# UMich-CURLY/unified_cvo

Hardware: AMD Instinct MI355X
Metric: frame-pair align()/sec, 10k x 10k geometric clouds (higher is better)
Workload: dtype f32

## Files before the change

include/cvo_hip_debug.h:

```cpp
#ifndef CVO_HIP_DEBUG_H
#define CVO_HIP_DEBUG_H

#include "cvo_hip.h"

#ifdef __cplusplus
extern "C" {
#endif

int cvo_debug_last_ell(cvo_ctx* ctx, int K, float* mat, int* ind, unsigned int* nonzeros);
int cvo_debug_last_geometry(cvo_ctx* ctx, int* n_groups, int* pairs_per_group);
int cvo_debug_time_scan(cvo_ctx* ctx, int reps, float* ms);
int cvo_debug_scan_stats(cvo_ctx* ctx, unsigned long long* tiles, int* rows_per_tile, int* targets_per_tile);
int cvo_debug_time_kernels(cvo_ctx* ctx, int reps, float* ms_assoc, float* ms_coeff);
int cvo_debug_kernel_clock(cvo_ctx* ctx, float* ms_assoc, float* ms_coeff, unsigned long long* launches);
int cvo_debug_list_builds(cvo_ctx* ctx, unsigned long long* builds, unsigned long long* iterations,
                          unsigned long long* candidate_evaluations);
int cvo_debug_row_classes(cvo_ctx* ctx, int pair, int* overflow_rows, int* scanned_rows, int* dense_regime);
int cvo_debug_speculation(cvo_ctx* ctx, int pair, int* adopted, int* iterations);
int cvo_debug_last_candidates(cvo_ctx* ctx, unsigned long long* out);
int cvo_debug_scalar_math(cvo_ctx* ctx, int op, int n, const double* in, double* out);
int cvo_debug_verified_rows(cvo_ctx* ctx, unsigned long long* rows);
int cvo_debug_cloud_order(const cvo_cloud* cloud, int* out);
int cvo_debug_last_score_batch(const cvo_ctx* ctx, int* overlap_evals, int* chain_evals, int* launches);
int cvo_debug_device_memory(cvo_ctx* ctx, size_t* free_bytes, size_t* total_bytes);
int cvo_debug_irls_normal(cvo_ctx* ctx, const cvo_cloud* frame1, const cvo_cloud* frame2, const double pose1[12],
                          const double pose2[12], double* out);
int cvo_debug_irls_eval(cvo_ctx* ctx, int n_frames, const cvo_cloud* const* clouds, const double* poses, int n_edges,
                        const int* edge_frames, const int* slot_off, const int* ent_r, const int* ent_c, const float* ent_w,
                        int normal, double* out);
int cvo_debug_irls_gather(cvo_ctx* ctx, int K, int* r, int* c, float* w);
int cvo_debug_voxel_stats(cvo_ctx* ctx, unsigned long long* capacity, unsigned long long* occupied,
                          unsigned long long* probes_total, unsigned long long* probe_longest, unsigned long long* entered);
int cvo_debug_rgbd_stats(cvo_ctx* ctx, int* n_tried, int* potentials , int* counts ,
                         unsigned long long* edge_selected, unsigned long long* edge_points,
                         unsigned long long* surface_points, unsigned long long* with_depth, int* on_device);
int cvo_debug_stereo_stats(cvo_ctx* ctx, int capacity, int* n_tried, int* thresholds, int* counts, int* threshold_used,
                           unsigned* histogram , unsigned long long* candidates, unsigned long long* kept, int* on_device);
int cvo_debug_lidar_stats(cvo_ctx* ctx, unsigned long long* counts , int* on_device);
int cvo_debug_lidar_atan2(int n, const double* y, const double* x, double* out);
int cvo_debug_nlm_stats(cvo_ctx* ctx, int* on_device, int* mult, int* shift, int* n_nonzero, int* tile_w, int* tile_h,
                        int* table_in_lds);

#ifdef __cplusplus
}
#endif
#endif
```

unified_cvo_amd/_capi.py:

```python
import ctypes as C
import os

HERE = os.path.dirname(os.path.abspath(__file__))
LIB_PATH = os.path.join(HERE, "lib", "libcvo_hip.so")

CVO_OK = 0
CVO_RET_FLOW_VANISHED = -1
CVO_E_INVALID = -2
CVO_E_HIP = -3
CVO_E_NOMEM = -4
CVO_E_UNSUPPORTED = -5
CVO_E_VERIFY = -6


class cvo_params_t(C.Structure):

    _fields_ = [
        ("ell_init_first_frame", C.c_float),
        ("ell_init", C.c_float),
        ("ell_min", C.c_float),
        ("min_ell_iter_limit", C.c_int),
        ("ell_max", C.c_float),
        ("dl", C.c_double),
        ("dl_step", C.c_double),
# ... 71 lines not shown
        ("ret", C.c_int),
        ("final_ell", C.c_float),
        ("final_num_neighbors", C.c_int),
        ("seconds", C.c_double),
    ]


class cvo_align_opts_t(C.Structure):
    _fields_ = [
        ("max_iterations", C.c_int),
        ("override_state", C.c_int),
        ("ell0", C.c_float),
        ("K0", C.c_int),
        ("trace", C.POINTER(cvo_trace_t)),
        ("trace_capacity", C.c_int),
        ("trace_dense", C.c_int),
        ("trace_every", C.c_int),
        ("n_trace", C.POINTER(C.c_int)),
        ("iters_per_launch", C.c_int),
        ("use_graph", C.c_int),
        ("kernel_clock", C.c_int),
    ]


class cvo_multiframe_info_t(C.Structure):
    _fields_ = [
        ("outer_iterations", C.c_int),
        ("solves", C.c_int),
        ("steps", C.c_int),
        ("accepted_steps", C.c_int),
        ("final_ell", C.c_float),
        ("last_total_nonzeros", C.c_uint),
        ("seconds", C.c_double),
    ]


class cvo_multiframe_trace_t(C.Structure):
    _fields_ = [
        ("iter", C.c_int),
        ("n_active_edges", C.c_int),
        ("solved", C.c_int),
        ("steps", C.c_int),
        ("accepted", C.c_int),
        ("termination", C.c_int),
        ("ell", C.c_float),
        ("total_nonzeros", C.c_uint),
        ("cost_initial", C.c_double),
        ("cost_final", C.c_double),
    ]


class cvo_batch_result_t(C.Structure):
    _fields_ = [
        ("ticket", C.c_longlong),
        ("transform", C.c_float * 16),
        ("info", cvo_align_info_t),
    ]


class cvo_rgbd_frame_t(C.Structure):
    _fields_ = [
        ("rows", C.c_int),
        ("cols", C.c_int),
        ("channels", C.c_int),
        ("image", C.c_void_p),
        ("gray", C.c_void_p),
        ("depth", C.c_void_p),
        ("depth_type", C.c_int),
        ("fx", C.c_float),
        ("fy", C.c_float),
        ("cx", C.c_float),
        ("cy", C.c_float),
        ("scaling_factor", C.c_float),
        ("num_classes", C.c_int),
        ("semantic", C.c_void_p),
    ]


class cvo_fast_schedule_t(C.Structure):
    _fields_ = [("thresh", C.c_int), ("num_want", C.c_int), ("num_min", C.c_int), ("break_thresh", C.c_int)]


class cvo_stereo_frame_t(C.Structure):
    _fields_ = [
        ("rows", C.c_int),
        ("cols", C.c_int),
        ("channels", C.c_int),
        ("image", C.c_void_p),
        ("gray", C.c_void_p),
        ("disparity", C.c_void_p),
        ("fx", C.c_float),
        ("fy", C.c_float),
        ("cx", C.c_float),
        ("cy", C.c_float),
        ("baseline", C.c_float),
        ("num_classes", C.c_int),
        ("semantic", C.c_void_p),
    ]


class cvo_lidar_scan_t(C.Structure):
    _fields_ = [("n", C.c_int), ("xyzi", C.c_void_p), ("semantic", C.c_void_p), ("num_classes", C.c_int)]


class cvo_lidar_config_t(C.Structure):
    _fields_ = [
        ("n_scan", C.c_int),
        ("horizon_scan", C.c_int),
        ("ang_res_x", C.c_float),
        ("ground_scan_ind", C.c_int),
        ("sensor_min_range", C.c_float),
        ("sensor_mount_angle", C.c_float),
        ("segment_theta", C.c_float),
        ("segment_alpha_x", C.c_float),
        ("segment_alpha_y", C.c_float),
        ("segment_valid_point_num", C.c_int),
        ("segment_valid_line_num", C.c_int),
        ("edge_threshold", C.c_float),
        ("surf_threshold", C.c_float),
        ("intensity_bound", C.c_double),
        ("depth_bound", C.c_double),
        ("distance_bound", C.c_double),
        ("beam_num", C.c_int),
        ("tan_theta", C.c_double),
        ("sin_alpha_x", C.c_double),
        ("cos_alpha_x", C.c_double),
        ("sin_alpha_y", C.c_double),
        ("cos_alpha_y", C.c_double),
        ("tan_ground_lo", C.c_double),
        ("tan_ground_hi", C.c_double),
        ("tan_self_lo", C.c_double),
        ("tan_self_hi", C.c_double),
    ]


class cvo_lidar_rand_t(C.Structure):
    _fields_ = [("r", C.c_uint * 31), ("front", C.c_int), ("rear", C.c_int)]


class cvo_nlm_config_t(C.Structure):
    _fields_ = [("h", C.c_float), ("template_window", C.c_int), ("search_window", C.c_int)]


CVO_DEPTH_U16, CVO_DEPTH_F32 = 0, 1
CVO_SELECT_CV_FAST, CVO_SELECT_DSO_EDGES, CVO_SELECT_FULL = 0, 2, 8
CVO_FAST_RGBD, CVO_FAST_STEREO, CVO_FAST_STEREO_SEMANTIC = (9, 15000, 12000, 13), (4, 24000, 15000, 50), (4, 28000, 15000, 50)

EXPORTED = [
    "cvo_params_default", "cvo_ctx_create", "cvo_ctx_destroy", "cvo_last_error", "cvo_ctx_stream",
    "cvo_ctx_synchronize", "cvo_cloud_upload", "cvo_cloud_upload_aos192", "cvo_cloud_size", "cvo_cloud_free",
    "cvo_align", "cvo_align_ex", "cvo_align_batch", "cvo_batch_poses_to_device", "cvo_inner_product",
    "cvo_function_angle", "cvo_association", "cvo_association_non_isotropic", "cvo_cloud_transformed", "cvo_edge_kernel_matrix", "cvo_debug_last_ell", "cvo_debug_time_scan", "cvo_debug_time_kernels",
    "cvo_debug_kernel_clock",
    "cvo_debug_last_candidates", "cvo_debug_list_builds", "cvo_debug_row_classes", "cvo_debug_speculation", "cvo_debug_scan_stats", "cvo_debug_last_geometry", "cvo_version",
    "cvo_align_association", "cvo_debug_scalar_math", "cvo_debug_verified_rows", "cvo_debug_device_memory", "cvo_cloud_upload_many",
    "cvo_ctx_set_option", "cvo_ctx_advice", "cvo_debug_cloud_order",
    "cvo_process_hint_hw_queues", "cvo_shutdown",
    "cvo_batch_open", "cvo_batch_submit", "cvo_batch_poll", "cvo_batch_pending", "cvo_batch_stats", "cvo_batch_close",
    "cvo_inner_product_batch", "cvo_function_angle_batch", "cvo_debug_last_score_batch",
    "cvo_multiframe_align", "cvo_debug_irls_normal", "cvo_debug_irls_eval", "cvo_debug_irls_gather",
    "cvo_voxel_select", "cvo_voxel_select_host", "cvo_cloud_upload_voxel", "cvo_debug_voxel_stats",
    "cvo_rgbd_points", "cvo_rgbd_points_host", "cvo_cloud_upload_rgbd", "cvo_debug_rgbd_stats",
    "cvo_fast_select", "cvo_fast_select_host", "cvo_stereo_points", "cvo_stereo_points_host", "cvo_cloud_upload_stereo",
    "cvo_cloud_upload_stereo_recipe", "cvo_debug_stereo_stats",
    "cvo_lidar_config_default", "cvo_lidar_config_derive", "cvo_lidar_rand_seed", "cvo_lidar_rand_next", "cvo_lidar_select", "cvo_lidar_select_host",
    "cvo_cloud_upload_lidar", "cvo_debug_lidar_stats", "cvo_debug_lidar_atan2",
    "cvo_nlm_config_default", "cvo_nlm_weights", "cvo_nlm_denoise_host", "cvo_nlm_denoise", "cvo_nlm_denoise_lab_host",
    "cvo_nlm_denoise_lab", "cvo_debug_nlm_stats",
]

_libs = {}


def lib(path=None):
    path = os.path.abspath(path) if path else LIB_PATH
    if path in _libs:
        return _libs[path]
    if not os.path.exists(path):
        raise RuntimeError(
            f"{path} is missing: build it with `python -m unified_cvo_amd.build` "
            "(there is no CPU fallback for the hot path)")
    L = C.CDLL(path)
    vp, ip, fp = C.c_void_p, C.c_int, C.POINTER(C.c_float)
    L.cvo_version.restype = C.c_char_p
    L.cvo_params_default.argtypes = [C.POINTER(cvo_params_t)]
    L.cvo_params_default.restype = None
    L.cvo_ctx_create.argtypes = [ip, C.POINTER(vp)]
    L.cvo_ctx_destroy.argtypes = [vp]
    L.cvo_ctx_destroy.restype = None
    L.cvo_ctx_set_option.argtypes = [vp, C.c_char_p, C.c_char_p]
    L.cvo_last_error.argtypes = [vp]
    L.cvo_last_error.restype = C.c_char_p
    L.cvo_ctx_advice.argtypes = [vp]
    L.cvo_ctx_advice.restype = C.c_char_p
    L.cvo_ctx_stream.argtypes = [vp]
    L.cvo_ctx_stream.restype = vp
    L.cvo_ctx_synchronize.argtypes = [vp]
    L.cvo_cloud_upload.argtypes = [vp, ip, fp, fp, fp, fp, C.POINTER(vp)]
    L.cvo_cloud_upload_aos192.argtypes = [vp, ip, vp, C.POINTER(vp)]
    L.cvo_cloud_upload_many.argtypes = [vp, ip, C.POINTER(C.c_int), C.POINTER(fp), C.POINTER(fp), C.POINTER(fp),
                                        C.POINTER(fp), ip, C.POINTER(vp)]
    L.cvo_cloud_size.argtypes = [vp]
    L.cvo_cloud_free.argtypes = [vp]
    L.cvo_cloud_free.restype = None
    L.cvo_align.argtypes = [vp, C.POINTER(cvo_params_t), vp, vp, fp, fp, C.POINTER(cvo_align_info_t)]
    L.cvo_align_ex.argtypes = [vp, C.POINTER(cvo_params_t), vp, vp, fp, fp, C.POINTER(cvo_align_info_t),
                               C.POINTER(cvo_align_opts_t)]
    L.cvo_align_batch.argtypes = [vp, C.POINTER(cvo_params_t), ip, C.POINTER(vp), C.POINTER(vp), fp, fp,
                                  C.POINTER(cvo_align_info_t), C.POINTER(cvo_align_opts_t)]
    L.cvo_batch_poses_to_device.argtypes = [vp, vp, ip]
    L.cvo_batch_open.argtypes = [vp, C.POINTER(cvo_params_t), ip, ip, ip, ip, C.POINTER(cvo_align_opts_t), C.POINTER(vp)]
    L.cvo_batch_submit.argtypes = [vp, vp, vp, fp, ip, C.POINTER(C.c_longlong)]
    L.cvo_batch_poll.argtypes = [vp, ip, ip, C.POINTER(cvo_batch_result_t), C.POINTER(C.c_int)]
    L.cvo_batch_pending.argtypes = [vp]
    L.cvo_batch_stats.argtypes = [vp, C.POINTER(C.c_ulonglong), C.POINTER(C.c_ulonglong), C.POINTER(C.c_ulonglong)]
    L.cvo_batch_close.argtypes = [vp]
    L.cvo_batch_close.restype = None
    L.cvo_inner_product.argtypes = [vp, C.POINTER(cvo_params_t), vp, vp, fp, C.c_float, fp]
    L.cvo_function_angle.argtypes = [vp, C.POINTER(cvo_params_t), vp, vp, fp, C.c_float, ip, fp]
    L.cvo_inner_product_batch.argtypes = [vp, C.POINTER(cvo_params_t), ip, C.POINTER(vp), C.POINTER(vp), fp, fp, fp]
    L.cvo_function_angle_batch.argtypes = [vp, C.POINTER(cvo_params_t), ip, C.POINTER(vp), C.POINTER(vp), fp, fp, ip, fp]
    L.cvo_debug_last_score_batch.argtypes = [vp, C.POINTER(C.c_int), C.POINTER(C.c_int), C.POINTER(C.c_int)]
    L.cvo_association.argtypes = [vp, C.POINTER(cvo_params_t), vp, vp, fp, C.c_float, C.POINTER(C.c_int),
                                  C.POINTER(C.c_int), fp, C.c_size_t, C.POINTER(C.c_size_t)]
    L.cvo_association_non_isotropic.argtypes = [vp, C.POINTER(cvo_params_t), vp, vp, fp, fp, C.POINTER(C.c_int),
                                                 C.POINTER(C.c_int), fp, C.c_size_t, C.POINTER(C.c_size_t)]
    L.cvo_cloud_transformed.argtypes = [vp, vp, fp, C.POINTER(vp)]
    L.cvo_edge_kernel_matrix.argtypes = [vp, C.POINTER(cvo_params_t), vp, vp, C.c_float, ip, fp, C.POINTER(C.c_int), C.POINTER(C.c_uint), C.POINTER(C.c_uint)]
    L.cvo_debug_last_ell.argtypes = [vp, ip, fp, C.POINTER(C.c_int), C.POINTER(C.c_uint)]
    L.cvo_debug_time_scan.argtypes = [vp, ip, fp]
    L.cvo_debug_time_kernels.argtypes = [vp, ip, fp, fp]
    L.cvo_debug_kernel_clock.argtypes = [vp, fp, fp, C.POINTER(C.c_ulonglong)]
    L.cvo_debug_last_candidates.argtypes = [vp, C.POINTER(C.c_ulonglong)]
    L.cvo_debug_list_builds.argtypes = [vp, C.POINTER(C.c_ulonglong), C.POINTER(C.c_ulonglong), C.POINTER(C.c_ulonglong)]
    L.cvo_debug_row_classes.argtypes = [vp, C.c_int, C.POINTER(C.c_int), C.POINTER(C.c_int), C.POINTER(C.c_int)]
    L.cvo_debug_speculation.argtypes = [vp, C.c_int, C.POINTER(C.c_int), C.POINTER(C.c_int)]
    L.cvo_debug_last_geometry.argtypes = [vp, C.POINTER(C.c_int), C.POINTER(C.c_int)]
    L.cvo_debug_scan_stats.argtypes = [vp, C.POINTER(C.c_ulonglong), C.POINTER(C.c_int), C.POINTER(C.c_int)]
    L.cvo_align_association.argtypes = [vp, ip, C.POINTER(C.c_int), C.POINTER(C.c_int), fp, C.c_size_t,
                                        C.POINTER(C.c_size_t), C.POINTER(C.c_int), C.POINTER(C.c_int)]
    L.cvo_debug_scalar_math.argtypes = [vp, ip, ip, C.POINTER(C.c_double), C.POINTER(C.c_double)]
    L.cvo_debug_verified_rows.argtypes = [vp, C.POINTER(C.c_ulonglong)]
    L.cvo_debug_device_memory.argtypes = [vp, C.POINTER(C.c_size_t), C.POINTER(C.c_size_t)]
    L.cvo_debug_cloud_order.argtypes = [vp, C.POINTER(C.c_int)]
    dp = C.POINTER(C.c_double)
    L.cvo_multiframe_align.argtypes = [vp, C.POINTER(cvo_params_t), ip, C.POINTER(vp), dp, C.POINTER(C.c_int), ip,
                                       C.POINTER(C.c_int), C.POINTER(cvo_multiframe_info_t),
                                       C.POINTER(cvo_multiframe_trace_t), ip, C.POINTER(C.c_int)]
    L.cvo_debug_irls_normal.argtypes = [vp, vp, vp, dp, dp, dp]
    ipp = C.POINTER(C.c_int)
    L.cvo_debug_irls_eval.argtypes = [vp, ip, C.POINTER(vp), dp, ip, ipp, ipp, ipp, ipp, fp, ip, dp]
    L.cvo_debug_irls_gather.argtypes = [vp, ip, ipp, ipp, fp]
    L.cvo_voxel_select.argtypes = [vp, ip, fp, C.c_float, ipp, ipp]
    L.cvo_voxel_select_host.argtypes = [ip, fp, C.c_float, ipp, ipp]
    L.cvo_cloud_upload_voxel.argtypes = [vp, ip, fp, fp, fp, fp, C.c_float, C.POINTER(vp), ipp, ipp]
    L.cvo_debug_voxel_stats.argtypes = [vp] + [C.POINTER(C.c_ulonglong)] * 5
    fr = C.POINTER(cvo_rgbd_frame_t)
    L.cvo_rgbd_points.argtypes = [vp, fr, ip, ipp, ipp, fp, fp, fp, fp]
    L.cvo_rgbd_points_host.argtypes = [fr, ip, ipp, ipp, fp, fp, fp, fp]
    L.cvo_cloud_upload_rgbd.argtypes = [vp, fr, C.c_float, C.c_float, C.POINTER(vp), ipp, C.POINTER(C.c_ubyte), ipp]
    L.cvo_debug_rgbd_stats.argtypes = [vp, ipp, ipp, ipp] + [C.POINTER(C.c_ulonglong)] * 4 + [ipp]
    sched, sf, up = C.POINTER(cvo_fast_schedule_t), C.POINTER(cvo_stereo_frame_t), C.POINTER(C.c_ubyte)
    L.cvo_fast_select.argtypes = [vp, ip, ip, up, sched, ipp, ipp, ipp]
    L.cvo_fast_select_host.argtypes = [ip, ip, up, sched, ipp, ipp, ipp]
    L.cvo_stereo_points.argtypes = [vp, sf, ip, ipp, ipp, fp, fp, fp, fp]
    L.cvo_stereo_points_host.argtypes = [sf, ip, ipp, ipp, fp, fp, fp, fp]
    L.cvo_cloud_upload_stereo.argtypes = [vp, sf, ip, C.POINTER(vp), ipp, ipp]
    L.cvo_cloud_upload_stereo_recipe.argtypes = [vp, sf, C.c_float, C.c_float, C.POINTER(vp), ipp, up, ipp]
    L.cvo_debug_stereo_stats.argtypes = [vp, ip, ipp, ipp, ipp, ipp, C.POINTER(C.c_uint)] + [C.POINTER(C.c_ulonglong)] * 2 + [ipp]
    ls, lc, lr = C.POINTER(cvo_lidar_scan_t), C.POINTER(cvo_lidar_config_t), C.POINTER(cvo_lidar_rand_t)
    L.cvo_lidar_config_default.argtypes = [lc, ip]
    L.cvo_lidar_config_default.restype = None
    L.cvo_lidar_config_derive.argtypes = [lc]
    L.cvo_lidar_config_derive.restype = None
    L.cvo_lidar_rand_seed.argtypes = [lr, C.c_uint]
    L.cvo_lidar_rand_seed.restype = None
    L.cvo_lidar_rand_next.argtypes = [lr]
    L.cvo_lidar_rand_next.restype = C.c_uint
    L.cvo_debug_lidar_atan2.argtypes = [ip, dp, dp, dp]
    L.cvo_lidar_select_host.argtypes = [ls, lc, lr, ipp, up, ipp]
    L.cvo_lidar_select.argtypes = [vp, ls, lc, lr, ipp, up, ipp]
    L.cvo_cloud_upload_lidar.argtypes = [vp, ls, lc, lr, C.POINTER(vp), ipp, ipp]
    L.cvo_debug_lidar_stats.argtypes = [vp, C.POINTER(C.c_ulonglong), ipp]
    nc, bp = C.POINTER(cvo_nlm_config_t), C.POINTER(C.c_ubyte)
    L.cvo_nlm_config_default.argtypes = [nc]
    L.cvo_nlm_config_default.restype = None
    L.cvo_nlm_weights.argtypes = [nc, ip, ipp, ip, ipp, ipp, ipp, ipp]
    L.cvo_nlm_denoise_host.argtypes = [ip, ip, ip, bp, nc, bp]
    L.cvo_nlm_denoise.argtypes = [vp, ip, ip, ip, bp, nc, bp]
    L.cvo_nlm_denoise_lab_host.argtypes = [ip, ip, bp, nc, C.c_float, bp]
    L.cvo_nlm_denoise_lab.argtypes = [vp, ip, ip, bp, nc, C.c_float, bp]
    L.cvo_debug_nlm_stats.argtypes = [vp] + [ipp] * 7
    for name in EXPORTED:
        getattr(L, name)
    _libs[path] = L
    return L
```

unified_cvo_amd/api.py:

```python
import ctypes as C
import weakref
import os

import numpy as np

from . import _capi
from .params import CvoParams, read_cvo_params_yaml
from .synth import FEATURE_DIMENSIONS, NUM_CLASSES


class CvoError(RuntimeError):
    pass


def _fptr(a):
    return None if a is None else a.ctypes.data_as(C.POINTER(C.c_float))


class CvoPointCloud:

    def __init__(self, feature_dimensions=0, num_classes=0):
        self.num_points_ = 0
        self.feature_dimensions_ = feature_dimensions
        self.num_classes_ = num_classes
# ... 967 lines not shown
        f1, f2 = self._dev(frame1), self._dev(frame2)
        K = int(num_neighbors)
        mat = np.zeros((f1.n, K), np.float32)
        ind = np.zeros((f1.n, K), np.int32)
        nz = np.zeros(f1.n, np.uint32)
        total = C.c_uint()
        p = self.params.to_ctypes()
        self._check(self.L.cvo_edge_kernel_matrix(self.ctx, C.byref(p), f1.handle, f2.handle, float(ell), K, _fptr(mat),
                                                  ind.ctypes.data_as(C.POINTER(C.c_int)),
                                                  nz.ctypes.data_as(C.POINTER(C.c_uint)), C.byref(total)))
        return mat, ind, nz, total.value

    def align_multiframe(self, frames, hold_const, edges, trace=False):
        frames = list(frames)
        F = len(frames)
        pos = {id(f): i for i, f in enumerate(frames)}
        flat = []
        for a, b in edges:
            for f in (a, b):
                flat.append(int(f) if isinstance(f, (int, np.integer)) else pos[id(f)])
        E = len(flat) // 2
        handles = (C.c_void_p * max(F, 1))(*[f._init.handle for f in frames])
        poses = np.ascontiguousarray(np.concatenate([np.asarray(f.pose_vec, np.float64).reshape(12) for f in frames])
                                     if F else np.zeros(12), np.float64)
        hold = None if hold_const is None else np.ascontiguousarray([1 if h else 0 for h in hold_const], np.int32)
        if hold is not None and hold.shape[0] != F:
            raise ValueError("hold_const: one flag per frame")
        ed = np.ascontiguousarray(flat if E else [0, 0], np.int32)
        info = _capi.cvo_multiframe_info_t()
        cap = max(self.params.multiframe_max_iters + 2, 1) if trace else 0
        rows = (_capi.cvo_multiframe_trace_t * max(cap, 1))()
        n_trace = C.c_int()
        p = self.params.to_ctypes()
        ip = C.POINTER(C.c_int)
        self._check(self.L.cvo_multiframe_align(
            self.ctx, C.byref(p), F, handles, poses.ctypes.data_as(C.POINTER(C.c_double)),
            None if hold is None else hold.ctypes.data_as(ip), E, ed.ctypes.data_as(ip), C.byref(info), rows, cap,
            C.byref(n_trace)))
        for i, f in enumerate(frames):
            f.pose_vec[:] = poses[12 * i:12 * i + 12]
            f.transform_pointcloud()
        names = [n for n, _ in _capi.cvo_multiframe_trace_t._fields_]
        out = [{n: getattr(rows[i], n) for n in names} for i in range(n_trace.value)]
        return {n: getattr(info, n) for n, _ in _capi.cvo_multiframe_info_t._fields_}, out

    def multiframe_align_raw(self, clouds, poses, hold_const, edges, trace_capacity=0):
        F = len(clouds)
        handles = (C.c_void_p * max(F, 1))(*[None if c is None else c.handle for c in clouds])
        P = np.ascontiguousarray(np.asarray(poses, np.float64).reshape(-1) if F else np.zeros(12), np.float64).copy()
        hold = None if hold_const is None else np.ascontiguousarray(hold_const, np.int32)
        ed = np.ascontiguousarray(list(edges) if len(edges) else [0, 0], np.int32)
        info = _capi.cvo_multiframe_info_t()
        rows = (_capi.cvo_multiframe_trace_t * max(trace_capacity, 1))()
        n_trace = C.c_int(-7)
        p = self.params.to_ctypes()
        ip = C.POINTER(C.c_int)
        rc = self.L.cvo_multiframe_align(self.ctx, C.byref(p), F, handles, P.ctypes.data_as(C.POINTER(C.c_double)),
                                         None if hold is None else hold.ctypes.data_as(ip), len(edges) // 2,
                                         ed.ctypes.data_as(ip), C.byref(info), rows, trace_capacity, C.byref(n_trace))
        return rc, P, info, rows, n_trace.value

    def debug_irls_normal(self, frame1, frame2, pose1, pose2):
        f1, f2 = self._dev(frame1), self._dev(frame2)
        a = np.ascontiguousarray(np.asarray(pose1, np.float64).reshape(12))
        b = np.ascontiguousarray(np.asarray(pose2, np.float64).reshape(12))
        out = np.zeros(91, np.float64)
        dp = C.POINTER(C.c_double)
        self._check(self.L.cvo_debug_irls_normal(self.ctx, f1.handle, f2.handle, a.ctypes.data_as(dp),
                                                 b.ctypes.data_as(dp), out.ctypes.data_as(dp)))
        H = np.zeros((12, 12))
        H[np.triu_indices(12)] = out[13:]
        H = H + np.triu(H, 1).T
        return out[0], out[1:13].copy(), H

    def debug_irls_eval(self, clouds, poses, edge_frames, slot_off, ent_r, ent_c, ent_w, normal=True):
        devs = [self._dev(c) for c in clouds]
        F = len(devs)
        handles = (C.c_void_p * max(F, 1))(*[d.handle for d in devs])
        X = np.ascontiguousarray(np.asarray(poses, np.float64).reshape(-1) if F else np.zeros(12))
        ef = np.ascontiguousarray(np.asarray(edge_frames, np.int32).reshape(-1))
        E = ef.shape[0] // 2
        so = np.ascontiguousarray(slot_off, np.int32)
        r, c = np.ascontiguousarray(ent_r, np.int32), np.ascontiguousarray(ent_c, np.int32)
        w = np.ascontiguousarray(ent_w, np.float32)
        if X.shape[0] != 12 * max(F, 1) or so.shape[0] != E + 1 or not (r.shape == c.shape == w.shape) or \
                (E and r.shape[0] < so[-1]):
            raise ValueError("debug_irls_eval: array sizes do not match")
        out = np.zeros((E, 91) if normal else (E,), np.float64)
        ip, dp = C.POINTER(C.c_int), C.POINTER(C.c_double)
        pad = np.zeros(1, np.int32)
        self._check(self.L.cvo_debug_irls_eval(
            self.ctx, F, handles, X.ctypes.data_as(dp), E, (ef if E else pad).ctypes.data_as(ip), so.ctypes.data_as(ip),
            (r if r.size else pad).ctypes.data_as(ip), (c if c.size else pad).ctypes.data_as(ip),
            _fptr(w if w.size else np.zeros(1, np.float32)), 1 if normal else 0,
            (out if E else np.zeros(1)).ctypes.data_as(dp)))
        return out

    def debug_irls_gather(self, n_rows, K):
        r = np.zeros((n_rows, K), np.int32)
        c = np.zeros((n_rows, K), np.int32)
        w = np.zeros((n_rows, K), np.float32)
        ip = C.POINTER(C.c_int)
        self._check(self.L.cvo_debug_irls_gather(self.ctx, K, r.ctypes.data_as(ip), c.ctypes.data_as(ip), _fptr(w)))
        return r, c, w

    def debug_last_ell(self, n_rows, K):
        mat = np.zeros((n_rows, K), np.float32)
        ind = np.zeros((n_rows, K), np.int32)
        nz = np.zeros(n_rows, np.uint32)
        self._check(self.L.cvo_debug_last_ell(self.ctx, K, _fptr(mat), ind.ctypes.data_as(C.POINTER(C.c_int)),
                                              nz.ctypes.data_as(C.POINTER(C.c_uint))))
        return mat, ind, nz

    def debug_time_scan(self, reps=20):
        ms = C.c_float()
        self._check(self.L.cvo_debug_time_scan(self.ctx, reps, C.byref(ms)))
        return ms.value

    def debug_time_kernels(self, reps=20):
        a, c = C.c_float(), C.c_float()
        self._check(self.L.cvo_debug_time_kernels(self.ctx, reps, C.byref(a), C.byref(c)))
        return a.value, c.value

    def debug_kernel_clock(self):
        a, c, n = C.c_float(), C.c_float(), C.c_ulonglong()
        self._check(self.L.cvo_debug_kernel_clock(self.ctx, C.byref(a), C.byref(c), C.byref(n)))
        return a.value, c.value, n.value

    def debug_last_geometry(self):
        g, p = C.c_int(), C.c_int()
        self._check(self.L.cvo_debug_last_geometry(self.ctx, C.byref(g), C.byref(p)))
        return g.value, p.value

    def debug_scan_stats(self):
        t, r, c = C.c_ulonglong(), C.c_int(), C.c_int()
        self._check(self.L.cvo_debug_scan_stats(self.ctx, C.byref(t), C.byref(r), C.byref(c)))
        return t.value, r.value, c.value

    def debug_list_builds(self):
        b, it, ce = C.c_ulonglong(), C.c_ulonglong(), C.c_ulonglong()
        self._check(self.L.cvo_debug_list_builds(self.ctx, C.byref(b), C.byref(it), C.byref(ce)))
        return b.value, it.value, ce.value

    def debug_row_classes(self, pair=0):
        a, b, c = C.c_int(), C.c_int(), C.c_int()
        self._check(self.L.cvo_debug_row_classes(self.ctx, pair, C.byref(a), C.byref(b), C.byref(c)))
        return a.value, b.value, bool(c.value)

    def debug_speculation(self, pair=0):
        a, it = C.c_int(), C.c_int()
        self._check(self.L.cvo_debug_speculation(self.ctx, pair, C.byref(a), C.byref(it)))
        return a.value, it.value

    def advice(self):
        return self.L.cvo_ctx_advice(self.ctx).decode()

    def debug_scalar_math(self, op, items):
        dp = C.POINTER(C.c_double)
        if op == 7:
            a = np.ascontiguousarray(items, np.float64).reshape(-1)
            n = a.shape[0] - 2
            out = np.zeros(n, np.float64)
        else:
            it = np.atleast_2d(np.asarray(items, np.float64))
            n = it.shape[0]
            a = np.zeros((n, 16), np.float64)
            a[:, :it.shape[1]] = it
            out = np.zeros((n, 16), np.float64)
        self._check(self.L.cvo_debug_scalar_math(self.ctx, op, n, a.ctypes.data_as(dp), out.ctypes.data_as(dp)))
        return out

    def debug_device_memory(self):
        f, t = C.c_size_t(), C.c_size_t()
        self._check(self.L.cvo_debug_device_memory(self.ctx, C.byref(f), C.byref(t)))
        return f.value, t.value

    def debug_verified_rows(self):
        v = C.c_ulonglong()
        self._check(self.L.cvo_debug_verified_rows(self.ctx, C.byref(v)))
        return v.value

    def debug_last_candidates(self):
        v = C.c_ulonglong()
        self._check(self.L.cvo_debug_last_candidates(self.ctx, C.byref(v)))
        return v.value


class CvoFrameGPU:

    def __init__(self, gpu, pts, poses):
        self.gpu = gpu
        self.points = pts
        self.pose_vec = np.asarray(poses, np.float64).reshape(12).copy()
        self._init = gpu.upload(pts)
        self._transformed = None
        self.transform_pointcloud()

    def transform_pointcloud(self):
        if self._transformed is not None:
            self._transformed.free()
        self._transformed = self.gpu.transformed(self._init, self.pose_vec)

    def points_transformed_gpu(self):
        return self._transformed


class BinaryStateGPU:

    def __init__(self, frame1, frame2, num_neighbor, init_ell):
        self.frame1, self.frame2 = frame1, frame2
        self.init_num_neighbors = int(num_neighbor)
        self.num_neighbors = int(num_neighbor)
        self.ell = float(init_ell)
        self.iter = 0
        self.mat = self.ind = self.nonzeros = None
        self.nonzero_sum = 0

    def update_inner_product(self):
        last = int(self.nonzeros.max()) if self.nonzeros is not None and self.nonzeros.size else 0
        if last > 0:
            self.num_neighbors = min(self.init_num_neighbors, int(last * 1.1))
        gpu = self.frame1.gpu
        self.mat, self.ind, self.nonzeros, self.nonzero_sum = gpu.edge_kernel_matrix(
            self.frame1.points_transformed_gpu(), self.frame2.points_transformed_gpu(), self.ell, self.num_neighbors)
        self.iter += 1
        return self.nonzero_sum
```

unified_cvo_amd/csrc/cvo_debug.hip:

```cpp
extern "C" {

int cvo_debug_scalar_math(cvo_ctx* ctx, int op, int n, const double* in, double* out) {
  if (!ctx || !in || !out || n <= 0 || op < 0 || op > 13) return fail(ctx, CVO_E_INVALID, "cvo_debug_scalar_math: bad argument");
  HIP_TRY(ctx, hipSetDevice(ctx->device));
  const size_t n_in = op == 7 ? (size_t)n + 2 : 16 * (size_t)n, n_out = op == 7 ? (size_t)n : 16 * (size_t)n;
  double *d_in = nullptr, *d_out = nullptr;
  PairState* d_st = nullptr;
  int rc = CVO_OK;
  auto cleanup = [&]() {
    if (d_in) (void)hipFree(d_in);
    if (d_out) (void)hipFree(d_out);
    if (d_st) (void)hipFree(d_st);
  };
  if (hipMalloc(&d_in, sizeof(double) * n_in) != hipSuccess || hipMalloc(&d_out, sizeof(double) * n_out) != hipSuccess ||
      hipMalloc(&d_st, sizeof(PairState)) != hipSuccess) {
    cleanup();
    return fail(ctx, CVO_E_NOMEM, "cvo_debug_scalar_math: hipMalloc failed");
  }
  hipError_t e = hipMemcpyAsync(d_in, in, sizeof(double) * n_in, hipMemcpyHostToDevice, ctx->stream);
  if (e == hipSuccess) e = hipMemsetAsync(d_out, 0, sizeof(double) * n_out, ctx->stream);
  if (e == hipSuccess) e = hipMemsetAsync(d_st, 0, sizeof(PairState), ctx->stream);
  if (e == hipSuccess) {
    hipLaunchKernelGGL(k_scalar_math, dim3(op == 7 ? 1 : n), dim3(64), 0, ctx->stream, op, n, d_in, d_out, d_st);
    e = hipGetLastError();
// ... 23 lines not shown
  if (!ctx) return CVO_E_INVALID;
  if (overlap_evals) *overlap_evals = ctx->last_score_overlap;
  if (chain_evals) *chain_evals = ctx->last_score_chain;
  if (launches) *launches = ctx->last_score_launches;
  return CVO_OK;
}

int cvo_debug_verified_rows(cvo_ctx* ctx, unsigned long long* rows) {
  if (!ctx || !rows || ctx->last_pairs < 1) return fail(ctx, CVO_E_INVALID, "cvo_debug_verified_rows: bad argument");
  unsigned long long t = 0;
  for (int p = 0; p < ctx->last_pairs; p++) t += ctx->h_states[p].verify_rows;
  *rows = t;
  return CVO_OK;
}

int cvo_debug_last_candidates(cvo_ctx* ctx, unsigned long long* out) {
  if (!ctx || !out || ctx->last_pairs < 1) return fail(ctx, CVO_E_INVALID, "cvo_debug_last_candidates: bad argument");
  *out = ctx->h_states[0].ncand;
  return CVO_OK;
}

int cvo_debug_time_kernels(cvo_ctx* ctx, int reps, float* ms_assoc, float* ms_coeff) {
  if (!ctx || reps <= 0 || ctx->last_pairs < 1 || !ms_assoc || !ms_coeff)
    return fail(ctx, CVO_E_INVALID, "cvo_debug_time_kernels: bad argument");
  HIP_TRY(ctx, hipSetDevice(ctx->device));
  const int n_pairs = ctx->last_pairs, G = ctx->last.G;
  const DevParams& dp = ctx->last_params;
  const LaunchGeom& g0 = ctx->last.geom;
  const IterWords w = iteration_words({.idx32 = !g0.idx16, .rebuild_follows = true, .replay = true});
  float out[2] = {0.f, 0.f};
  for (int which = 0; which < 2; which++) {
    auto sweep = [&]() {
      for (int q = 0; q < G; q++) {
        const LaunchGeom g = group_geom(ctx, ctx->last, n_pairs, q);
        const PairDesc* descs = ctx->d_descs + g.p0;
        if (which == 0)
          launch_assoc(ctx->stream, g.idx16, g.feat, g.instr, g.nba, g.n_pairs, descs, ctx->d_params, ctx->d_states + g.p0, g.arena,
                       w.assoc);
        else
          launch_coeff(ctx->stream, g.instr, g.nba, g.csplit, g.n_pairs, descs, ctx->d_params, ctx->d_states + g.p0, g.arena, w.iter);
      }
    };
    sweep();
    HIP_TRY(ctx, hipEventRecord(ctx->ev_start, ctx->stream));
    for (int r = 0; r < reps; r++) sweep();
    HIP_TRY(ctx, hipEventRecord(ctx->ev_stop, ctx->stream));
    HIP_TRY(ctx, hipGetLastError());
    HIP_TRY(ctx, hipStreamSynchronize(ctx->stream));
    HIP_TRY(ctx, hipEventElapsedTime(&out[which], ctx->ev_start, ctx->ev_stop));
    out[which] /= (float)(reps * G);
  }
  if (dp.phase_ticks) {
    static unsigned long long h[2][8192][4];
    HIP_TRY(ctx, hipMemcpyFromSymbol(h, HIP_SYMBOL(g_phase_ticks), sizeof(h)));
    const int np = n_pairs - (int)((long)n_pairs * (G - 1) / G);
    for (int which = 0; which < 2; which++) {
      const int nb = std::min(4096, 8 * ((np + 7) / 8) * g0.nba * (which ? g0.csplit : 1));
      double sum[3] = {0, 0, 0}, mx[3] = {0, 0, 0};
      int cnt = 0;
      for (int b = 0; b < nb; b++) {
        if (!h[which][b][0] || !h[which][b][3]) continue;
        for (int q = 0; q < 3; q++) {
          const double d = (double)(long long)(h[which][b][q + 1] - h[which][b][q]);
          sum[q] += d;
          mx[q] = std::max(mx[q], d);
        }
        cnt++;
      }
      if (!cnt) continue;
      fprintf(stderr, "[cvo] %s: %d blocks; ticks (avg / max) %s %.0f / %.0f, row loop %.0f / %.0f, %s %.0f / %.0f\n",
              which ? "k_coeff" : "k_assoc", cnt, which ? "prologue + twist" : "prologue", sum[0] / cnt, mx[0], sum[1] / cnt,
              mx[1], which ? "reduction + counter" : "reduction + flow gate", sum[2] / cnt, mx[2]);
      if (which)
        for (int p = 0; p < std::min(np, 3); p++)
          fprintf(stderr, "[cvo]   pair %d, updating block: entry -> counter %.0f, update %.0f ticks\n", p,
                  (double)(long long)(h[1][4096 + p][1] - h[1][4096 + p][0]),
                  (double)(long long)(h[1][4096 + p][2] - h[1][4096 + p][1]));
      if (which) {
        unsigned long long u[8];
        HIP_TRY(ctx, hipMemcpyFromSymbol(u, HIP_SYMBOL(g_upd_ticks), sizeof(u)));
        fprintf(stderr, "[cvo]   inside the update (last pair to run it): reduce %lld, step %lld, pose + distance + indicator %lld, "
                        "update_tf + list bookkeeping %lld, rest %lld, write-back %lld ticks\n",
                (long long)(u[1] - u[0]), (long long)(u[2] - u[1]), (long long)(u[3] - u[2]), (long long)(u[4] - u[3]),
                (long long)(u[5] - u[4]), (long long)(u[6] - u[5]));
      }
    }
  }
  *ms_assoc = out[0];
  *ms_coeff = out[1];
  return CVO_OK;
}

int cvo_debug_kernel_clock(cvo_ctx* ctx, float* ms_assoc, float* ms_coeff, unsigned long long* launches) {
  if (!ctx || ctx->last_pairs < 1 || !ms_assoc || !ms_coeff)
    return fail(ctx, CVO_E_INVALID, "cvo_debug_kernel_clock: bad argument");
  if (!ctx->last_params.kernel_clock) return fail(ctx, CVO_E_INVALID, "cvo_debug_kernel_clock: the last call ran without CVO_KERNEL_CLOCK");
  HIP_TRY(ctx, hipSetDevice(ctx->device));
  if (ctx->clock_ms_per_tick <= 0.0) {
    HIP_TRY(ctx, hipStreamSynchronize(ctx->stream));
    float ms = 0.f;
    for (int rep = 0; rep < 2; rep++) {
      HIP_TRY(ctx, hipEventRecord(ctx->ev_start, ctx->stream));
      hipLaunchKernelGGL(k_hold, dim3(1), dim3(64), 0, ctx->stream, 1000000ull);
      HIP_TRY(ctx, hipEventRecord(ctx->ev_stop, ctx->stream));
      HIP_TRY(ctx, hipStreamSynchronize(ctx->stream));
      HIP_TRY(ctx, hipEventElapsedTime(&ms, ctx->ev_start, ctx->ev_stop));
    }
    ctx->clock_ms_per_tick = (double)ms / 1e6;
  }
  double sum[2] = {0, 0}, n[2] = {0, 0};
  for (int p = 0; p < ctx->last_pairs; p++)
    for (int w = 0; w < 2; w++) {
      sum[w] += (double)ctx->h_states[p].clk_sum[w];
      n[w] += (double)ctx->h_states[p].clk_n[w];
    }
  *ms_assoc = n[0] > 0 ? (float)(sum[0] / n[0] * ctx->clock_ms_per_tick) : 0.f;
  *ms_coeff = n[1] > 0 ? (float)(sum[1] / n[1] * ctx->clock_ms_per_tick) : 0.f;
  if (launches) *launches = (unsigned long long)n[1];
  return CVO_OK;
}

int cvo_debug_list_builds(cvo_ctx* ctx, unsigned long long* builds, unsigned long long* iterations,
                          unsigned long long* candidate_evaluations) {
  if (!ctx || !builds || ctx->last_pairs < 1) return fail(ctx, CVO_E_INVALID, "cvo_debug_list_builds: bad argument");
  unsigned long long b = 0, it = 0, ce = 0;
  for (int p = 0; p < ctx->last_pairs; p++) {
    b += (unsigned long long)ctx->h_states[p].n_builds;
    it += (unsigned long long)ctx->h_states[p].iterations;
    ce += ctx->h_states[p].ncand_total;
  }
  *builds = b;
  if (iterations) *iterations = it;
  if (candidate_evaluations) *candidate_evaluations = ce;
  return CVO_OK;
}

int cvo_debug_row_classes(cvo_ctx* ctx, int pair, int* overflow_rows, int* scanned_rows, int* dense_regime) {
  if (!ctx || pair < 0 || pair >= ctx->last_pairs) return fail(ctx, CVO_E_INVALID, "cvo_debug_row_classes: bad argument");
  const PairState& st = ctx->h_states[pair];
  if (overflow_rows) *overflow_rows = st.n_ovf;
  if (scanned_rows) *scanned_rows = st.n_scan;
  if (dense_regime) *dense_regime = st.all_dense;
  return CVO_OK;
}

int cvo_debug_speculation(cvo_ctx* ctx, int pair, int* adopted, int* iterations) {
  if (!ctx || pair < 0 || pair >= ctx->last_pairs) return fail(ctx, CVO_E_INVALID, "cvo_debug_speculation: bad argument");
  const PairState& st = ctx->h_states[pair];
  if (adopted) *adopted = st.n_adopted;
  if (iterations) *iterations = st.status ? st.iterations : st.k;
  return CVO_OK;
}

int cvo_debug_scan_stats(cvo_ctx* ctx, unsigned long long* tiles, int* rows_per_tile, int* targets_per_tile) {
  if (!ctx || !tiles || ctx->last_pairs < 1) return fail(ctx, CVO_E_INVALID, "cvo_debug_scan_stats: bad argument");
  HIP_TRY(ctx, hipSetDevice(ctx->device));
  unsigned long long total = 0;
  for (int p = 0; p < ctx->last_pairs; p++) {
    unsigned long long v = 0;
    HIP_TRY(ctx, hipMemcpy(&v, ctx->h_descs[p].tile_count, sizeof(v), hipMemcpyDeviceToHost));
    total += v;
  }
  *tiles = total;
  if (rows_per_tile) *rows_per_tile = ROWS_PER_GROUP;
  if (targets_per_tile) *targets_per_tile = 64 * ctx->last.geom.T;
  return CVO_OK;
}

int cvo_debug_last_geometry(cvo_ctx* ctx, int* n_groups, int* pairs_per_group) {
  if (!ctx || ctx->last_pairs < 1) return fail(ctx, CVO_E_INVALID, "cvo_debug_last_geometry: bad argument");
  if (n_groups) *n_groups = ctx->last.G;
  if (pairs_per_group) *pairs_per_group = (ctx->last_pairs + ctx->last.G - 1) / ctx->last.G;
  return CVO_OK;
}

int cvo_debug_time_scan(cvo_ctx* ctx, int reps, float* ms) {
  if (!ctx || !ms || reps <= 0 || ctx->last_pairs < 1)
    return fail(ctx, CVO_E_INVALID, "cvo_debug_time_scan: bad argument");
  HIP_TRY(ctx, hipSetDevice(ctx->device));
  const int n_pairs = ctx->last_pairs, G = ctx->last.G;
  auto sweep = [&]() {
    for (int q = 0; q < G; q++) {
      const LaunchGeom g = group_geom(ctx, ctx->last, n_pairs, q);
      launch_scan(ctx->stream, g.T, dim3(g.gx, g.gy, g.n_pairs), ctx->d_descs + g.p0, ctx->d_params, ctx->d_states + g.p0, true);
    }
  };
  sweep();
  HIP_TRY(ctx, hipEventRecord(ctx->ev_start, ctx->stream));
  for (int r = 0; r < reps; r++) sweep();
  HIP_TRY(ctx, hipEventRecord(ctx->ev_stop, ctx->stream));
  HIP_TRY(ctx, hipGetLastError());
  for (int p = 0; p < n_pairs; p++) {
    const PairDesc& D = ctx->h_descs[p];
    HIP_TRY(ctx, hipMemsetAsync(D.rowbits, 0, sizeof(unsigned) * (size_t)(ctx->last.N + 4) * D.rbw, ctx->stream));
  }
  HIP_TRY(ctx, hipStreamSynchronize(ctx->stream));
  float t = 0;
  HIP_TRY(ctx, hipEventElapsedTime(&t, ctx->ev_start, ctx->ev_stop));
  *ms = t / (reps * G);
  return CVO_OK;
}

}
```

unified_cvo_amd/csrc/cvo_device.h:

```cpp
#pragma once
#include <hip/hip_runtime.h>

#include "../../include/cvo_hip.h"
#include "../../include/cvo_hip_debug.h"

namespace cvo_dev {

constexpr int FD = CVO_FEATURE_DIMENSIONS;
constexpr int NC = CVO_NUM_CLASSES;
constexpr int FD_PAD = 8;
constexpr int NC_PAD = 20;
constexpr int IND_CAP = 512;

enum CallMode : int {
  CALL_ALIGN = 0,
  CALL_SINGLE = 1,
  CALL_NONISO = 2,
};

struct DevParams {
  float sp_thres, sigma2, c2, c_sigma2, s_ell, s_sigma, c, d;
  float log_geo;
  float d2_c_thres, d2_s_thres;
  float ell_min, ell_decay_rate;
  int ell_decay_start;
  int max_iter;
  float eps, eps_2, min_step, max_step;
  int K_max;
  int window;
  float stable_thr;
  int use_geo, use_col, use_sem, use_range_ell, use_geotype;
  int trace_dense, trace_every, trace_capacity;
  int mode;
  float kinv[9];
  float d2_cull;
  float s_ell_sq;
  int T;
  int groups_per_block;
  float skin_frac;
  float rebuild_shrink;
  int lean_U;
  int lean_U2;
  int calm_U;
  int shrink_align;
  float skin_min, skin_max;
  float skin_blend;
  int dense_regime;
  float lean_skin;
  float horizon_margin;
  int kernel_clock;
  int phase_ticks;
  int verify_lists;
  int keep_columns;
  int fast_div_cd;
  int row_max_cap;
  int row_max_busy;
  int long_lists;
  int debug_drop_partial;
  int debug_no_motion_bound;
  int no_speculate;
};

struct PairState {
  int status;
  int rebuild;
  int n_ovf;
  int K;
  float ell;
  int epoch;
  int k;
  int iterations;
  float Rinv[9], Tinv[3];
  float R[9], T[3];
  int ret;
  float step;
  float omega[3], v[3];
  unsigned nnz, max_nnz;
  double B, C, D, E;
  double dist;
  double asum;
  unsigned long long ncand;
  unsigned long long ncand_list;
  unsigned long long noverflow;
  unsigned long long ncand_total;
  int n_trace;
  float out_T[16];
  float Rb[9], Tb[3];
  float ell_build;
  float skin_rot, skin_tr;
  int n_builds;
  int n_adopted;
  int sync_err;
  int want_full, n_stalls;
  int all_dense;
  float skin_scale;
  int row_max;
  int n_scan;
  int s_head, s_size, e_head, e_size;
  float s_sum, e_sum;
  unsigned clk_last_assoc, clk_n[2];
  float last_used, last_rate;
  int K_last;
  float temp_coef;
  unsigned long long clk_sum[2];
  float sq[IND_CAP], eq[IND_CAP];
  float xi[48];
  unsigned long long clk_start[2];
  int verify_err, verify_k, verify_pos, verify_what;
  unsigned long long verify_rows;
};

#ifdef CVO_ELL8
struct EllEntry {
  float a;
  int p;
};
static_assert(sizeof(EllEntry) == 8, "EllEntry");
constexpr bool ELL8 = true;
#else
struct EllEntry {
  float a, yx, yy, yz;
};
static_assert(sizeof(EllEntry) == 16, "EllEntry");
constexpr bool ELL8 = false;
#endif
__device__ __forceinline__ EllEntry make_ell(float a, float yx, float yy, float yz, int p) {
#ifdef CVO_ELL8
  return EllEntry{a, p};
#else
  return EllEntry{a, yx, yy, yz};
#endif
}

struct RowRes {
  float o[3], v[3];
  double asum;
};
static_assert(sizeof(RowRes) == 32, "RowRes");

constexpr int ROW_PAD = 256;
__host__ __device__ inline size_t row_off_cand_cnt(int) { return 0; }
__host__ __device__ inline size_t row_off_ip(int Np) { return (size_t)4 * Np; }
__host__ __device__ inline size_t row_off_nnz(int Np) { return (size_t)8 * Np; }
__host__ __device__ inline size_t row_off_xp4(int Np) { return (size_t)16 * Np; }
__host__ __device__ inline size_t row_off_cand_j(int Np) { return (size_t)32 * Np; }
__host__ __device__ inline size_t row_off_ell(int Np) { return (size_t)160 * Np; }

struct PairDesc {
  int N, M, nblk_assoc, nblk_coeff;
  int* cand_cnt;
  void* cand_j;
  float4* xp4;
  int* ip;
  const float4* y4;
  EllEntry* ell;
  int* ell_j;
  unsigned* nnz_row;
  double* rowcoef;
  RowRes* rowres;
  unsigned long long* flow_part;
  unsigned long long* cnt_part;
  unsigned long long* shadow;
  unsigned long long* coef_part;
  int* done;
  int csplit;
  const float4* xfeat;
  const float4* yfeat;
  const float4* xlabel;
  const float4* ylabel;
  const float2* xgeo;
  const float2* ygeo;
  const int* xlid;
  const int* ylid;
  int Mpad, nchunks, nslices, rbw;
  int NG;
  int NGpad;
  float cx, cy, cz;
  float ymax;
  double sqrt_nm;
  const float4* x4;
  const float4* xs4;
  const int* xorder;
  const float4* ys4;
  const int* yorder;
  const int* yinv;
  float4* ycull;
  float4* xcull;
  int* rowperm;
  int* iorig;
  float4* gbox;
  float4* cellbox;
  float4* sbox;
  unsigned long long* masks;
  unsigned* rowbits;
  int* row_cnt;
  unsigned long long* tile_count;
  int* ovf_rows;
  unsigned long long* ovf_bits;
  unsigned short* long_j;
  unsigned long long* long_stamp;
  unsigned long long call_serial;
  int max_iter;
  PairState* st;
  cvo_trace_t* trace;
  int* status_out;
  int* want_out;
  int* status_host;
  int* want_host;
  double* asum_host;
  int* gate;
  int* gate_flow;
  int* dense_rel;
  int* ovf_wsum;
  int* word_base;
  int* dense_off;
};

constexpr unsigned NNZ_DENSE_FLAG = 0x80000000u;
__host__ __device__ inline unsigned nnz_count(unsigned v) { return v & ~NNZ_DENSE_FLAG; }
constexpr int ELL_LOWER_SLOTS = 64;
__host__ __device__ inline size_t ell_index(int N, int s, int pos, int off) {
  return off >= 0 ? (size_t)off + (size_t)s : (size_t)s * (size_t)N + (size_t)pos;
}
__host__ __device__ inline size_t ell_upper_capacity(int N, int K_max) {
  return K_max > ELL_LOWER_SLOTS ? (size_t)(K_max - ELL_LOWER_SLOTS) * (size_t)N : 0;
}
constexpr int COEFF_SPLIT_MAX = 32;
constexpr int ROWS_PER_GROUP = 4;

enum AssocFlags : int {
  ASSOC_LEAN = 1,
  ASSOC_REPLAY = 2,
  ASSOC_LEAN_DENSE = 4,
  ASSOC_ASUM_ONLY = 8,
};
enum IterFlags : int {
  ITER_LEAN = 1,
  ITER_REBUILD_FOLLOWS = 2,
  ITER_FROM_COEFF = 4,
  ITER_REPLAY = 8,
  ITER_LEAN_DENSE = 32,
  ITER_IDX32 = 64,
};
constexpr int ITER_HORIZON_SHIFT = 8;
__host__ __device__ constexpr int iter_horizon(int flags) { return flags >> ITER_HORIZON_SHIFT; }

struct SlotState {
  int rebuild, n_ovf;
};
template <class St>
__device__ __forceinline__ bool slot_waits(int flags, int lean, int lean_dense, const St* st) {
  bool w = false;
  if ((flags & lean) && (st->rebuild || (st->n_ovf > 0 && !(flags & lean_dense)))) w = true;
  return w;
}

constexpr int ASSOC_WORD_FLAG_BITS = 4, ASSOC_WORD_NBLK_BITS = 16;
constexpr int COEFF_WORD_NBLK_BITS = 14, COEFF_WORD_SPLIT_BITS = 6;
constexpr int LAUNCH_WORD_PAIR_SHIFT = 20, LAUNCH_WORD_PAIR_BITS = 12;
constexpr int LAUNCH_PAIRS_MAX = (1 << LAUNCH_WORD_PAIR_BITS) - 1;
constexpr int LAUNCH_NBLK_MAX = (1 << COEFF_WORD_NBLK_BITS) - 1;
struct AssocWord {
// ... 698 lines not shown
```

unified_cvo_amd/csrc/cvo_internal.h:

```cpp
#pragma once
#include <hip/hip_runtime.h>

#include <algorithm>
#include <atomic>
#include <chrono>
#include <climits>
#include <cmath>
#include <cstdio>
#include <cstdlib>
#include <cstdint>
#include <cstring>
#include <deque>
#include <map>
#include <memory_resource>
#include <mutex>
#include <string>
#include <thread>
#include <tuple>
#include <vector>

#include "cvo_kernels.h"

using namespace cvo_dev;

#include "cvo_options.h"

#define CVO_VERSION_STRING "unified_cvo_amd 0.1 (gfx950)"

struct cvo_cloud {
  cvo_ctx* ctx = nullptr;
  int device = 0;
  int n = 0;
  char* slab = nullptr;
  size_t slab_bytes = 0;
  float4* x4 = nullptr;
  float4* xs4 = nullptr;
  float4* feat = nullptr;
  float4* label = nullptr;
  float2* geo = nullptr;
  int* lid = nullptr;
  mutable char* zero_slab = nullptr;
  mutable float4* tile4 = nullptr;
  int* order = nullptr;
  int* inv = nullptr;
  std::vector<int> h_order;
  float cx = 0, cy = 0, cz = 0;
  float rmax = 0;
};

namespace {

enum class ChunkKind { Full, FullNoDense, Lean, ShortLean, Calm };
static const char* const kChunkNames[] = {"full", "full-nodense", "lean", "short", "calm"};

struct ChunkPlan {
  ChunkKind kind = ChunkKind::Full;
  bool dense = false;
  int U = 0;
  int period = 0;
  bool every_iteration() const { return kind == ChunkKind::Full || kind == ChunkKind::FullNoDense; }
};

struct ArenaArg {
  const char* base;
  unsigned stride256;
  int Npad;
};

struct GraphKey {
  ChunkPlan plan;
  int n_pairs = 0, p0 = 0, T = 0, gx = 0, gy = 0, npb = 0, nbl = 0, nba = 0, csplit = 0, dense_blocks = 0, horizon_cap = 0, feat = 0;
  bool idx16 = false, wide = false, instr = false, verify = false;
  ArenaArg arena{};
  auto fields() const {
    return std::tie(plan.kind, plan.dense, plan.U, plan.period, n_pairs, p0, T, gx, gy, npb, nbl, nba, csplit, dense_blocks,
                    horizon_cap, feat, idx16, wide, instr, verify, arena.base, arena.stride256, arena.Npad);
  }
  bool operator==(const GraphKey& o) const { return fields() == o.fields(); }
};

struct Dims {
  int Mpad, nchunks, rbw_max, nblk_assoc, NG, NGpad, Npad;
};

struct LaunchGeom {
  int n_pairs, p0, T, gx, gy, nba, npb, csplit;
  int nbl, nbv;
  int dense_blocks = DENSE_BLOCKS_MIN;
  int horizon_cap = 1 << 20;
  bool idx16, instr, verify;
  bool wide;
  int feat = FEAT_GEO;
  hipStream_t stream;
  ArenaArg arena;
};

struct BatchSetup {
  int N, M, G;
  bool long_lists = false;
  Dims d;
  size_t slot_bytes;
  LaunchGeom geom;
};

struct CachedGraph {
  hipGraphExec_t exec = nullptr;
  GraphKey key;
};

inline size_t align_up(size_t v, size_t a) { return (v + a - 1) / a * a; }

}

struct RgbdStatsAcc {
  int n_tried = 0, tried[8] = {}, count[8] = {};
  unsigned long long edge_selected = 0, edge_points = 0, surface_points = 0, with_depth = 0;
  int on_device = 0;
};

struct StereoStatsAcc {
  std::vector<int> tried, count;
  int threshold_used = -1;
  unsigned hist[257] = {};
  unsigned long long candidates = 0, kept = 0;
  int on_device = 0;
};

struct LidarStatsAcc {
  unsigned long long projected = 0, ground = 0, valid = 0, invalid = 0, segmented = 0, edges = 0, draws = 0, thinned = 0, edge_detected = 0;
  int on_device = 0;
};

struct NlmStatsAcc {
  int on_device = 0, mult = 0, shift = 0, n_nonzero = 0, tile_w = 0, tile_h = 0, table_in_lds = 0;
};

struct ScratchLayout {
  size_t off = 0;
  size_t take(size_t bytes) {
    const size_t o = off;
    off = align_up(off + bytes, 256);
    return o;
  }
};

struct DeviceScratch {
  char* p = nullptr;
  size_t bytes = 0;
  int reserve(cvo_ctx* ctx, size_t need, const char* what);
  void release() {
    if (p) (void)hipFree(p);
    p = nullptr;
    bytes = 0;
  }
};

struct cvo_ctx {
  int device = 0;
  CtxOptions opt;
  std::mutex upload_mutex;
  std::mutex kd_mutex;
  KdJob* d_kd_jobs = nullptr;
  int kd_jobs_cap = 0;
  hipStream_t stream = nullptr;
  hipStream_t upload_stream = nullptr;
  std::string err;
  std::string advice;
  char* arena = nullptr;
  size_t arena_bytes = 0;
  PairDesc* d_descs = nullptr;
  PairState* d_states = nullptr;
  int* d_status = nullptr;
  DevParams* d_params = nullptr;
  char* d_ctl = nullptr;
  char* h_ctl = nullptr;
  size_t ctl_bytes = 0, ctl_off_status = 0, ctl_off_descs = 0, ctl_off_states = 0;
  int cap_pairs = 0;
  std::vector<PairDesc> h_descs;
  std::vector<PairState> h_states;
  char* d_sb = nullptr;
  char* d_sb_table = nullptr;
  char* h_sb = nullptr;
  char* h_sb_res = nullptr;
  int sb_jobs_cap = 0, sb_tiles_cap = 0;
  int last_score_overlap = 0, last_score_chain = 0, last_score_launches = 0;
  int* h_status[2] = {nullptr, nullptr};
  hipEvent_t ev_start = nullptr, ev_stop = nullptr;
  static constexpr int MAX_GROUPS = MAX_STREAMS;
  hipStream_t gstream[MAX_GROUPS] = {};
  hipEvent_t ev_chk[2][MAX_GROUPS] = {};
  hipEvent_t ev_fork = nullptr, ev_join[MAX_GROUPS] = {};
  static constexpr int GRAPH_SLOTS = 48;
  CachedGraph graphs[MAX_GROUPS][GRAPH_SLOTS];
  CachedGraph chain_graph;
  int last_chunks = 0, last_lean_launches = 0, last_full_launches = 0;
  int last_pairs = 0;
  BatchSetup last{};
  DevParams last_params{};
  std::vector<int> last_xorder;
  bool queue_open = false;
  cvo_batch_queue* queue = nullptr;
  DeviceScratch vox_scratch;
  unsigned long long vox_capacity = 0;
  VoxelCtl vox_last{};
  DeviceScratch rgbd_scratch;
  std::vector<unsigned char> rgbd_excl;
  RgbdStatsAcc rgbd_last{};
  StereoStatsAcc stereo_last{};
  DeviceScratch lidar_scratch;
  LidarStatsAcc lidar_last{};
  DeviceScratch nlm_scratch;
  NlmStatsAcc nlm_last{};
  double clock_ms_per_tick = 0.0;
};

namespace {

int fail(cvo_ctx* ctx, int code, const std::string& msg) {
  if (ctx) ctx->err = msg;
  return code;
}

#define HIP_TRY(ctx, expr)                                                                       \
  do {                                                                                           \
    hipError_t e__ = (expr);                                                                     \
    if (e__ != hipSuccess)                                                                       \
      return fail(ctx, CVO_E_HIP, std::string(#expr) + ": " + hipGetErrorString(e__));           \
  } while (0)

}
```

unified_cvo_amd/csrc/cvo_k_assoc.h:

```cpp
#pragma once
#include "cvo_wave.h"
#include "cvo_pair_math.h"

namespace cvo_dev {

static_assert(sizeof(XiMats) <= 46 * sizeof(float), "PairState::xi holds an XiMats and the two words of its stamp");
__device__ __forceinline__ double coeff_twist_load(const PairDesc* __restrict__ D, int nparts, unsigned tag) {
  const int lane = threadIdx.x & 63;
  const CVO_GLOBAL unsigned long long* src = as_global(D->flow_part) + 2 * (lane & 7);
  double acc = 0;
  for (int b = lane >> 3; b < nparts; b += 64) {
    TaggedF64 p[8];
    const bool pad = (lane & 7) == 7;
    for (int polls = 0;; polls++) {
#pragma unroll
      for (int u = 0; u < 8; u++) p[u] = ld_tagged<true>(src + (size_t)min(b + 8 * u, nparts - 1) * FLOW_GRANULES);
      bool ok = true;
#pragma unroll
      for (int u = 0; u < 8; u++) ok = ok && (pad || p[u].carries(tag));
      if (__ballot(!ok) == 0ull) break;
      if (polls > PARTIAL_POLL_LIMIT) {
        if (lane == 0) D->st->sync_err = 1;
        break;
      }
      __builtin_amdgcn_s_sleep(2);
    }
#pragma unroll
    for (int u = 0; u < 8; u++) acc += (b + 8 * u < nparts) ? p[u].value() : 0.0;
  }
  return acc;
}
__device__ __forceinline__ void twist_finalize(const PairDesc* __restrict__ D, int nparts, unsigned tag, int stamp_epoch, int stamp_k) {
  double acc = coeff_twist_load(D, nparts, tag);
  acc += dpp_f64<0x128>(acc);
  acc = xor16_sum(acc);
  acc = xor32_sum(acc);
  float own = (float)acc;
  float ov[6];
#pragma unroll
  for (int q = 0; q < 6; q++) ov[q] = __builtin_bit_cast(float, __builtin_amdgcn_readlane(__builtin_bit_cast(int, own), q));
  float z = 0;
#pragma unroll
  for (int q = 0; q < 6; q++) z = z + ov[q] * ov[q];
  if (z > 0) {
    const float sq = sqrtf(z);
    own = own / sq;
#pragma unroll
    for (int q = 0; q < 6; q++) ov[q] = __builtin_bit_cast(float, __builtin_amdgcn_readlane(__builtin_bit_cast(int, own), q));
  }
  XiMats M;
  xi_mats(ov, ov + 3, M);
  if ((threadIdx.x & 63) == 0) {
    const float* mv = reinterpret_cast<const float*>(&M);
    float* dst = D->st->xi;
#pragma unroll
    for (int q = 0; q < (int)(sizeof(XiMats) / sizeof(float)); q++) dst[q] = mv[q];
    dst[46] = __int_as_float(stamp_epoch);
    dst[47] = __int_as_float(stamp_k);
  }
}
__device__ __forceinline__ bool flow_gate(const PairDesc* __restrict__ D, int nblocks, int nparts, unsigned tag, int stamp_epoch, int stamp_k) {
  __shared__ int s_flow_last;
  __syncthreads();
  if (threadIdx.x == 0) {
    const int done = __hip_atomic_fetch_add(D->gate_flow, 1, __ATOMIC_RELAXED, __HIP_MEMORY_SCOPE_AGENT);
    s_flow_last = (done == nblocks - 1) ? 1 : 0;
    if (done == nblocks - 1) __hip_atomic_store(D->gate_flow, 0, __ATOMIC_RELAXED, __HIP_MEMORY_SCOPE_AGENT);
  }
  __syncthreads();
  if (s_flow_last && threadIdx.x < 64) twist_finalize(D, nparts, tag, stamp_epoch, stamp_k);
  return s_flow_last != 0;
}

__device__ __forceinline__ void asum_gate(const PairDesc* __restrict__ D, int nblk) {
  __shared__ int s_asum_last;
  asm volatile("s_waitcnt vmcnt(0)" ::: "memory");
  __syncthreads();
  if (threadIdx.x == 0) {
    const int done = __hip_atomic_fetch_add(D->gate_flow, 1, __ATOMIC_RELAXED, __HIP_MEMORY_SCOPE_AGENT);
    s_asum_last = (done == nblk - 1) ? 1 : 0;
    if (done == nblk - 1) __hip_atomic_store(D->gate_flow, 0, __ATOMIC_RELAXED, __HIP_MEMORY_SCOPE_AGENT);
  }
  __syncthreads();
  if (!s_asum_last) return;
  double s = 0;
  if (threadIdx.x < 16)
    for (int b = (int)threadIdx.x; b < nblk; b += 16) s += ld_tagged<true>(as_global(D->flow_part) + (size_t)b * FLOW_GRANULES + 12).value();
  s += dpp_f64<DPP_XOR1>(s);
  s += dpp_f64<DPP_XOR2>(s);
  s += dpp_f64<DPP_HALF_MIRROR>(s);
  s += dpp_f64<DPP_MIRROR>(s);
  if (threadIdx.x == 0) {
    D->st->asum = s;
    *D->asum_host = s;
  }
}

__device__ unsigned long long g_phase_ticks[2][8192][4];
__device__ unsigned long long g_upd_ticks[8];
#define CVO_UPD_STAMP(i) do { if (P.phase_ticks && threadIdx.x == 0) g_upd_ticks[i] = __builtin_readcyclecounter(); } while (0)

__device__ __forceinline__ void pair_clock_begin(bool on, PairState* st, int which) {
  if (on && threadIdx.x == 0) st_x<true>(&st->clk_start[which], (unsigned long long)__builtin_amdgcn_s_memrealtime());
}
__device__ __forceinline__ unsigned long long pair_clock_peek(bool on, const PairState* st, int which) {
  return (on && threadIdx.x == 0) ? ld_x<true>(&st->clk_start[which]) : 0ull;
}
__device__ __forceinline__ unsigned pair_clock_ticks(unsigned long long t0) {
  const unsigned long long t1 = __builtin_amdgcn_s_memrealtime();
  return (t0 != 0ull && t0 <= t1 && t1 - t0 < 400000ull) ? (unsigned)(t1 - t0) : 0u;
}
struct AssocRowHead {
  int cnt, ip, j1;
  float4 x;
};
template <int NC>
struct BlockRedShared {
  double v[NC][ASSOC_THREADS + 8];
};
template <int NC>
__device__ __forceinline__ double block_reduce_lds(BlockRedShared<NC>& S, const double (&x)[NC]) {
  static_assert(NC <= 8, "eight lanes per component in one wave");
#pragma unroll
  for (int c = 0; c < NC; c++) S.v[c][threadIdx.x] = x[c];
  __syncthreads();
  double t = 0;
  if (threadIdx.x < 8 * NC) {
    const int c = threadIdx.x >> 3, g = threadIdx.x & 7;
    double p[ASSOC_THREADS / 8];
#pragma unroll
    for (int k = 0; k < ASSOC_THREADS / 8; k++) p[k] = S.v[c][8 * k + g];
#pragma unroll
    for (int k = 0; k < ASSOC_THREADS / 8; k++) t += p[k];
  }
  if (threadIdx.x < 64) {
    t += dpp_f64<DPP_XOR1>(t);
    t += dpp_f64<DPP_XOR2>(t);
    t += dpp_f64<DPP_HALF_MIRROR>(t);
  }
  return t;
}

struct AssocShared {
  union {
    BlockRedShared<7> red;
    EllEntry stage[ELL_STAGE][ASSOC_THREADS];
  };
  unsigned long long cnt[ASSOC_THREADS / 64][4];
};

template <typename IdxT, int ASSOC_CAP, int FEAT, bool INSTR>
__device__ __forceinline__ void assoc_phase(const DevParams& P, const PairDesc* __restrict__ D, const IterView& iv,
                                            AssocShared& S, const int bx, const AssocRowHead& head, const unsigned tag) {
  const int N = D->N;
  const int pos = bx * ASSOC_THREADS + threadIdx.x;
  const int K = iv.K;
  RowAcc A;
  A.slot = D->ell + pos;
  A.stage = (CVO_LDS ell_vec_t*)&S.stage[0][threadIdx.x];
  unsigned overflowed = 0;
  unsigned long long tt1 = 0, tt2 = 0;
  if (pos < N) {
    const int j1s = head.j1;
    const int j2s = (int)(reinterpret_cast<const IdxT*>(D->cand_j) + pos)[N];
    const int cnt = head.cnt;
    overflowed = cnt > min(iv.row_max, ASSOC_CAP) ? 1u : 0u;
    if (!overflowed) {
      const int i = head.ip;
      const float4 x = head.x;
      RowData r = make_row(P, x, iv.ell);
      if (FEAT == FEAT_HOT) r.lid = D->xlid[i];
      const FeatDen F = make_feat_den(P);
      const V3 pxe{x.x, x.y, x.z};
      const Pose& pose = iv.pose;
      const CVO_GLOBAL IdxT* cj = as_global(reinterpret_cast<const IdxT*>(D->cand_j)) + pos;
      const CVO_GLOBAL f32x4* ysrc = (const CVO_GLOBAL f32x4*)D->ys4;
      int j1 = cnt > 0 ? j1s : 0;
      int j2 = cnt > 1 ? j2s : 0;
      if (INSTR) tt1 = __builtin_readcyclecounter();
      float4 y1 = ldg_xyz(ysrc + j1);
      const CVO_GLOBAL IdxT* cjn = cj + (size_t)2 * N;
      if (geo_fast_path<FEAT>(P)) {
        for (int k = 0; k < cnt && A.nnz < (unsigned)K; k++) {
          const int j = j1;
          const float4 ycur = y1;
          j1 = j2;
          y1 = ldg_xyz(ysrc + j1);
          if (k + 2 < cnt) j2 = (int)*cjn;
          cjn += N;
          const V3 ytv = transform_point(pose.Ri, pose.Ti, ycur.x, ycur.y, ycur.z);
          visit_pair_geo(P, F, N, r, pxe, j, ytv, A);
        }
      } else {
        for (int k = 0; k < cnt && A.nnz < (unsigned)K; k++) {
          const int j = j1;
          const float4 ycur = y1;
          j1 = j2;
          y1 = ldg_xyz(ysrc + j1);
          if (k + 2 < cnt) j2 = (int)*cjn;
          cjn += N;
          const V3 ytv = transform_point(pose.Ri, pose.Ti, ycur.x, ycur.y, ycur.z);
          visit_pair_yt<FEAT>(P, D, F, i, pos, N, r, pxe, j, make_float4(ytv.x, ytv.y, ytv.z, 0.f), A);
        }
      }
      D->nnz_row[pos] = A.nnz;
      {
        const unsigned ns = min(A.nnz, (unsigned)ELL_STAGE);
        EllEntry* dst = D->ell + pos;
        for (unsigned q = 0; q < ns; q++) {
          const ell_vec_t ev = A.stage[q * ASSOC_THREADS];
#ifdef CVO_ELL8
          asm volatile("flat_store_dwordx2 %0, %1 sc1" ::"v"(dst), "v"(ev) : "memory");
#else
          asm volatile("flat_store_dwordx4 %0, %1 sc1" ::"v"(dst), "v"(ev) : "memory");
#endif
          dst += N;
        }
      }
      if (INSTR) tt2 = __builtin_readcyclecounter();
    } else {
      const RowRes rr = D->rowres[pos];
      A.o0 = rr.o[0]; A.o1 = rr.o[1]; A.o2 = rr.o[2];
      A.v0 = rr.v[0]; A.v1 = rr.v[1]; A.v2 = rr.v[2];
      A.asum = rr.asum;
      A.nnz = nnz_count(D->nnz_row[pos]);
    }
  }
  if (INSTR && P.phase_ticks && threadIdx.x == 0) {
    g_phase_ticks[0][blockIdx.x & 8191][1] = tt1;
    g_phase_ticks[0][blockIdx.x & 8191][2] = tt2;
  }
  float fq[6];
  {
    const float fn[6] = {A.o0, A.o1, A.o2, A.v0, A.v1, A.v2};
    const bool safe = P.fast_div_cd != 0 && fdiv_operands_safe(fn);
    if (__ballot(!safe) == 0ull) {
      const FDivU uc = fdiv_prepare(P.c), ud = fdiv_prepare(P.d);
#pragma unroll
      for (int q = 0; q < 3; q++) {
        fq[q] = fdiv_hoisted(fn[q], uc);
        fq[3 + q] = fdiv_hoisted(fn[3 + q], ud);
      }
    } else {
#pragma unroll
      for (int q = 0; q < 3; q++) {
        fq[q] = fn[q] / P.c;
        fq[3 + q] = fn[3 + q] / P.d;
      }
    }
  }
  const double red[7] = {(double)fq[0], (double)fq[1], (double)fq[2], (double)fq[3], (double)fq[4], (double)fq[5], A.asum};
  constexpr int NW = ASSOC_THREADS / 64;
  const int wave = threadIdx.x >> 6, lane = threadIdx.x & 63;
  const unsigned long long nn = wave_sum_u32(A.nnz);
  const unsigned mx = wave_max_u32(A.nnz);
  const unsigned long long nov = (unsigned long long)__builtin_popcountll(__ballot(overflowed != 0));
  if (lane == 0) {
    S.cnt[wave][0] = nn;
    S.cnt[wave][1] = mx;
    S.cnt[wave][2] = 0ull;
    S.cnt[wave][3] = nov;
  }
  __syncthreads();
  const double tot = block_reduce_lds<7>(S.red, red);
  if (threadIdx.x < 56 && (threadIdx.x & 7) == 0 && !(P.debug_drop_partial == 1 && bx == 1)) {
    st_tagged(D->flow_part + (size_t)bx * FLOW_GRANULES + 2 * (threadIdx.x >> 3), tot, tag);
  } else if (threadIdx.x == 57) {
    unsigned long long a0 = 0, a1 = 0, a2 = 0, a3 = 0;
#pragma unroll
    for (int w = 0; w < NW; w++) {
      a0 += S.cnt[w][0];
      a1 = max(a1, S.cnt[w][1]);
      a2 += S.cnt[w][2];
      a3 += S.cnt[w][3];
    }
    unsigned long long* cp = D->cnt_part + (size_t)bx * 4;
    cp[0] = a0;
    cp[1] = a1;
    cp[2] = a2;
    cp[3] = a3;
  }
}

template <typename IdxT, int ASSOC_CAP, int FEAT, bool INSTR>
__global__ __launch_bounds__(ASSOC_THREADS, FEAT != FEAT_GEO ? 1 : CVO_ASSOC_WAVES) void k_assoc(const PairDesc* __restrict__ descs,
                                                          const DevParams* __restrict__ Pp,
                                                          const PairState* __restrict__ states,
                                                          const char* __restrict__ arena, int lean_nblk_pairs,
                                                          unsigned stride256, int Npad) {
  const unsigned long long tt0 = INSTR ? __builtin_readcyclecounter() : 0ull;
  const AssocWord aw = unpack_assoc_word(lean_nblk_pairs);
  const int lean = aw.flags, nblk = aw.nblk, n_pairs = aw.n_pairs;
  PairBlock pb;
  if (!pair_block(nblk, n_pairs, pb)) return;
  const PairDesc* __restrict__ D = descs + pb.pair;
  const PairState* __restrict__ st = states + pb.pair;
  AssocRowHead head;
  {
    const char* wb = arena + (size_t)pb.pair * ((size_t)stride256 << 8);
    const int pos = pb.bx * ASSOC_THREADS + threadIdx.x;
    head.ip = FEAT != FEAT_GEO ? reinterpret_cast<const int*>(wb + row_off_ip(Npad))[pos] : 0;
    head.j1 = (int)reinterpret_cast<const IdxT*>(wb + row_off_cand_j(Npad))[pos];
    head.x = reinterpret_cast<const float4*>(wb + row_off_xp4(Npad))[pos];
    head.cnt = __float_as_int(head.x.w);
  }
  const int status_v = st->status, rebuild_v = st->rebuild, n_ovf_v = st->n_ovf;
  const DevParams P = *Pp;
  {
    const int n = D->N, k = st->K;
    const int* a0 = D->cand_cnt;
    const void* a1 = D->cand_j;
    const float4* a2 = D->xp4;
    const float4* a3 = D->ys4;
    const EllEntry* a4 = D->ell;
    const float e = st->ell, r0 = st->Rinv[0], t0 = st->Tinv[0];
    asm volatile("" ::"s"(n), "s"(k), "s"(a0), "s"(a1), "s"(a2), "s"(a3), "s"(a4), "s"(e), "s"(r0), "s"(t0), "s"(P.sp_thres),
                 "s"(P.log_geo), "s"(P.c), "s"(P.d), "s"(P.d2_c_thres));
  }
  const bool replay = (lean & ASSOC_REPLAY) != 0;
  if (!replay && status_v != 0) return;
  const SlotState sv{rebuild_v, n_ovf_v};
  if (slot_waits(lean, ASSOC_LEAN, ASSOC_LEAN_DENSE, &sv)) return;
  pair_clock_begin(INSTR && P.kernel_clock && (lean & (ASSOC_LEAN | ASSOC_REPLAY)) == ASSOC_LEAN && pb.bx == 0, const_cast<PairState*>(st), 0);
  __shared__ AssocShared S;
  const int stamp_epoch = st->epoch, stamp_k = st->k;
  const unsigned tag = partial_tag(D->call_serial, (unsigned)stamp_k);
  assoc_phase<IdxT, ASSOC_CAP, FEAT, INSTR>(P, D, load_iter_view(st), S, pb.bx, head, tag);
  if (threadIdx.x >= 64) return;
  if (P.mode == CALL_ALIGN) {
    const unsigned long long clk0 = pair_clock_peek(INSTR && P.kernel_clock && (lean & (ASSOC_LEAN | ASSOC_REPLAY)) == ASSOC_LEAN, st, 0);
    const bool last = flow_gate(D, nblk, nblk, tag, stamp_epoch, stamp_k);
    if (last && threadIdx.x == 0 && clk0) D->st->clk_last_assoc = pair_clock_ticks(clk0);
  } else if (lean & ASSOC_ASUM_ONLY) {
    asum_gate(D, nblk);
  }
  if (INSTR && P.phase_ticks && threadIdx.x == 0) {
    g_phase_ticks[0][blockIdx.x & 8191][0] = tt0;
    g_phase_ticks[0][blockIdx.x & 8191][3] = __builtin_readcyclecounter();
  }
}

}
```

unified_cvo_amd/csrc/cvo_kernels.h:

```cpp
#pragma once
#include "cvo_device.h"

#if defined(__HIP_DEVICE_COMPILE__) && !defined(__gfx950__)
#error "unified_cvo_amd kernels target gfx950 (MI355X) only: build with --offload-arch=gfx950"
#endif

#ifndef CVO_COEFF_WAVES
#define CVO_COEFF_WAVES 1
#endif
#ifndef CVO_ASSOC_WAVES
#define CVO_ASSOC_WAVES 6
#endif


#include "cvo_wave.h"
#include "cvo_pair_math.h"
#include "cvo_k_prep.h"
#include "cvo_k_scan.h"
#include "cvo_k_list.h"
#include "cvo_k_assoc.h"
#include "cvo_k_assoc_dense.h"
#include "cvo_update.h"
#include "cvo_k_coeff.h"
#include "cvo_k_overlap.h"
#include "cvo_k_coeff_dense.h"
#include "cvo_k_debug.h"
#include "cvo_k_cloud.h"
#include "cvo_k_irls.h"
#include "cvo_k_compact.h"
#include "cvo_k_voxel.h"
#include "cvo_k_rgbd.h"
#include "cvo_k_fast.h"
#include "cvo_k_stereo.h"
#include "cvo_k_lidar.h"
#include "cvo_k_nlm.h"
```

unified_cvo_amd/csrc/cvo_launch.hip:

```cpp
#ifndef CVO_COEFF_DENSE_MULTI_FROM
#define CVO_COEFF_DENSE_MULTI_FROM 8
#endif

namespace {

void choose_scan_config(const cvo_ctx* ctx, int n_pairs, int NG, int Mpad, int* T_out, int* gpb_out) {
  const int T = 2;
  const long slices = Mpad / (64 * T);
  const int ngr = (int)align_up((size_t)NG, 64);
  int gpb = ngr;
  while (gpb > 64) {
    const long waves = slices * ((ngr + gpb - 1) / gpb) * n_pairs;
    if (waves >= 4096) break;
    gpb = (int)align_up((size_t)gpb / 2, 64);
  }
  *T_out = T;
  *gpb_out = gpb;
}

void launch_scan(hipStream_t s, int T, dim3 grid, const PairDesc* descs, const DevParams* dp, const PairState* st, bool force) {
  switch (T) {
    case 1: hipLaunchKernelGGL(k_scan<1>, grid, dim3(256), 0, s, descs, dp, st, force); break;
    case 2: hipLaunchKernelGGL(k_scan<2>, grid, dim3(256), 0, s, descs, dp, st, force); break;
    case 4: hipLaunchKernelGGL(k_scan<4>, grid, dim3(256), 0, s, descs, dp, st, force); break;
    default: hipLaunchKernelGGL(k_scan<8>, grid, dim3(256), 0, s, descs, dp, st, force); break;
  }
}

inline dim3 row_grid(int nblk, int n_pairs) { return dim3((unsigned)(nblk * ((n_pairs + 7) / 8 * 8))); }

void launch_list(hipStream_t s, bool idx16, int nblk, int n_pairs, const PairDesc* descs, const DevParams* dp,
                 const PairState* st) {
  const dim3 blk(LIST_THREADS), grid = row_grid(nblk, n_pairs);
  if (idx16)
    hipLaunchKernelGGL((k_list<unsigned short, ASSOC_CAP16>), grid, blk, 0, s, descs, dp, st, nblk, n_pairs);
  else
    hipLaunchKernelGGL((k_list<int, ASSOC_CAP32>), grid, blk, 0, s, descs, dp, st, nblk, n_pairs);
}

template <typename IdxT, int CAP, int FEAT>
void launch_assoc_t(hipStream_t s, bool instr, dim3 grid, const PairDesc* descs, const DevParams* dp, const PairState* st,
                    const ArenaArg& A, int packed) {
  const dim3 blk(ASSOC_THREADS);
  if (instr)
    hipLaunchKernelGGL((k_assoc<IdxT, CAP, FEAT, true>), grid, blk, 0, s, descs, dp, st, A.base, packed, A.stride256, A.Npad);
  else
    hipLaunchKernelGGL((k_assoc<IdxT, CAP, FEAT, false>), grid, blk, 0, s, descs, dp, st, A.base, packed, A.stride256, A.Npad);
}

void launch_assoc(hipStream_t s, bool idx16, int feat, bool instr, int nblk, int n_pairs, const PairDesc* descs,
                  const DevParams* dp, const PairState* st, const ArenaArg& A, int flags) {
  const dim3 grid = row_grid(nblk, n_pairs);
  const int packed = pack_assoc_word(flags, nblk, n_pairs);
#define CVO_ASSOC_CASE(F)                                                                              \
  case F:                                                                                              \
    if (idx16)                                                                                         \
      launch_assoc_t<unsigned short, ASSOC_CAP16, F>(s, instr, grid, descs, dp, st, A, packed);        \
    else                                                                                               \
      launch_assoc_t<int, ASSOC_CAP32, F>(s, instr, grid, descs, dp, st, A, packed);                   \
    break;
  switch (feat) {
    CVO_ASSOC_CASE(FEAT_GEO)
    CVO_ASSOC_CASE(FEAT_COL)
    CVO_ASSOC_CASE(FEAT_HOT)
    default:
      CVO_ASSOC_CASE(FEAT_ALL)
  }
#undef CVO_ASSOC_CASE
}

void launch_coeff(hipStream_t s, bool instr, int nblk, int split, int n_pairs, const PairDesc* descs, const DevParams* dp,
                  PairState* st, const ArenaArg& A, int flags) {
  const int packed = pack_coeff_word(nblk, split, n_pairs);
  if (instr)
    hipLaunchKernelGGL(k_coeff<true>, row_grid(nblk * split + 1, n_pairs), dim3(ASSOC_THREADS), 0, s, descs, dp, st, A.base, flags,
                       packed, A.stride256, A.Npad);
  else
    hipLaunchKernelGGL(k_coeff<false>, row_grid(nblk * split + 1, n_pairs), dim3(ASSOC_THREADS), 0, s, descs, dp, st, A.base, flags,
                       packed, A.stride256, A.Npad);
}

void launch_verify(hipStream_t s, int feat, int nblk, int n_pairs, const PairDesc* descs, const DevParams* dp, const int* st,
                   int flags) {
  const dim3 grid((unsigned)nblk, (unsigned)n_pairs);
  if (feat != FEAT_GEO)
    hipLaunchKernelGGL(k_verify<FEAT_ALL>, grid, dim3(256), 0, s, descs, dp, st, flags);
  else
    hipLaunchKernelGGL(k_verify<FEAT_GEO>, grid, dim3(256), 0, s, descs, dp, st, flags);
}

inline bool dense_wide(int N, int n_pairs) { return n_pairs <= 1 && N <= DENSE_BLOCKS_MAX / 2; }

void launch_dense(hipStream_t s, int feat, bool wide, int n_pairs, int dense_blocks, const PairDesc* descs, const DevParams* dp,
                  const PairState* st) {
  const dim3 grid(dense_blocks, n_pairs);
#define CVO_LAUNCH_DENSE(F)                                                                                  \
  do {                                                                                                       \
    if (wide)                                                                                                \
      hipLaunchKernelGGL((k_assoc_dense<F, 4, true>), grid, dim3(256), 0, s, descs, dp, st);                 \
    else                                                                                                     \
      hipLaunchKernelGGL((k_assoc_dense<F, 4, false>), grid, dim3(256), 0, s, descs, dp, st);                \
  } while (0)
  switch (feat) {
    case FEAT_GEO: CVO_LAUNCH_DENSE(FEAT_GEO); break;
    case FEAT_COL: CVO_LAUNCH_DENSE(FEAT_COL); break;
    case FEAT_HOT: CVO_LAUNCH_DENSE(FEAT_HOT); break;
    default: CVO_LAUNCH_DENSE(FEAT_ALL); break;
  }
#undef CVO_LAUNCH_DENSE
}

inline int call_feat(const DevParams& dp, bool all_one_hot) {
  if (dp.mode == CALL_NONISO) return FEAT_ALL;
  if (!(dp.use_col || dp.use_sem || dp.use_geotype)) return FEAT_GEO;
  if (!dp.use_sem) return FEAT_COL;
  return all_one_hot ? FEAT_HOT : FEAT_ALL;
}

struct IterSlot {
  bool lean = false;
  bool lean_dense = false;
  bool idx32 = false;
  bool rebuild_follows = false;
  int horizon = 0;
  bool replay = false;
  bool asum_only = false;
};
struct IterWords {
  int assoc;
  int iter;
};
inline IterWords iteration_words(const IterSlot& s) {
  const bool lean_dense = s.lean && s.lean_dense;
  return {(s.lean ? ASSOC_LEAN : 0) | (s.replay ? ASSOC_REPLAY : 0) | (lean_dense ? ASSOC_LEAN_DENSE : 0) |
              (s.asum_only ? ASSOC_ASUM_ONLY : 0),
          (s.lean ? ITER_LEAN : 0) | (s.rebuild_follows ? ITER_REBUILD_FOLLOWS : 0) | (s.replay ? ITER_REPLAY : 0) |
              (lean_dense ? ITER_LEAN_DENSE : 0) | (s.idx32 ? ITER_IDX32 : 0) | (s.horizon << ITER_HORIZON_SHIFT)};
}

void launch_init(cvo_ctx* c, const LaunchGeom& g) {
  hipLaunchKernelGGL(k_update<true>, dim3(g.n_pairs), dim3(64), 0, g.stream, c->d_descs + g.p0, c->d_params,
                     c->d_status + 2 * g.p0, iteration_words({}).iter);
}

void launch_rebuild(cvo_ctx* c, const LaunchGeom& g) {
  const PairDesc* descs = c->d_descs + g.p0;
  const PairState* states = c->d_states + g.p0;
  hipLaunchKernelGGL(k_prep, dim3(g.npb, g.n_pairs), dim3(PREP_THREADS), 0, g.stream, descs, c->d_params, states);
  launch_scan(g.stream, g.T, dim3(g.gx, g.gy, g.n_pairs), descs, c->d_params, states, false);
  launch_list(g.stream, g.idx16, g.nbl, g.n_pairs, descs, c->d_params, states);
}

void launch_core(cvo_ctx* c, const LaunchGeom& g, const IterSlot& slot) {
  const PairDesc* descs = c->d_descs + g.p0;
  const int* st = c->d_status + 2 * g.p0;
  const IterWords w = iteration_words(slot);
  const bool dense = !slot.lean || slot.lean_dense;
  if (dense) launch_dense(g.stream, g.feat, g.wide, g.n_pairs, g.dense_blocks, descs, c->d_params, c->d_states + g.p0);
  launch_assoc(g.stream, g.idx16, g.feat, g.instr, g.nba, g.n_pairs, descs, c->d_params, c->d_states + g.p0, g.arena, w.assoc);
  if (g.verify) launch_verify(g.stream, g.feat, g.nbv, g.n_pairs, descs, c->d_params, st, w.assoc);
  if (dense)
    hipLaunchKernelGGL((k_coeff_dense<4>), dim3(g.n_pairs <= 4 ? std::min(2 * g.dense_blocks, (int)DENSE_BLOCKS_MAX) : g.dense_blocks, g.n_pairs), dim3(256), 0, g.stream, descs,
                       c->d_params, c->d_states + g.p0, g.n_pairs >= CVO_COEFF_DENSE_MULTI_FROM ? 8 : 1);
  launch_coeff(g.stream, g.instr, g.nba, g.csplit, g.n_pairs, descs, c->d_params, c->d_states + g.p0, g.arena, w.iter);
}

void launch_chunk(cvo_ctx* c, const LaunchGeom& g, const ChunkPlan& p) {
  if (p.every_iteration()) {
    const IterSlot slot{.lean = p.kind == ChunkKind::FullNoDense, .idx32 = !g.idx16, .rebuild_follows = true};
    for (int u = 0; u < p.U; u++) {
      launch_rebuild(c, g);
      launch_core(c, g, slot);
    }
    return;
  }
  for (int u = 0; u < p.U; u++) {
    if (u % p.period == 0) launch_rebuild(c, g);
    const bool last = (u % p.period == p.period - 1) || u == p.U - 1;
    launch_core(c, g, {.lean = true, .lean_dense = p.dense, .idx32 = !g.idx16, .rebuild_follows = last,
                       .horizon = std::min(p.period, g.horizon_cap)});
  }
}

GraphKey graph_key(const LaunchGeom& g, const ChunkPlan& plan) {
  return {plan, g.n_pairs, g.p0, g.T, g.gx, g.gy, g.npb, g.nbl, g.nba, g.csplit, g.dense_blocks, g.horizon_cap, g.feat,
          g.idx16, g.wide, g.instr, g.verify, g.arena};
}

template <typename Launches>
int capture_graph(cvo_ctx* ctx, CachedGraph& cg, const GraphKey& key, hipStream_t s, const LaunchGeom* flight, int n_flight,
                  const char* what, Launches&& launches) {
  if (cg.exec && cg.key == key) return CVO_OK;
  if (cg.exec) (void)hipGraphExecDestroy(cg.exec);
  cg.exec = nullptr;
  hipGraph_t gr = nullptr;
  HIP_TRY(ctx, hipStreamBeginCapture(s, hipStreamCaptureModeThreadLocal));
  launches();
  const hipError_t e_launch = hipGetLastError();
  hipError_t e = hipStreamEndCapture(s, &gr);
  if (e == hipSuccess && e_launch != hipSuccess) e = e_launch;
  if (e == hipSuccess) e = hipGraphInstantiate(&cg.exec, gr, nullptr, nullptr, 0);
  if (gr) (void)hipGraphDestroy(gr);
  if (e != hipSuccess) {
    cg.exec = nullptr;
    for (int q = 0; q < n_flight; q++) (void)hipStreamSynchronize(flight[q].stream);
    return fail(ctx, CVO_E_HIP, std::string(what) + ": " + hipGetErrorString(e));
  }
  cg.key = key;
  return CVO_OK;
}

}
```

unified_cvo_amd/csrc/cvo_options.h:

```cpp
#pragma once

namespace {

constexpr int MAX_STREAMS = 8;
constexpr float SKIN_MIN = 0.05f;

enum class CloudOrder { Device, Host, Virtual };

struct CtxOptions {
  float skin = 1.0f;
  float lean_skin = 0.5f;
  float horizon_margin = 0.3f;
  float skin_max = 0.35f;
  int shrink_align = 0;
  int lean_U = 8;
  bool no_lean = false, no_dense_regime = false, fixed_chunks = false;
  int first_U = 0;
  int first_chunks = 2;
  int streams = 0;
  int queue_admit = 4;
  bool no_sort = false, no_long_lists = false, no_onehot = false, ip_chain = false, keep_columns = false, no_speculate = false;
  CloudOrder order = CloudOrder::Device;
  int row_max = ASSOC_CAP16;
  int voxel_host = -1;
  int rgbd_host = -1;
  int stereo_host = -1;
  int lidar_host = -1;
  int nlm_host = -1;
  int fast_tile = 1;
  int voxel_prepass = 1;
  int verbose = 0;
  bool kernel_clock = false, phase_ticks = false, verify_lists = false, debug_no_motion_bound = false;
  int debug_drop_partial = 0;
};

enum class OptKind { Flag, Level, Integer, Real, Order };

struct OptionSpec {
  const char* name;
  OptKind kind;
  bool CtxOptions::*flag;
  int CtxOptions::*integer;
  float CtxOptions::*real;
  double lo, hi;
};
constexpr OptionSpec opt_flag(const char* name, bool CtxOptions::*m) { return {name, OptKind::Flag, m, nullptr, nullptr, 0, 0}; }
constexpr OptionSpec opt_int(const char* name, int CtxOptions::*m, double lo = INT_MIN, double hi = INT_MAX) { return {name, OptKind::Integer, nullptr, m, nullptr, lo, hi}; }
constexpr OptionSpec opt_real(const char* name, float CtxOptions::*m, double lo) { return {name, OptKind::Real, nullptr, nullptr, m, lo, HUGE_VAL}; }

constexpr OptionSpec kOptions[] = {
    opt_real("SKIN", &CtxOptions::skin, 0.0),
    opt_real("SKIN_MAX", &CtxOptions::skin_max, SKIN_MIN),
    opt_real("LEAN_SKIN", &CtxOptions::lean_skin, 0.1),
    opt_real("HORIZON_MARGIN", &CtxOptions::horizon_margin, 0.0),
    opt_int("SHRINK_ALIGN", &CtxOptions::shrink_align, 0),
    opt_int("LEAN_U", &CtxOptions::lean_U, 1),
    opt_flag("NO_LEAN", &CtxOptions::no_lean),
    opt_flag("NO_DENSE_REGIME", &CtxOptions::no_dense_regime),
    opt_flag("FIXED_CHUNKS", &CtxOptions::fixed_chunks),
    opt_int("FIRST_U", &CtxOptions::first_U, 1),
    opt_int("FIRST_CHUNKS", &CtxOptions::first_chunks, 0),
    opt_int("STREAMS", &CtxOptions::streams, 1, MAX_STREAMS),
    opt_int("QUEUE_ADMIT", &CtxOptions::queue_admit, 1),
    opt_flag("NO_SORT", &CtxOptions::no_sort),
    {"ORDER", OptKind::Order, nullptr, nullptr, nullptr, 0, 0},
    opt_flag("NO_LONG_LISTS", &CtxOptions::no_long_lists),
    opt_int("ROW_MAX", &CtxOptions::row_max, 1, ASSOC_CAP16),
    opt_flag("NO_ONEHOT", &CtxOptions::no_onehot),
    opt_flag("IP_CHAIN", &CtxOptions::ip_chain),
    opt_flag("KEEP_COLUMNS", &CtxOptions::keep_columns),
    opt_flag("NO_SPECULATE", &CtxOptions::no_speculate),
    opt_int("VOXEL_HOST", &CtxOptions::voxel_host, -1, 1),
    opt_int("VOXEL_PREPASS", &CtxOptions::voxel_prepass, 0, 1),
    opt_int("RGBD_HOST", &CtxOptions::rgbd_host, -1, 1),
    opt_int("STEREO_HOST", &CtxOptions::stereo_host, -1, 1),
    opt_int("LIDAR_HOST", &CtxOptions::lidar_host, -1, 1),
    opt_int("NLM_HOST", &CtxOptions::nlm_host, -1, 1),
    opt_int("FAST_TILE", &CtxOptions::fast_tile, 0, 1),
    {"VERBOSE", OptKind::Level, nullptr, &CtxOptions::verbose, nullptr, 0, 0},
    opt_flag("KERNEL_CLOCK", &CtxOptions::kernel_clock),
    opt_flag("PHASE_TICKS", &CtxOptions::phase_ticks),
    opt_flag("VERIFY_LISTS", &CtxOptions::verify_lists),
    opt_flag("DEBUG_NO_MOTION_BOUND", &CtxOptions::debug_no_motion_bound),
    opt_int("DEBUG_DROP_PARTIAL", &CtxOptions::debug_drop_partial),
};

inline void parse_option(CtxOptions& o, const OptionSpec& s, const char* text) {
  const CtxOptions def;
  char* end = nullptr;
  const bool on = text && !(std::strtol(text, &end, 10) == 0 && end != text);
  switch (s.kind) {
    case OptKind::Flag: o.*s.flag = on; break;
    case OptKind::Level: o.*s.integer = on ? std::max(1, atoi(text)) : 0; break;
    case OptKind::Integer: o.*s.integer = text ? std::max((int)s.lo, std::min(atoi(text), (int)s.hi)) : def.*s.integer; break;
    case OptKind::Real: o.*s.real = text ? std::max((float)s.lo, std::min((float)atof(text), (float)s.hi)) : def.*s.real; break;
    case OptKind::Order: o.order = !text ? def.order : (!std::strcmp(text, "host") ? CloudOrder::Host : (!std::strcmp(text, "virtual") ? CloudOrder::Virtual : CloudOrder::Device)); break;
  }
}

}
```

unified_cvo_amd/csrc/cvo_sched.hip:

```cpp
namespace {

struct QueueDims {
  int n_max, m_max, n_min;
};

struct BatchCall {
  const cvo_params_t* params;
  int n_pairs;
  const cvo_cloud *const *sources, *const *targets;
  const float* init_T;
  const cvo_align_opts_t* opts;
  CallMode mode;
  float mode_ell;
  const float* kernel_inv_and_cull;
  const QueueDims* qd;
};

DevParams make_dev_params(const cvo_ctx* ctx, const cvo_params_t& p, CallMode mode, const BatchCall* c = nullptr, const BatchSetup* S = nullptr) {
  const CtxOptions& o = ctx->opt;
  DevParams d{};
  d.mode = mode;
  d.sp_thres = p.sp_thres;
  d.sigma2 = p.sigma * p.sigma;
  d.c2 = p.c_ell * p.c_ell;
  d.c_sigma2 = p.c_sigma * p.c_sigma;
  d.s_ell = p.s_ell;
  d.s_sigma = p.s_sigma;
  d.c = p.c;
  d.d = p.d;
  const float s_sigma2 = p.s_sigma * p.s_sigma;
  d.log_geo = std::log(p.sp_thres / d.sigma2);
  d.d2_c_thres = 1.f;
  d.d2_s_thres = 1.f;
  if (p.is_using_intensity) d.d2_c_thres = (float)(-2.0 * d.c2 * (double)std::log(p.sp_thres / d.c_sigma2));
  if (p.is_using_semantics)
    d.d2_s_thres = (float)(-2.0 * d.s_ell * d.s_ell * (double)std::log(p.sp_thres / s_sigma2));
  d.ell_min = p.ell_min;
  d.ell_decay_rate = p.ell_decay_rate;
  d.ell_decay_start = p.ell_decay_start;
  d.max_iter = p.MAX_ITER;
  d.eps = p.eps;
  d.eps_2 = p.eps_2;
  d.min_step = p.min_step;
  d.max_step = p.max_step;
  d.K_max = p.nearest_neighbors_max;
  d.window = p.indicator_window_size;
  d.stable_thr = p.indicator_stable_threshold;
  d.use_geo = p.is_using_geometry != 0;
  d.use_col = p.is_using_intensity != 0;
  d.use_sem = p.is_using_semantics != 0;
  d.use_range_ell = p.is_using_range_ell != 0;
  d.use_geotype = p.is_using_geometric_type != 0;
  {
    auto mid = [](float v) { const float a = std::fabs(v); return std::isfinite(v) && a >= 0x1p-20f && a <= 0x1p20f; };
    d.fast_div_cd = mid(p.c) && mid(p.d) ? 1 : 0;
  }
  d.skin_frac = o.skin;
  d.lean_skin = o.lean_skin;
  d.dense_regime = o.no_dense_regime ? 0 : 1;
  d.skin_blend = 0.25f;
  d.skin_min = SKIN_MIN;
  d.skin_max = o.skin_max;
  d.horizon_margin = o.horizon_margin;
#ifndef CVO_REBUILD_SHRINK
#define CVO_REBUILD_SHRINK 0.9f
#endif
  d.rebuild_shrink = CVO_REBUILD_SHRINK;
  d.phase_ticks = o.phase_ticks;
  d.kernel_clock = o.kernel_clock;
  d.verify_lists = o.verify_lists;
  d.debug_no_motion_bound = o.debug_no_motion_bound;
  d.debug_drop_partial = o.debug_drop_partial;
  if (!c) return d;

  const cvo_align_opts_t* opts = c->opts;
  const int trace_cap = (opts && opts->trace) ? opts->trace_capacity : 0;
  if (mode == CALL_NONISO) {
    for (int q = 0; q < 9; q++) d.kinv[q] = c->kernel_inv_and_cull[q];
    d.d2_cull = c->kernel_inv_and_cull[9];
    d.s_ell_sq = p.s_ell * p.s_ell;
    d.use_geotype = 0;
    if (p.is_using_semantics) d.d2_s_thres = (float)(-2.0 * d.s_ell_sq * (double)std::log(p.sp_thres / s_sigma2));
  }
  choose_scan_config(ctx, (c->n_pairs + S->G - 1) / S->G, S->d.NG, S->d.Mpad, &d.T, &d.groups_per_block);
  d.long_lists = S->long_lists ? 1 : 0;
  d.row_max_cap = o.row_max;
  d.row_max_busy = c->n_pairs <= 4 ? 8 : (c->n_pairs <= 16 ? 24 : (int)ASSOC_CAP16);
  d.lean_U = o.lean_U;
  d.calm_U = 4;
  d.lean_U2 = 2;
  if (d.lean_U2 >= d.lean_U) d.lean_U2 = 0;
  d.shrink_align = o.shrink_align;
  if (opts && opts->max_iterations > 0) d.max_iter = std::min(d.max_iter, opts->max_iterations);
  if (opts && opts->kernel_clock) d.kernel_clock = 1;
  d.trace_capacity = trace_cap;
  d.keep_columns = (mode != CALL_ALIGN || trace_cap > 0 || d.verify_lists || p.is_exporting_association || o.keep_columns) ? 1 : 0;
  d.no_speculate = o.no_speculate;
  d.trace_dense = opts ? opts->trace_dense : 0;
  d.trace_every = opts ? opts->trace_every : 0;
  return d;
}

struct GroupRange {
  int p0, p1;
};
inline GroupRange group_bounds(int n, int G, int g) { return {(int)((long)n * g / G), (int)((long)n * (g + 1) / G)}; }
inline int group_of(int n, int G, int p) {
  int g = 0;
  while (g + 1 < G && group_bounds(n, G, g + 1).p0 <= p) g++;
  return g;
}

void fill_pair(cvo_ctx* ctx, const BatchSetup* S, const cvo_params_t* params, const cvo_align_opts_t* opts, CallMode mode, float mode_ell,
               int n_slots, int p, const cvo_cloud* X, const cvo_cloud* Y, const float* Tm, unsigned long long serial, int max_iter) {
  const int trace_cap = (opts && opts->trace) ? opts->trace_capacity : 0;
  const int Kmax = params->nearest_neighbors_max;
  PairDesc& D = ctx->h_descs[p];
  std::memset(&D, 0, sizeof(D));
  place_regions(D, (uintptr_t)ctx->arena + S->slot_bytes * (size_t)p, S->N, S->d, Kmax, trace_cap, S->long_lists);
  D.N = X->n;
  D.M = Y->n;
  D.call_serial = serial;
  D.max_iter = max_iter;
  D.Mpad = S->d.Mpad;
  D.nchunks = S->d.nchunks;
  D.nslices = S->d.Mpad / (64 * S->geom.T);
  D.rbw = (int)align_up((size_t)(S->d.Mpad / (64 * S->geom.T) + 31) / 32, 4);
  D.nblk_assoc = S->d.nblk_assoc;
  D.csplit = coeff_split(X->n);
  D.nblk_coeff = S->d.nblk_assoc * D.csplit;
  D.NG = (X->n + ROWS_PER_GROUP - 1) / ROWS_PER_GROUP;
  D.NGpad = S->d.NGpad;
  D.ymax = Y->rmax;
  D.sqrt_nm = std::sqrt((double)X->n * (double)Y->n);
  D.cx = X->cx;
  D.cy = X->cy;
  D.cz = X->cz;
  D.x4 = X->x4;
  D.xs4 = X->xs4;
  D.xfeat = X->feat;
  D.xlabel = X->label;
  D.xgeo = X->geo;
  D.xorder = X->order;
  D.y4 = Y->x4;
  D.ys4 = Y->xs4;
  D.yfeat = Y->feat;
  D.ylabel = Y->label;
  D.ygeo = Y->geo;
  D.xlid = X->lid;
  D.ylid = Y->lid;
  D.yorder = Y->order;
  D.yinv = Y->inv;
  D.st = ctx->d_states + p;
  {
    const auto [p0, p1] = group_bounds(n_slots, S->G, group_of(n_slots, S->G, p));
    D.status_out = ctx->d_status + 2 * p0 + (p - p0);
    D.want_out = ctx->d_status + 2 * p0 + (p1 - p0) + (p - p0);
    D.status_host = ctx->h_status[0] + 2 * p0 + (p - p0);
    D.want_host = ctx->h_status[0] + 2 * p0 + (p1 - p0) + (p - p0);
  }
  D.asum_host = reinterpret_cast<double*>(ctx->h_status[1]) + p;

  PairState& st = ctx->h_states[p];
  std::memset(&st, 0, sizeof(st));
  for (int i = 0; i < 3; i++) {
    for (int j = 0; j < 3; j++) st.R[3 * i + j] = Tm[4 * j + i];
    st.T[i] = Tm[12 + i];
  }
  st.ell = mode == CALL_ALIGN ? params->ell_init : mode_ell;
  st.K = Kmax;
  if (mode == CALL_ALIGN && opts && opts->override_state) {
    st.ell = opts->ell0;
    st.K = opts->K0;
  }
  st.K_last = 0;
}

unsigned long long next_call_serial() {
  static std::atomic<unsigned long long> g_call_serial{1};
  return g_call_serial.fetch_add(1);
}

int check_call(cvo_ctx* ctx, const cvo_params_t* params, int n_pairs, const cvo_cloud* const* sources, const cvo_cloud* const* targets,
               const cvo_align_opts_t* opts, CallMode mode, float mode_ell, const QueueDims* qd, int* N_out, int* M_out) {
  if (!ctx) return CVO_E_INVALID;
  if (ctx->queue_open && !qd) return fail(ctx, CVO_E_INVALID, "a batch queue is open on this context (cvo_batch_close it first)");
  if (!params || n_pairs <= 0 || (!qd && (!sources || !targets))) return fail(ctx, CVO_E_INVALID, "null argument");
  if (params->is_using_kdtree)
    return fail(ctx, CVO_E_UNSUPPORTED, "is_using_kdtree=1 is out of scope (SURVEY.md section 2, row 11)");
  if (params->nearest_neighbors_max <= 0) return fail(ctx, CVO_E_INVALID, "nearest_neighbors_max must be > 0");
  if (params->indicator_window_size + 1 >= IND_CAP || params->indicator_window_size < 0)
    return fail(ctx, CVO_E_INVALID, "indicator_window_size out of range");
  {
    auto ok_scale = [](float v) { return std::isfinite(v) && v >= 1e-30f && v <= 1e15f; };
    const float ell0 = mode == CALL_ALIGN ? ((opts && opts->override_state) ? opts->ell0 : params->ell_init) : mode_ell;
    if (!ok_scale(ell0) || (mode == CALL_ALIGN && !ok_scale(params->ell_min)))
      return fail(ctx, CVO_E_INVALID, "lengthscale outside [1e-30, 1e15] (ell_init / ell_min / the ell of the call)");
    if (params->is_using_intensity && !ok_scale(params->c_ell)) return fail(ctx, CVO_E_INVALID, "c_ell outside [1e-30, 1e15]");
    if (params->is_using_semantics && !ok_scale(params->s_ell)) return fail(ctx, CVO_E_INVALID, "s_ell outside [1e-30, 1e15]");
  }
  if (mode == CALL_ALIGN && opts && opts->override_state) {
    if (opts->K0 < 1 || opts->K0 > params->nearest_neighbors_max)
      return fail(ctx, CVO_E_INVALID, "cvo_align_opts_t.K0 must lie in [1, nearest_neighbors_max]");
    if (!(opts->ell0 > 0.f) || !std::isfinite(opts->ell0))
      return fail(ctx, CVO_E_INVALID, "cvo_align_opts_t.ell0 must be finite and > 0");
  }
  int N = qd ? qd->n_max : 0, M = qd ? qd->m_max : 0;
  if (qd && (qd->n_max <= 0 || qd->m_max <= 0 || qd->n_min <= 0 || qd->n_min > qd->n_max))
    return fail(ctx, CVO_E_INVALID, "cvo_batch_open: bad cloud sizes");
  for (int p = 0; p < n_pairs && !qd; p++) {
    if (!sources[p] || !targets[p]) return fail(ctx, CVO_E_INVALID, "null cloud");
    if (sources[p]->ctx != ctx || targets[p]->ctx != ctx)
      return fail(ctx, CVO_E_INVALID, "cloud belongs to another context");
    if (sources[p]->n <= 0 || targets[p]->n <= 0) return fail(ctx, CVO_E_INVALID, "empty cloud in batch");
    if (!(sources[p]->rmax <= 1e15f) || !(targets[p]->rmax <= 1e15f))
      return fail(ctx, CVO_E_INVALID, "cloud with non-finite or astronomically large coordinates (|p| > 1e15)");
    N = std::max(N, sources[p]->n);
    M = std::max(M, targets[p]->n);
  }
  HIP_TRY(ctx, hipSetDevice(ctx->device));
  (void)hipGetLastError();
  {
    const bool nf = params->is_using_intensity != 0, nl = params->is_using_semantics != 0,
               ng = params->is_using_geometric_type != 0 && mode != CALL_NONISO;
    if ((nf || nl || ng) && !qd)
      for (int p = 0; p < n_pairs; p++) {
        int rc0 = ensure_attributes(ctx, sources[p], nf, nl, ng);
        if (rc0 == CVO_OK) rc0 = ensure_attributes(ctx, targets[p], nf, nl, ng);
        if (rc0 != CVO_OK) return rc0;
      }
  }
  *N_out = N;
  *M_out = M;
  return CVO_OK;
}

int plan_batch(cvo_ctx* ctx, const BatchCall& c, int N, int M, BatchSetup* S, DevParams* dp) {
  const CtxOptions& o = ctx->opt;
  const int n_pairs = c.n_pairs;
  const int trace_cap = (c.opts && c.opts->trace) ? c.opts->trace_capacity : 0;
  const int Kmax = c.params->nearest_neighbors_max;
  S->N = N;
  S->M = M;
  if (M >= (1 << 23)) return fail(ctx, CVO_E_INVALID, "target clouds are limited to 8388607 points");
  if ((unsigned long long)N * (unsigned long long)std::max(Kmax, 1) >= (1ull << 32))
    return fail(ctx, CVO_E_INVALID, "source rows x nearest_neighbors_max must stay below 2^32");
  S->d = make_dims(N, M);
  S->long_lists = M <= 65535 && !o.no_long_lists;
  auto slot_bytes = [&](bool long_lists) { PairDesc unused{}; return place_regions(unused, 0, N, S->d, Kmax, trace_cap, long_lists); };
  S->slot_bytes = slot_bytes(S->long_lists);
  {
    size_t free_b = 0, total_b = 0;
    size_t need = S->slot_bytes * (size_t)n_pairs;
    const bool tight = need > ctx->arena_bytes && hipMemGetInfo(&free_b, &total_b) == hipSuccess && need > free_b + ctx->arena_bytes;
    if (tight && S->long_lists) {
      S->long_lists = false;
      S->slot_bytes = slot_bytes(false);
      need = S->slot_bytes * (size_t)n_pairs;
      if (o.verbose) fprintf(stderr, "[cvo] workspace: long lists dropped to fit device memory\n");
    }
    if (need > ctx->arena_bytes && hipMemGetInfo(&free_b, &total_b) == hipSuccess && need > free_b + ctx->arena_bytes) {
      char msg[320];
      snprintf(msg, sizeof msg,
               "workspace of %d pair(s) of %d x %d points needs %.1f GiB (candidate bitmap N*M/8 = %.1f GiB per pair, ELL "
               "%.1f GiB per pair; the long lists of overflow rows have already been dropped) but %.1f GiB of device memory are "
               "free: split the batch or the clouds",
               n_pairs, N, M, need / 1073741824.0, (double)N * S->d.Mpad / 8.0 / 1073741824.0,
               (double)S->d.Npad * Kmax * 20.0 / 1073741824.0, (free_b + ctx->arena_bytes) / 1073741824.0);
      return fail(ctx, CVO_E_NOMEM, msg);
    }
  }
  S->G = std::min(n_pairs, o.streams ? o.streams : (n_pairs >= 32 ? 4 : (n_pairs >= 8 ? 2 : 1)));
  if ((n_pairs + S->G - 1) / S->G > LAUNCH_PAIRS_MAX || S->d.nblk_assoc > LAUNCH_NBLK_MAX) {
    char msg[160];
    snprintf(msg, sizeof msg, "batch too large for one call: at most %d pairs per stream and %d source points per cloud",
             LAUNCH_PAIRS_MAX, LAUNCH_NBLK_MAX * ASSOC_THREADS);
    return fail(ctx, CVO_E_INVALID, msg);
  }
  *dp = make_dev_params(ctx, *c.params, c.mode, &c, S);
  const int T = dp->T, gpb = dp->groups_per_block;

  LaunchGeom& geom = S->geom;
  geom.n_pairs = n_pairs;
  geom.p0 = 0;
  geom.stream = ctx->stream;
  geom.T = T;
  geom.gx = (S->d.Mpad / (64 * T) + 3) / 4;
  geom.gy = ((int)align_up((size_t)S->d.NG, 64) + gpb - 1) / gpb;
  geom.nba = S->d.nblk_assoc;
  geom.nbl = (N + LIST_THREADS - 1) / LIST_THREADS;
  geom.nbv = std::min((N + 3) / 4, 2048);
  geom.wide = dense_wide(N, n_pairs);
  geom.dense_blocks = dense_blocks_for(N, n_pairs);
  geom.arena.stride256 = (unsigned)(S->slot_bytes >> 8);
  geom.arena.Npad = S->d.Npad;
  geom.csplit = c.qd ? coeff_split(c.qd->n_min) : 1;
  for (int p = 0; p < n_pairs && !c.qd; p++) geom.csplit = std::max(geom.csplit, coeff_split(c.sources[p]->n));
  geom.npb = S->d.Mpad / PREP_THREADS + (S->d.NGpad * ROWS_PER_GROUP + PREP_THREADS - 1) / PREP_THREADS;
  geom.idx16 = M < 65536;
  {
    bool all_hot = !c.qd && !o.no_onehot;
    for (int p = 0; p < n_pairs && all_hot; p++) all_hot = c.sources[p]->lid != nullptr && c.targets[p]->lid != nullptr;
    geom.feat = call_feat(*dp, all_hot);
  }
  geom.instr = dp->kernel_clock || dp->phase_ticks;
  geom.verify = dp->verify_lists != 0;
  geom.horizon_cap = std::max(1, dp->lean_U);
  return CVO_OK;
}

int commit_batch(cvo_ctx* ctx, const BatchCall& c, BatchSetup* S, const DevParams& dp) {
  const int n_pairs = c.n_pairs;
  if (const int rc = ensure_workspace(ctx, n_pairs, S->slot_bytes); rc != CVO_OK) return rc;
  S->geom.arena.base = ctx->arena;
  ctx->h_descs.resize(n_pairs);
  ctx->h_states.resize(n_pairs);
  if (!c.qd) {
    const unsigned long long serial = next_call_serial();
    for (int p = 0; p < n_pairs; p++)
      fill_pair(ctx, S, c.params, c.opts, c.mode, c.mode_ell, n_pairs, p, c.sources[p], c.targets[p], c.init_T + 16 * (size_t)p, serial, dp.max_iter);
  } else {
    for (int p = 0; p < n_pairs; p++) {
      std::memset(&ctx->h_descs[p], 0, sizeof(PairDesc));
      std::memset(&ctx->h_states[p], 0, sizeof(PairState));
      ctx->h_states[p].status = 1;
    }
  }
  std::memcpy(ctx->h_ctl, &dp, sizeof(DevParams));
  std::memset(ctx->h_ctl + ctx->ctl_off_status, c.qd ? 1 : 0, sizeof(int) * 2 * (size_t)ctx->cap_pairs);
  std::memcpy(ctx->h_ctl + ctx->ctl_off_descs, ctx->h_descs.data(), sizeof(PairDesc) * (size_t)n_pairs);
  std::memcpy(ctx->h_ctl + ctx->ctl_off_states, ctx->h_states.data(), sizeof(PairState) * (size_t)n_pairs);
  std::memset(ctx->h_status[0], c.qd ? 1 : 0, sizeof(int) * 2 * (size_t)ctx->cap_pairs);
  {
    const size_t upto = ctx->ctl_off_states + sizeof(PairState) * (size_t)n_pairs;
    if ((size_t)n_pairs * 2 >= (size_t)ctx->cap_pairs) {
      HIP_TRY(ctx, hipMemcpyAsync(ctx->d_ctl, ctx->h_ctl, upto, hipMemcpyHostToDevice, ctx->stream));
    } else {
      HIP_TRY(ctx, hipMemcpyAsync(ctx->d_ctl, ctx->h_ctl, ctx->ctl_off_descs + sizeof(PairDesc) * (size_t)n_pairs, hipMemcpyHostToDevice, ctx->stream));
      HIP_TRY(ctx, hipMemcpyAsync(ctx->d_ctl + ctx->ctl_off_states, ctx->h_ctl + ctx->ctl_off_states, sizeof(PairState) * (size_t)n_pairs,
                                  hipMemcpyHostToDevice, ctx->stream));
    }
  }
  if (!c.qd) ctx->last_xorder = c.sources[0]->h_order;
  ctx->last_pairs = n_pairs;
  ctx->last = *S;
  ctx->last_params = dp;
  return CVO_OK;
}

int setup_batch(cvo_ctx* ctx, const BatchCall& c, BatchSetup* S, DevParams* dp) {
  int N = 0, M = 0;
  int rc = check_call(ctx, c.params, c.n_pairs, c.sources, c.targets, c.opts, c.mode, c.mode_ell, c.qd, &N, &M);
  if (rc == CVO_OK) rc = plan_batch(ctx, c, N, M, S, dp);
  if (rc == CVO_OK) rc = commit_batch(ctx, c, S, *dp);
  return rc;
}

struct LoopCfg {
  int U, U_late, lean_U, lean_U2;
  bool instr;
  bool allow_lean, start_nodense, allow_calm;
};

LoopCfg loop_cfg(const cvo_ctx* ctx, const BatchSetup& S, const DevParams& dp, int U, int U_late) {
  const bool allow_lean = !ctx->opt.no_lean;
  return {U, U_late, std::max(1, std::min(dp.lean_U, U)), std::max(0, std::min(dp.lean_U2, U)), S.geom.instr,
          allow_lean, allow_lean && S.N > 4096, dp.calm_U > 0};
}

LaunchGeom group_geom(const cvo_ctx* ctx, const BatchSetup& S, int n, int g) {
  const auto [p0, p1] = group_bounds(n, S.G, g);
  LaunchGeom geom = S.geom;
  geom.p0 = p0;
  geom.n_pairs = p1 - p0;
  geom.arena.base += S.slot_bytes * (size_t)p0;
  geom.stream = ctx->gstream[g];
  geom.wide = dense_wide(S.N, geom.n_pairs);
  return geom;
}

struct GroupWant {
  int level = -1;
  bool dense = false;
  void add(int w) {
    const WantWord d = want_decode(w);
    level = std::max(level, d.level);
    dense = dense || d.dense;
  }
};

inline ChunkPlan first_chunk(const LoopCfg& c) { return {c.start_nodense ? ChunkKind::FullNoDense : ChunkKind::Full}; }

ChunkPlan choose_chunk(const LoopCfg& c, GroupWant w) {
  if (w.level == 1 && c.lean_U2 <= 0) w.level = 2;
  if (!c.allow_lean) return {ChunkKind::Full};
  if (w.level >= 2) return w.dense ? ChunkPlan{ChunkKind::Full} : first_chunk(c);
  return {w.level == 1 ? ChunkKind::ShortLean : (w.level == 0 || !c.allow_calm ? ChunkKind::Lean : ChunkKind::Calm), w.dense};
}

ChunkPlan sized_chunk(const LoopCfg& c, ChunkPlan p, int U) {
  p.U = U;
  p.period = p.kind == ChunkKind::Lean ? c.lean_U : (p.kind == ChunkKind::ShortLean ? c.lean_U2 : (p.kind == ChunkKind::Calm ? U : 0));
  return p;
}

inline int graph_slot(const LoopCfg& c, const ChunkPlan& p) {
  const int kd = (int)p.kind + (p.dense ? 3 : 0);
  return kd + (c.instr ? 8 : 0) + 16 * (p.U == c.U ? 0 : (p.U == c.U_late ? 1 : 2));
}

int chunk_graph(cvo_ctx* ctx, const LaunchGeom* geom, int G, const LoopCfg& cfg, int g, const ChunkPlan& p, hipGraphExec_t* exec) {
  CachedGraph& cg = ctx->graphs[g][graph_slot(cfg, p)];
  const int rc = capture_graph(ctx, cg, graph_key(geom[g], p), geom[g].stream, geom, G, "graph capture / instantiate",
                               [&] { launch_chunk(ctx, geom[g], p); });
  *exec = cg.exec;
  return rc;
}

cvo_align_info_t info_from_state(const PairState& st, double seconds) {
  return {st.status ? st.iterations : st.k, st.ret, st.ell, st.K, seconds};
}

}

extern "C" {

int cvo_align_batch(cvo_ctx* ctx, const cvo_params_t* params, int n_pairs, const cvo_cloud* const* sources,
                    const cvo_cloud* const* targets, const float* init_T, float* out_T, cvo_align_info_t* infos,
                    const cvo_align_opts_t* opts) {
  if (!ctx) return CVO_E_INVALID;
  if (!init_T || !out_T) return fail(ctx, CVO_E_INVALID, "null transform pointer");
  BatchSetup S;
  DevParams dp;
  const auto t_host0 = std::chrono::steady_clock::now();
  int rc = setup_batch(ctx, {params, n_pairs, sources, targets, init_T, opts, CALL_ALIGN, 0.f, nullptr, nullptr}, &S, &dp);
  if (rc != CVO_OK) return rc;
  const auto t_host1 = std::chrono::steady_clock::now();

  const int max_iter = dp.max_iter, verbose = ctx->opt.verbose;
  int U = (opts && opts->iters_per_launch > 0) ? opts->iters_per_launch : 16;
  U = std::max(1, std::min(U, std::max(1, max_iter)));
  const bool adaptive_chunks = !(opts && opts->iters_per_launch > 0) && !ctx->opt.fixed_chunks && max_iter >= 512;
  const int U_late = adaptive_chunks ? 2 * U : U;
  const int n_early_chunks = adaptive_chunks ? 256 / U : 0;
  const int U_first = !adaptive_chunks ? U : (ctx->opt.first_U ? std::min(ctx->opt.first_U, U) : std::max(1, U / 4));
  const int n_first_chunks = U_first != U ? ctx->opt.first_chunks : 0;
  const int graph_mode = opts ? opts->use_graph : 0;
  const bool use_graph = graph_mode != 1;

  const int G = S.G;
  LaunchGeom geom[cvo_ctx::MAX_GROUPS];
  for (int g = 0; g < G; g++) geom[g] = group_geom(ctx, S, n_pairs, g);

  HIP_TRY(ctx, hipEventRecord(ctx->ev_start, ctx->stream));
  HIP_TRY(ctx, hipEventRecord(ctx->ev_fork, ctx->stream));
  for (int g = 0; g < G; g++) {
    if (g) HIP_TRY(ctx, hipStreamWaitEvent(geom[g].stream, ctx->ev_fork, 0));
    launch_init(ctx, geom[g]);
  }
  HIP_TRY(ctx, hipGetLastError());

  if (max_iter > 0) {
    const LoopCfg cfg = loop_cfg(ctx, S, dp, U, U_late);
    const int n_chunks = (max_iter + U_first - 1) / U_first;
    const int chunk_cap = 4 * n_chunks + 16;
    ChunkPlan next[cvo_ctx::MAX_GROUPS];
    for (int g = 0; g < G; g++) next[g] = first_chunk(cfg);
    bool all_done = false;
    int ch = 0;
    int n_lean_launch = 0, n_full_launch = 0;
    double t_launch = 0, t_wait = 0;
    auto now = [] { return std::chrono::steady_clock::now(); };
    auto ms_since = [&](std::chrono::steady_clock::time_point t) { return std::chrono::duration<double, std::milli>(now() - t).count(); };
    for (; ch < chunk_cap && !all_done; ch++) {
      const int slot = ch & 1;
      const int Uc = ch < n_first_chunks ? U_first : (ch < n_early_chunks + n_first_chunks ? U : U_late);
      if (verbose >= 3) {
        fprintf(stderr, "[cvo] chunk %d (%d iterations): graphs", ch, Uc);
        for (int g = 0; g < G; g++) fprintf(stderr, " %s%s", kChunkNames[(int)next[g].kind], next[g].dense ? "+dense" : "");
        fprintf(stderr, "\n");
      }
      for (int g = 0; g < G; g++) {
        const ChunkPlan p = sized_chunk(cfg, next[g], Uc);
        (p.every_iteration() ? n_full_launch : n_lean_launch)++;
        if (use_graph) {
          hipGraphExec_t exec = nullptr;
          rc = chunk_graph(ctx, geom, G, cfg, g, p, &exec);
          if (rc != CVO_OK) return rc;
          const auto tl = now();
          HIP_TRY(ctx, hipGraphLaunch(exec, geom[g].stream));
          t_launch += ms_since(tl);
        } else {
          launch_chunk(ctx, geom[g], p);
          HIP_TRY(ctx, hipGetLastError());
        }
        HIP_TRY(ctx, hipEventRecord(ctx->ev_chk[slot][g], geom[g].stream));
      }
      if (ch >= 1) {
        const int ws = (ch - 1) & 1;
        const auto tw = now();
        for (int g = 0; g < G; g++) HIP_TRY(ctx, hipEventSynchronize(ctx->ev_chk[ws][g]));
        t_wait += ms_since(tw);
        all_done = true;
        for (int g = 0; g < G; g++) {
          const volatile int* hs = ctx->h_status[0] + 2 * geom[g].p0;
          const int ng = geom[g].n_pairs;
          for (int q = 0; q < ng; q++) all_done = all_done && hs[q] != 0;
          GroupWant want;
          for (int q = 0; q < ng; q++)
            if (hs[q] == 0) want.add(hs[ng + q]);
          next[g] = choose_chunk(cfg, want);
          if (verbose >= 2 && ch < 12) {
            int nw = 0;
            for (int q = 0; q < ng; q++) nw += hs[ng + q] != 0;
            fprintf(stderr, "[cvo] after chunk %d group %d: %d of %d pairs ask for the full graph\n", ch - 1, g, nw, geom[g].n_pairs);
          }
        }
      }
    }
    ctx->last_chunks = ch;
    if (verbose) fprintf(stderr, "[cvo] host loop: %.2f ms in hipGraphLaunch, %.2f ms waiting for the device\n", t_launch, t_wait);
    ctx->last_lean_launches = n_lean_launch;
    ctx->last_full_launches = n_full_launch;
    if (!all_done) {
      for (int g = 0; g < G; g++) HIP_TRY(ctx, hipStreamSynchronize(geom[g].stream));
      bool fin = true;
      for (int g = 0; g < G; g++)
        for (int q = 0; q < geom[g].n_pairs; q++) fin = fin && ((volatile int*)ctx->h_status[0])[2 * geom[g].p0 + q] != 0;
      if (!fin && ch >= chunk_cap) return fail(ctx, CVO_E_HIP, "cvo_align_batch: optimiser loop did not terminate");
    }
  }
  for (int g = 1; g < G; g++) {
    HIP_TRY(ctx, hipEventRecord(ctx->ev_join[g], geom[g].stream));
    HIP_TRY(ctx, hipStreamWaitEvent(ctx->stream, ctx->ev_join[g], 0));
  }
  HIP_TRY(ctx, hipEventRecord(ctx->ev_stop, ctx->stream));
  HIP_TRY(ctx, hipMemcpyAsync(ctx->h_states.data(), ctx->d_states, sizeof(PairState) * (size_t)n_pairs,
                              hipMemcpyDeviceToHost, ctx->stream));
  HIP_TRY(ctx, hipStreamSynchronize(ctx->stream));
  const auto t_host2 = std::chrono::steady_clock::now();
  float ms = 0;
  HIP_TRY(ctx, hipEventElapsedTime(&ms, ctx->ev_start, ctx->ev_stop));
  if (verbose)
    fprintf(stderr, "[cvo] host: setup %.2f ms, enqueue + wait %.2f ms\n",
            std::chrono::duration<double, std::milli>(t_host1 - t_host0).count(),
            std::chrono::duration<double, std::milli>(t_host2 - t_host1).count());
  for (int p = 0; p < n_pairs; p++) {
    const PairState& st = ctx->h_states[p];
    if (st.sync_err)
      return fail(ctx, CVO_E_HIP, st.sync_err == 1 ? "a block partial of k_assoc never arrived at the flow gate (tagged-partial poll limit)"
                                                    : "a block partial of k_coeff never arrived at the update (tagged-partial poll limit)");
    if (st.verify_err) {
      char msg[256];
      snprintf(msg, sizeof msg,
               "CVO_VERIFY_LISTS: pair %d, iteration %d, row position %d: the list-derived row differs from the literal "
               "scan (%s)", p, st.verify_k, st.verify_pos,
               st.verify_what == 1 ? "nonzero count" : (st.verify_what == 2 ? "column" : "value"));
      return fail(ctx, CVO_E_VERIFY, msg);
    }
  }
  if (verbose) {
    long builds = 0, stalls = 0, its = 0, adopted = 0;
    for (int p = 0; p < n_pairs; p++) {
      adopted += ctx->h_states[p].n_adopted;
      builds += ctx->h_states[p].n_builds;
      stalls += ctx->h_states[p].n_stalls;
      its += ctx->h_states[p].status ? ctx->h_states[p].iterations : ctx->h_states[p].k;
    }
    if (verbose >= 2)
      for (int p = 0; p < std::min(n_pairs, 4); p++)
        fprintf(stderr, "[cvo]   pair %d: k %d, list allowance used %.3f, per iteration %.5f, want %d, builds %d, ell %.4f (built at %.4f)\n", p,
                ctx->h_states[p].k, ctx->h_states[p].last_used, ctx->h_states[p].last_rate, ctx->h_states[p].want_full,
                ctx->h_states[p].n_builds, ctx->h_states[p].ell, ctx->h_states[p].ell_build);
    fprintf(stderr, "[cvo] %d pairs, %d groups: %d chunks (%d full + %d lean group launches), iterations %ld (%ld with the speculative update adopted), list builds %ld, waits %ld, %.3f ms\n",
            n_pairs, G, ctx->last_chunks, ctx->last_full_launches, ctx->last_lean_launches, its, adopted, builds, stalls, ms);
  }
  for (int p = 0; p < n_pairs; p++) {
    const PairState& st = ctx->h_states[p];
    std::memcpy(out_T + 16 * (size_t)p, st.out_T, sizeof(float) * 16);
    if (infos) infos[p] = info_from_state(st, (double)ms * 1e-3);
    if (opts && opts->trace && opts->trace_capacity > 0) {
      const int nt = std::min(st.n_trace, opts->trace_capacity);
      if (nt > 0)
        HIP_TRY(ctx, hipMemcpy(opts->trace + (size_t)p * opts->trace_capacity, ctx->h_descs[p].trace,
                               sizeof(cvo_trace_t) * (size_t)nt, hipMemcpyDeviceToHost));
      if (opts->n_trace) opts->n_trace[p] = nt;
    }
  }
  return CVO_OK;
}

int cvo_align_ex(cvo_ctx* ctx, const cvo_params_t* params, const cvo_cloud* source, const cvo_cloud* target,
                 const float init_T[16], float out_T[16], cvo_align_info_t* info, const cvo_align_opts_t* opts) {
  if (!ctx) return CVO_E_INVALID;
  if (!source || !target) return fail(ctx, CVO_E_INVALID, "null cloud");
  if (info) std::memset(info, 0, sizeof(*info));
  if (source->n == 0 || target->n == 0) return 0;
  const cvo_cloud* src[1] = {source};
  const cvo_cloud* tgt[1] = {target};
  cvo_align_info_t local;
  int rc = cvo_align_batch(ctx, params, 1, src, tgt, init_T, out_T, &local, opts);
  if (rc != CVO_OK) return rc;
  if (info) *info = local;
  return local.ret;
}

int cvo_align(cvo_ctx* ctx, const cvo_params_t* params, const cvo_cloud* source, const cvo_cloud* target,
              const float init_T[16], float out_T[16], cvo_align_info_t* info) {
  return cvo_align_ex(ctx, params, source, target, init_T, out_T, info, nullptr);
}

int cvo_batch_poses_to_device(cvo_ctx* ctx, void* dst_device, int n_pairs) {
  if (!ctx || !dst_device || n_pairs <= 0 || n_pairs > ctx->last_pairs)
    return fail(ctx, CVO_E_INVALID, "cvo_batch_poses_to_device: bad argument");
  std::vector<float> poses(16 * (size_t)n_pairs);
  for (int p = 0; p < n_pairs; p++) std::memcpy(&poses[16 * (size_t)p], ctx->h_states[p].out_T, sizeof(float) * 16);
  HIP_TRY(ctx, hipMemcpyAsync(dst_device, poses.data(), sizeof(float) * poses.size(), hipMemcpyHostToDevice,
                              ctx->stream));
  HIP_TRY(ctx, hipStreamSynchronize(ctx->stream));
  return CVO_OK;
}

}
```

unified_cvo_amd/csrc/cvo_update.h:

```cpp
#pragma once
#include "cvo_wave.h"
#include "cvo_pair_math.h"

namespace cvo_dev {

constexpr int HOT_DWORDS = (int)(offsetof(PairState, sq) / 4);
constexpr int SHADOW_WORDS = 128;
static_assert(HOT_DWORDS + 4 <= SHADOW_WORDS, "the shadow holds the scalar state and four words of UpdOut");
struct UpdateShared {
  double c[4];
  unsigned long long n[4];
  unsigned hot[HOT_DWORDS];
  unsigned ext[SHADOW_WORDS - HOT_DWORDS];
};

struct UpdDesc {
  PairState* st;
  const unsigned long long* coef_part;
  const unsigned long long* flow_part;
  const unsigned long long* cnt_part;
  cvo_trace_t* trace;
  int* status_out;
  int* want_out;
  int* status_host;
// ... 252 lines not shown
      const bool dense_rows = c_ovf > 0 || c_dense != 0;
      st->row_max = (!INIT && P.long_lists && !c_dense && 16 * c_ovf > D.N) ? P.row_max_busy : ASSOC_CAP16;
      if (P.long_lists && P.row_max_cap > 0) st->row_max = min(st->row_max, P.row_max_cap);
      int want_full = 2;
      float s = 0.f;
      if (INIT) st->skin_scale = 1.f;
      else if (c_scan > 0 && !c_dense) st->skin_scale = fmaxf(0.5f * st->skin_scale, 1.f / 64.f);
      else st->skin_scale = fminf(1.f, 1.1f * st->skin_scale);
      if (!INIT && P.mode == CALL_ALIGN && P.use_geo && radius > 0.f && P.skin_frac > 0.f && !c_dense) {
        const float rel = step_move * frcp(radius);
        s = st->skin_scale * P.skin_frac * fminf(fmaxf(1.5f * fsqrt(rel), P.skin_min), P.skin_max);
        const float s_lean = fmaxf(s, P.lean_skin * (float)P.lean_U * rel);
        const float s_lean2 = fmaxf(s, P.lean_skin * (float)P.lean_U2 * rel);
        if (s_lean <= 0.5f && c_scan == 0) {
          s = s_lean;
          want_full = 0;
        } else if (P.lean_U2 > 0 && s_lean2 <= 0.5f && c_scan == 0) {
          s = s_lean2;
          want_full = 1;
        } else if (!(s >= 2.f * rel)) {
          s = 0.f;
        }
      }
      if (!(s == s)) s = 0.f;
      {
        const float life = step_move > 0.f ? s * radius * frcp(step_move * (1.f + P.skin_blend)) : 0.f;
        const float bl = P.skin_blend;
        st->skin_rot = life * ((1.f - bl) * rot_1 + bl * step_move * frcp(fmaxf(ymax, 1e-20f)));
        st->skin_tr = life * ((1.f - bl) * tr_1 + bl * step_move);
        if (!(st->skin_rot == st->skin_rot) || !(st->skin_tr == st->skin_tr)) st->skin_rot = st->skin_tr = 0.f;
      }
      if (c_dense) want_full = -1;
      want_full = want_encode(want_full, dense_rows);
      st->want_full = want_full;
      if (!dry) out.post_want(D, spec, want_full);
      st->n_builds = INIT ? 1 : st->n_builds + 1;
      st->rebuild = 1;
    } else if (c_scan == 0 && !c_dense) {
      const float c = fminf(P.lean_skin, 1.3f);
      int want = want_level(c_want);
      if (used + c * (float)P.lean_U * rate <= 1.f)
        want = 0;
      else if (P.lean_U2 > 0 && used + c * (float)P.lean_U2 * rate <= 1.f)
        want = min(want, 1);
      if (want == 0 && P.calm_U > 0 && used + c * (float)P.calm_U * rate <= 1.f) want = -1;
      want = want_encode(want, c_ovf > 0);
      if (want != c_want) {
        st->want_full = want;
        if (!dry) out.post_want(D, spec, want);
      }
    }
  }
  CVO_UPD_STAMP(4);
  for (int q = 0; q < 9; q++) st->Rinv[q] = Ri[q];
  for (int q = 0; q < 3; q++) st->Tinv[q] = Ti[q];
  if (done || INIT || P.mode != CALL_ALIGN) {
    for (int i = 0; i < 3; i++) {
      for (int j = 0; j < 3; j++) st->out_T[4 * j + i] = Ri[3 * i + j];
      st->out_T[12 + i] = Ti[i];
    }
    st->out_T[3] = st->out_T[7] = st->out_T[11] = 0;
    st->out_T[15] = 1;
  }
  if (clk0 && !dry) {
    if (st->clk_last_assoc) {
      st->clk_sum[0] += st->clk_last_assoc;
      st->clk_n[0]++;
      st->clk_last_assoc = 0;
    }
    const unsigned dt_coeff = pair_clock_ticks(clk0);
    if (dt_coeff) {
      st->clk_sum[1] += dt_coeff;
      st->clk_n[1]++;
    }
  }
  if (done && !dry) {
    st->status = 1;
    out.post_done(D, spec);
  }
}

__device__ __forceinline__ bool step_is_clamp(const DevParams& P, float step) {
  return step > 0.f && (step == P.min_step || step == P.max_step);
}

__device__ __forceinline__ void reduce_counts(const unsigned long long* cnt_part, int nba, int tid, unsigned long long* s_n) {
  const CVO_GLOBAL unsigned* cnt32 = as_global(reinterpret_cast<const unsigned*>(cnt_part));
  const int c = tid >> 4, bl = tid & 15;
  auto addsat = [](unsigned a, unsigned b) { const unsigned r = a + b; return r < a ? 0xffffffffu : r; };
  unsigned q = 0;
  for (int b0 = bl; b0 < nba; b0 += 128) {
    unsigned v[8];
#pragma unroll
    for (int u = 0; u < 8; u++) {
      const int b = b0 + 16 * u;
      v[u] = b < nba ? ld_g<false>(cnt32 + ((size_t)b * 4 + c) * 2) : 0u;
    }
#pragma unroll
    for (int u = 0; u < 8; u++) q = (c == 1) ? max(q, v[u]) : addsat(q, v[u]);
  }
  auto meet = [&](unsigned o) { q = (c == 1) ? max(q, o) : addsat(q, o); };
  meet((unsigned)dpp_i32<DPP_XOR1>((int)q));
  meet((unsigned)dpp_i32<DPP_XOR2>((int)q));
  meet((unsigned)dpp_i32<DPP_HALF_MIRROR>((int)q));
  meet((unsigned)dpp_i32<DPP_MIRROR>((int)q));
#pragma unroll
  for (int cc = 0; cc < 4; cc++) {
    const unsigned long long qv = (unsigned long long)(unsigned)__builtin_amdgcn_readlane((int)q, 16 * cc);
    if (tid == 0) s_n[cc] = qv;
  }
}

__device__ __forceinline__ void update_speculate(const PairDesc* __restrict__ Dp, PairState* const gst, const DevParams& P, int flags,
                                                 UpdateShared& U, unsigned long long call_serial) {
  const int tid = threadIdx.x;
  const UpdDesc D = load_upd_desc(Dp);
  unsigned* const s_hot = U.hot;
  {
    const unsigned h0 = reinterpret_cast<const unsigned*>(gst)[tid];
    const unsigned h1 = (tid + 64 < HOT_DWORDS) ? reinterpret_cast<const unsigned*>(gst)[tid + 64] : 0u;
    s_hot[tid] = h0;
    if (tid + 64 < HOT_DWORDS) s_hot[tid + 64] = h1;
  }
  __builtin_amdgcn_wave_barrier();
  PairState* const st = reinterpret_cast<PairState*>(s_hot);
  const float pred = st->step;
  if (!step_is_clamp(P, pred)) return;
  {
    const int xe = __float_as_int(gst->xi[46]), xk = __float_as_int(gst->xi[47]);
    if (xe != st->epoch || xk != st->k || st->status != 0) return;
  }
  const unsigned tag = partial_tag(call_serial, 0x80000000u | (unsigned)st->epoch);
  reduce_counts(D.cnt_part, Dp->nblk_assoc, tid, U.n);
  __builtin_amdgcn_wave_barrier();
  if (tid == 0) {
    const float e_front = gst->eq[st->e_head], s_front = gst->sq[st->s_head];
    const XiMats* xm = reinterpret_cast<const XiMats*>(gst->xi);
    const float twist[6] = {xm->omega[0], xm->omega[1], xm->omega[2], xm->v[0], xm->v[1], xm->v[2]};
    UpdOut out;
    update_advance<false>(D, P, flags, st, gst->sq, gst->eq, nullptr, U.n, pred, twist, e_front, s_front, 0ull, true, out);
    U.ext[0] = (unsigned)out.done;
    U.ext[1] = (unsigned)out.want_write;
    U.ext[2] = (unsigned)out.want_val;
    U.ext[3] = __float_as_uint(pred);
    for (int q = 4; q < SHADOW_WORDS - HOT_DWORDS; q++) U.ext[q] = 0u;
  }
  __builtin_amdgcn_wave_barrier();
  const unsigned long long t = (unsigned long long)tag << 32;
  const unsigned w0 = s_hot[tid], w1 = (tid + 64 < HOT_DWORDS) ? s_hot[tid + 64] : U.ext[tid + 64 - HOT_DWORDS];
  __hip_atomic_store(D.shadow + tid, t | w0, __ATOMIC_RELAXED, __HIP_MEMORY_SCOPE_AGENT);
  __hip_atomic_store(D.shadow + 64 + tid, t | w1, __ATOMIC_RELAXED, __HIP_MEMORY_SCOPE_AGENT);
}

template <bool INIT, bool COH>
__device__ __forceinline__ void update_body(const UpdDesc& D, const DevParams& P, int flags,
                                            int n_flow_parts, UpdateShared& U, const float* twist,
                                            const unsigned* preloaded_hot, unsigned long long clk0 = 0ull, unsigned tag = 0u,
                                            bool may_adopt = false) {
  PairState* const gst = D.st;
  const bool dry = (flags & ITER_REPLAY) != 0;
  double* const s_c = U.c;
  unsigned long long* const s_n = U.n;
  unsigned* const s_hot = U.hot;
  const int tid = threadIdx.x;
  const bool act = tid < 64;
  CVO_UPD_STAMP(0);

  static_assert(HOT_DWORDS <= 128, "two dwords per lane of the first wave cover the scalar state");
  if (act && preloaded_hot) {
    s_hot[tid] = preloaded_hot[0];
    if (tid + 64 < HOT_DWORDS) s_hot[tid + 64] = preloaded_hot[1];
  } else if (act) {
    for (int q = tid; q < HOT_DWORDS; q += 64) s_hot[q] = reinterpret_cast<const unsigned*>(gst)[q];
  }
  PairState* const st = reinterpret_cast<PairState*>(s_hot);
  float* const sq = gst->sq;
  float* const eq = gst->eq;
  bool spec_try = false;
  float pred = 0.f;
  unsigned long long g0 = 0ull, g1 = 0ull;
  if (!INIT && COH && may_adopt && !dry && P.mode == CALL_ALIGN && P.trace_capacity == 0) {
    __builtin_amdgcn_wave_barrier();
    pred = st->step;
    spec_try = step_is_clamp(P, pred);
    if (spec_try) {
      g0 = ld_g<true>(as_global(D.shadow) + tid);
      g1 = ld_g<true>(as_global(D.shadow) + 64 + tid);
    }
  }
  if (!INIT && act) {
    const int nba = n_flow_parts, nbc = D.nblk_coeff;
    const int c = tid >> 4, bl = tid & 15;
    double s = 0;
    const CVO_GLOBAL unsigned* cnt32 = as_global(reinterpret_cast<const unsigned*>(D.cnt_part));
    const CVO_GLOBAL unsigned long long* coef_part = as_global(D.coef_part);
    unsigned vq[8];
#pragma unroll
    for (int u = 0; u < 8; u++) {
      const int b = bl + 16 * u;
      vq[u] = b < nba ? ld_g<false>(cnt32 + ((size_t)b * 4 + c) * 2) : 0u;
    }
    if (P.mode == CALL_ALIGN) {
      for (int b0 = bl; b0 < nbc; b0 += 64) {
        TaggedF64 v[4];
        for (int polls = 0;; polls++) {
          bool ok = true;
#pragma unroll
          for (int u = 0; u < 4; u++) {
            const int b = min(b0 + 16 * u, nbc - 1);
            v[u] = ld_tagged<COH>(coef_part + (size_t)b * COEF_GRANULES + 2 * c);
          }
#pragma unroll
          for (int u = 0; u < 4; u++) ok = ok && (!COH || v[u].carries(tag));
          if (__ballot(!ok) == 0ull) break;
          if (polls > PARTIAL_POLL_LIMIT) {
            if (tid == 0) st->sync_err = 2;
            break;
          }
          __builtin_amdgcn_s_sleep(2);
        }
#pragma unroll
        for (int u = 0; u < 4; u++) s += (b0 + 16 * u < nbc) ? v[u].value() : 0.0;
      }
    } else if (c == 0) {
      for (int b = bl; b < nba; b += 16) s += ld_tagged<false>(as_global(D.flow_part) + (size_t)b * FLOW_GRANULES + 12).value();
    }
    auto addsat = [](unsigned a, unsigned b) { const unsigned r = a + b; return r < a ? 0xffffffffu : r; };
    unsigned q = 0;
#pragma unroll
    for (int u = 0; u < 8; u++) q = (c == 1) ? max(q, vq[u]) : addsat(q, vq[u]);
    for (int b0 = bl + 128; b0 < nba; b0 += 128) {
      unsigned v[8];
#pragma unroll
      for (int u = 0; u < 8; u++) {
        const int b = b0 + 16 * u;
        v[u] = b < nba ? ld_g<false>(cnt32 + ((size_t)b * 4 + c) * 2) : 0u;
      }
#pragma unroll
      for (int u = 0; u < 8; u++) q = (c == 1) ? max(q, v[u]) : addsat(q, v[u]);
    }
    s += dpp_f64<DPP_XOR1>(s);
    s += dpp_f64<DPP_XOR2>(s);
    s += dpp_f64<DPP_HALF_MIRROR>(s);
    s += dpp_f64<DPP_MIRROR>(s);
    {
      auto meet = [&](unsigned o) { q = (c == 1) ? max(q, o) : addsat(q, o); };
      meet((unsigned)dpp_i32<DPP_XOR1>((int)q));
      meet((unsigned)dpp_i32<DPP_XOR2>((int)q));
      meet((unsigned)dpp_i32<DPP_HALF_MIRROR>((int)q));
      meet((unsigned)dpp_i32<DPP_MIRROR>((int)q));
    }
#pragma unroll
    for (int cc = 0; cc < 4; cc++) {
      const double sv = lane_f64(s, 16 * cc);
      const unsigned long long qv = (unsigned long long)(unsigned)__builtin_amdgcn_readlane((int)q, 16 * cc);
      if (tid == 0) {
        s_c[cc] = sv;
        s_n[cc] = qv;
      }
    }
  }
  __syncthreads();
  float e_front = 0.f, s_front = 0.f;
  if (!INIT && tid == 0) {
    e_front = eq[st->e_head];
    s_front = sq[st->s_head];
  }
  CVO_UPD_STAMP(1);
  float step_w = 0.f;
  if (!INIT && act && P.mode == CALL_ALIGN) step_w = select_step<true>(s_c[0], s_c[1], s_c[2], s_c[3], P.min_step, P.max_step);
  CVO_UPD_STAMP(2);
  UpdOut out;
  bool adopt = false;
  if (spec_try && __float_as_uint(step_w) == __float_as_uint(pred) && s_hot[offsetof(PairState, sync_err) / 4] == 0u) {
    for (int polls = 0;; polls++) {
      const bool ok = (unsigned)(g0 >> 32) == tag && (unsigned)(g1 >> 32) == tag;
      if (__ballot(!ok) == 0ull) {
        adopt = true;
        break;
      }
      if (polls >= 3) break;
      __builtin_amdgcn_s_sleep(8);
      g0 = ld_g<true>(as_global(D.shadow) + tid);
      g1 = ld_g<true>(as_global(D.shadow) + 64 + tid);
    }
  }
  if (adopt) {
    s_hot[tid] = (unsigned)g0;
    if (tid + 64 < HOT_DWORDS)
      s_hot[tid + 64] = (unsigned)g1;
    else
      U.ext[tid + 64 - HOT_DWORDS] = (unsigned)g1;
    __builtin_amdgcn_wave_barrier();
    if (tid == 0) {
      st->B = s_c[0];
      st->C = s_c[1];
      st->D = s_c[2];
      st->E = s_c[3];
      st->n_adopted++;
      if (U.ext[1]) {
        *D.want_out = (int)U.ext[2];
        *D.want_host = (int)U.ext[2];
      }
      if (U.ext[0]) {
        *D.status_out = 1;
        *D.status_host = 1;
      }
    }
  } else if (tid == 0) {
    update_advance<INIT>(D, P, flags, st, sq, eq, s_c, s_n, step_w, twist, e_front, s_front, clk0, false, out);
  }
  CVO_UPD_STAMP(5);
  __syncthreads();
  if (act && !dry)
    for (int q = tid; q < HOT_DWORDS; q += 64) reinterpret_cast<unsigned*>(gst)[q] = s_hot[q];
  CVO_UPD_STAMP(6);
}

template <bool INIT>
__global__ __launch_bounds__(64) void k_update(const PairDesc* __restrict__ descs, const DevParams* __restrict__ Pp,
                                               const int* __restrict__ status, int flags) {
  if (!INIT && status[blockIdx.x] != 0) return;
  const PairDesc* __restrict__ D = descs + blockIdx.x;
  if (!INIT && slot_waits(flags, ITER_LEAN, ITER_LEAN_DENSE, D->st)) return;
  if (INIT && threadIdx.x == 0) {
    *D->status_out = 0;
    *D->status_host = 0;
    *D->gate = 0;
    *D->gate_flow = 0;
    *D->done = 0;
    *D->tile_count = 0ull;
  }
  const DevParams P = *Pp;
  __shared__ UpdateShared U;
  update_body<INIT, false>(load_upd_desc(D), P, flags, D->nblk_assoc, U, nullptr, nullptr);
}

}
```

unified_cvo_amd/csrc/cvo_wave.h:

```cpp
#pragma once
#include "cvo_device.h"

namespace cvo_dev {

constexpr int DPP_XOR1 = 0xB1, DPP_XOR2 = 0x4E, DPP_HALF_MIRROR = 0x141, DPP_MIRROR = 0x140;
template <int CTRL>
__device__ __forceinline__ int dpp_i32(int v) {
  return __builtin_amdgcn_update_dpp(0, v, CTRL, 0xf, 0xf, true);
}
template <int CTRL>
__device__ __forceinline__ double dpp_f64(double v) {
  const int lo = dpp_i32<CTRL>(__double2loint(v)), hi = dpp_i32<CTRL>(__double2hiint(v));
  return __hiloint2double(hi, lo);
}
__device__ __forceinline__ double xor16_sum(double v) {
  const auto lo = __builtin_amdgcn_permlane16_swap((unsigned)__double2loint(v), (unsigned)__double2loint(v), false, false);
  const auto hi = __builtin_amdgcn_permlane16_swap((unsigned)__double2hiint(v), (unsigned)__double2hiint(v), false, false);
  return __hiloint2double((int)hi[0], (int)lo[0]) + __hiloint2double((int)hi[1], (int)lo[1]);
}
__device__ __forceinline__ double xor32_sum(double v) {
  const auto lo = __builtin_amdgcn_permlane32_swap((unsigned)__double2loint(v), (unsigned)__double2loint(v), false, false);
  const auto hi = __builtin_amdgcn_permlane32_swap((unsigned)__double2hiint(v), (unsigned)__double2hiint(v), false, false);
  return __hiloint2double((int)hi[0], (int)lo[0]) + __hiloint2double((int)hi[1], (int)lo[1]);
}
__device__ __forceinline__ double lane_f64(double v, int l) {
  return __hiloint2double(__builtin_amdgcn_readlane(__double2hiint(v), l), __builtin_amdgcn_readlane(__double2loint(v), l));
}
template <int CTRL>
__device__ __forceinline__ unsigned long long dpp_u64(unsigned long long v) {
  const unsigned lo = (unsigned)dpp_i32<CTRL>((int)(unsigned)v), hi = (unsigned)dpp_i32<CTRL>((int)(unsigned)(v >> 32));
  return ((unsigned long long)hi << 32) | lo;
}
__device__ __forceinline__ unsigned long long lane_u64(unsigned long long v, int l) {
  return ((unsigned long long)(unsigned)__builtin_amdgcn_readlane((int)(unsigned)(v >> 32), l) << 32) |
         (unsigned)__builtin_amdgcn_readlane((int)(unsigned)v, l);
}
__device__ __forceinline__ double wave_sum(double v) {
  v += dpp_f64<DPP_XOR1>(v);
  v += dpp_f64<DPP_XOR2>(v);
  v += dpp_f64<DPP_HALF_MIRROR>(v);
  v += dpp_f64<DPP_MIRROR>(v);
  return (lane_f64(v, 0) + lane_f64(v, 16)) + (lane_f64(v, 32) + lane_f64(v, 48));
}
__device__ __forceinline__ unsigned wave_sum_u32(unsigned v) {
  v += (unsigned)dpp_i32<DPP_XOR1>((int)v);
  v += (unsigned)dpp_i32<DPP_XOR2>((int)v);
  v += (unsigned)dpp_i32<DPP_HALF_MIRROR>((int)v);
  v += (unsigned)dpp_i32<DPP_MIRROR>((int)v);
  return (unsigned)(__builtin_amdgcn_readlane((int)v, 0) + __builtin_amdgcn_readlane((int)v, 16) +
                    __builtin_amdgcn_readlane((int)v, 32) + __builtin_amdgcn_readlane((int)v, 48));
}
__device__ __forceinline__ unsigned wave_max_u32(unsigned v) {
  v = max(v, (unsigned)dpp_i32<DPP_XOR1>((int)v));
  v = max(v, (unsigned)dpp_i32<DPP_XOR2>((int)v));
  v = max(v, (unsigned)dpp_i32<DPP_HALF_MIRROR>((int)v));
  v = max(v, (unsigned)dpp_i32<DPP_MIRROR>((int)v));
  return max(max((unsigned)__builtin_amdgcn_readlane((int)v, 0), (unsigned)__builtin_amdgcn_readlane((int)v, 16)),
             max((unsigned)__builtin_amdgcn_readlane((int)v, 32), (unsigned)__builtin_amdgcn_readlane((int)v, 48)));
}
template <bool MAX>
__device__ __forceinline__ float wave_minmax_f32(float v) {
  auto meet = [](float a, int ob) {
    const float o = __builtin_bit_cast(float, ob);
    return MAX ? fmaxf(a, o) : fminf(a, o);
  };
  v = meet(v, dpp_i32<DPP_XOR1>(__builtin_bit_cast(int, v)));
  v = meet(v, dpp_i32<DPP_XOR2>(__builtin_bit_cast(int, v)));
  v = meet(v, dpp_i32<DPP_HALF_MIRROR>(__builtin_bit_cast(int, v)));
  v = meet(v, dpp_i32<DPP_MIRROR>(__builtin_bit_cast(int, v)));
  const int iv = __builtin_bit_cast(int, v);
  float m = meet(__builtin_bit_cast(float, __builtin_amdgcn_readlane(iv, 0)), __builtin_amdgcn_readlane(iv, 16));
  m = meet(m, __builtin_amdgcn_readlane(iv, 32));
  return meet(m, __builtin_amdgcn_readlane(iv, 48));
}
__device__ __forceinline__ int wave_prefix_incl_i32(int v, int lane) {
  v += __builtin_amdgcn_update_dpp(0, v, 0x111, 0xf, 0xf, true);
  v += __builtin_amdgcn_update_dpp(0, v, 0x112, 0xf, 0xf, true);
  v += __builtin_amdgcn_update_dpp(0, v, 0x114, 0xf, 0xf, true);
  v += __builtin_amdgcn_update_dpp(0, v, 0x118, 0xf, 0xf, true);
  const int t0 = __builtin_amdgcn_readlane(v, 15), t1 = __builtin_amdgcn_readlane(v, 31), t2 = __builtin_amdgcn_readlane(v, 47);
  const int quarter = lane >> 4;
  return v + (quarter > 0 ? t0 : 0) + (quarter > 1 ? t1 : 0) + (quarter > 2 ? t2 : 0);
}
__device__ __forceinline__ float wave_max_f32(float v) {
#pragma unroll
  for (int o = 32; o > 0; o >>= 1) v = fmaxf(v, __shfl_down(v, o));
  return v;
}

struct PairBlock {
  int pair, bx;
};
__device__ __forceinline__ int udiv_small(int n, int d) {
  if (n >= (1 << 22)) return n / d;
  int q = (int)((float)n * __builtin_amdgcn_rcpf((float)d));
  const int r = n - q * d;
  q += r >= d ? 1 : 0;
  q -= r < 0 ? 1 : 0;
  return q;
}
__device__ __forceinline__ bool pair_block(int nblk, int n_pairs, PairBlock& pb) {
  const int b = (int)blockIdx.x;
  const int slot = b >> 3;
  const int grp = udiv_small(slot, nblk);
  pb.pair = grp * 8 + (b & 7);
  pb.bx = slot - grp * nblk;
  return pb.pair < n_pairs;
}

#define CVO_GLOBAL __attribute__((address_space(1)))
#define CVO_CONST __attribute__((address_space(4)))
typedef float f32x4 __attribute__((ext_vector_type(4)));
typedef float f32x2 __attribute__((ext_vector_type(2)));
#define CVO_LDS __attribute__((address_space(3)))
#ifdef CVO_ELL8
typedef f32x2 ell_vec_t;
__device__ __forceinline__ ell_vec_t ell_to_vec(const EllEntry& e) { return ell_vec_t{e.a, __int_as_float(e.p)}; }
#else
typedef f32x4 ell_vec_t;
__device__ __forceinline__ ell_vec_t ell_to_vec(const EllEntry& e) { return ell_vec_t{e.a, e.yx, e.yy, e.yz}; }
#endif
__device__ __forceinline__ float4 ldg_f4(const CVO_GLOBAL f32x4* p) {
  const f32x4 v = *p;
  return make_float4(v.x, v.y, v.z, v.w);
}
typedef float f32x3 __attribute__((ext_vector_type(3)));
__device__ __forceinline__ float4 ldg_xyz(const CVO_GLOBAL f32x4* p) {
  const f32x3 v = *reinterpret_cast<const CVO_GLOBAL f32x3*>(p);
  return make_float4(v.x, v.y, v.z, 0.f);
}
template <typename T>
__device__ __forceinline__ const CVO_GLOBAL T* as_global(const T* p) {
  return (const CVO_GLOBAL T*)p;
}
template <bool COH, typename T>
__device__ __forceinline__ T ld_g(const CVO_GLOBAL T* p) {
  if (COH) return __hip_atomic_load(p, __ATOMIC_RELAXED, __HIP_MEMORY_SCOPE_AGENT);
  return *p;
}
template <bool COH, typename T>
__device__ __forceinline__ void st_x(T* p, T v) {
  if (COH)
    __hip_atomic_store(p, v, __ATOMIC_RELAXED, __HIP_MEMORY_SCOPE_AGENT);
  else
    *p = v;
}
template <bool COH, typename T>
__device__ __forceinline__ T ld_x(const T* p) {
  if (COH) return __hip_atomic_load(p, __ATOMIC_RELAXED, __HIP_MEMORY_SCOPE_AGENT);
  return *p;
}

__device__ __forceinline__ unsigned partial_tag(unsigned long long serial, unsigned n) {
  unsigned h = (unsigned)serial * 0x9E3779B1u + (unsigned)(serial >> 32) * 0x7FEB352Du + (n + 1u) * 0x85EBCA6Bu;
  h ^= h >> 15;
  h *= 0x2C1B3C6Du;
  h ^= h >> 12;
  return h;
}
__device__ __forceinline__ void st_tagged(unsigned long long* g, double v, unsigned tag) {
  const unsigned long long t = (unsigned long long)tag << 32;
  __hip_atomic_store(g, t | (unsigned long long)(unsigned)__double2loint(v), __ATOMIC_RELAXED, __HIP_MEMORY_SCOPE_AGENT);
  __hip_atomic_store(g + 1, t | (unsigned long long)(unsigned)__double2hiint(v), __ATOMIC_RELAXED, __HIP_MEMORY_SCOPE_AGENT);
}
struct TaggedF64 {
  unsigned long long lo, hi;
  __device__ __forceinline__ bool carries(unsigned tag) const { return (unsigned)(lo >> 32) == tag && (unsigned)(hi >> 32) == tag; }
  __device__ __forceinline__ double value() const { return __hiloint2double((int)(unsigned)hi, (int)(unsigned)lo); }
};
template <bool COH>
__device__ __forceinline__ TaggedF64 ld_tagged(const CVO_GLOBAL unsigned long long* g) {
  TaggedF64 t;
  t.lo = ld_g<COH>(g);
  t.hi = ld_g<COH>(g + 1);
  return t;
}
constexpr int FLOW_GRANULES = 16, COEF_GRANULES = 8;
constexpr int PARTIAL_POLL_LIMIT = 400000;

}
```

Measured before the change: 1175.

## Fuse association, coefficient and update into one speculative per-iteration kernel

Adds a k_iter kernel that runs the association, coefficient and pose-update phases of one CVO iteration in a single launch for lean, non-dense chunks. It predicts the next iteration's state from the clamped step, publishes it through a tagged shadow buffer, and falls back to the full update when the prediction misses. Association blocks publish their tagged counts so the predictor can reduce them without a separate pass. The aim is to remove per-iteration launch and graph-node overhead, at the cost of cross-block polling, extra graph slots, and wasted work on mispredictions.

```diff
diff --git a/include/cvo_hip_debug.h b/include/cvo_hip_debug.h
--- a/include/cvo_hip_debug.h
+++ b/include/cvo_hip_debug.h
@@ -17,6 +17,7 @@
                           unsigned long long* candidate_evaluations);
 int cvo_debug_row_classes(cvo_ctx* ctx, int pair, int* overflow_rows, int* scanned_rows, int* dense_regime);
 int cvo_debug_speculation(cvo_ctx* ctx, int pair, int* adopted, int* iterations);
+int cvo_debug_fused(cvo_ctx* ctx, int pair, int* one_launch, int* primed_only, int* mispredicted);
 int cvo_debug_last_candidates(cvo_ctx* ctx, unsigned long long* out);
 int cvo_debug_scalar_math(cvo_ctx* ctx, int op, int n, const double* in, double* out);
 int cvo_debug_verified_rows(cvo_ctx* ctx, unsigned long long* rows);
diff --git a/unified_cvo_amd/_capi.py b/unified_cvo_amd/_capi.py
--- a/unified_cvo_amd/_capi.py
+++ b/unified_cvo_amd/_capi.py
@@ -247,7 +247,7 @@
     "cvo_align", "cvo_align_ex", "cvo_align_batch", "cvo_batch_poses_to_device", "cvo_inner_product",
     "cvo_function_angle", "cvo_association", "cvo_association_non_isotropic", "cvo_cloud_transformed", "cvo_edge_kernel_matrix", "cvo_debug_last_ell", "cvo_debug_time_scan", "cvo_debug_time_kernels",
     "cvo_debug_kernel_clock",
-    "cvo_debug_last_candidates", "cvo_debug_list_builds", "cvo_debug_row_classes", "cvo_debug_speculation", "cvo_debug_scan_stats", "cvo_debug_last_geometry", "cvo_version",
+    "cvo_debug_last_candidates", "cvo_debug_list_builds", "cvo_debug_row_classes", "cvo_debug_speculation", "cvo_debug_fused", "cvo_debug_scan_stats", "cvo_debug_last_geometry", "cvo_version",
     "cvo_align_association", "cvo_debug_scalar_math", "cvo_debug_verified_rows", "cvo_debug_device_memory", "cvo_cloud_upload_many",
     "cvo_ctx_set_option", "cvo_ctx_advice", "cvo_debug_cloud_order",
     "cvo_process_hint_hw_queues", "cvo_shutdown",
@@ -330,6 +330,7 @@
     L.cvo_debug_list_builds.argtypes = [vp, C.POINTER(C.c_ulonglong), C.POINTER(C.c_ulonglong), C.POINTER(C.c_ulonglong)]
     L.cvo_debug_row_classes.argtypes = [vp, C.c_int, C.POINTER(C.c_int), C.POINTER(C.c_int), C.POINTER(C.c_int)]
     L.cvo_debug_speculation.argtypes = [vp, C.c_int, C.POINTER(C.c_int), C.POINTER(C.c_int)]
+    L.cvo_debug_fused.argtypes = [vp, C.c_int, C.POINTER(C.c_int), C.POINTER(C.c_int), C.POINTER(C.c_int)]
     L.cvo_debug_last_geometry.argtypes = [vp, C.POINTER(C.c_int), C.POINTER(C.c_int)]
     L.cvo_debug_scan_stats.argtypes = [vp, C.POINTER(C.c_ulonglong), C.POINTER(C.c_int), C.POINTER(C.c_int)]
     L.cvo_align_association.argtypes = [vp, ip, C.POINTER(C.c_int), C.POINTER(C.c_int), fp, C.c_size_t,
diff --git a/unified_cvo_amd/api.py b/unified_cvo_amd/api.py
--- a/unified_cvo_amd/api.py
+++ b/unified_cvo_amd/api.py
@@ -1143,6 +1143,11 @@
         self._check(self.L.cvo_debug_speculation(self.ctx, pair, C.byref(a), C.byref(it)))
         return a.value, it.value
 
+    def debug_fused(self, pair=0):
+        a, b, c = C.c_int(), C.c_int(), C.c_int()
+        self._check(self.L.cvo_debug_fused(self.ctx, pair, C.byref(a), C.byref(b), C.byref(c)))
+        return a.value, b.value, c.value
+
     def advice(self):
         return self.L.cvo_ctx_advice(self.ctx).decode()
 
diff --git a/unified_cvo_amd/csrc/cvo_debug.hip b/unified_cvo_amd/csrc/cvo_debug.hip
--- a/unified_cvo_amd/csrc/cvo_debug.hip
+++ b/unified_cvo_amd/csrc/cvo_debug.hip
@@ -199,6 +199,15 @@
   return CVO_OK;
 }
 
+int cvo_debug_fused(cvo_ctx* ctx, int pair, int* one_launch, int* primed_only, int* mispredicted) {
+  if (!ctx || pair < 0 || pair >= ctx->last_pairs) return fail(ctx, CVO_E_INVALID, "cvo_debug_fused: bad argument");
+  const PairState& st = ctx->h_states[pair];
+  if (one_launch) *one_launch = st.n_fused;
+  if (primed_only) *primed_only = st.n_primed;
+  if (mispredicted) *mispredicted = st.n_mispred;
+  return CVO_OK;
+}
+
 int cvo_debug_scan_stats(cvo_ctx* ctx, unsigned long long* tiles, int* rows_per_tile, int* targets_per_tile) {
   if (!ctx || !tiles || ctx->last_pairs < 1) return fail(ctx, CVO_E_INVALID, "cvo_debug_scan_stats: bad argument");
   HIP_TRY(ctx, hipSetDevice(ctx->device));
diff --git a/unified_cvo_amd/csrc/cvo_device.h b/unified_cvo_amd/csrc/cvo_device.h
--- a/unified_cvo_amd/csrc/cvo_device.h
+++ b/unified_cvo_amd/csrc/cvo_device.h
@@ -59,6 +59,7 @@
   int debug_drop_partial;
   int debug_no_motion_bound;
   int no_speculate;
+  int debug_fuse_mispredict;
 };
 
 struct PairState {
@@ -108,6 +109,7 @@
   unsigned long long clk_start[2];
   int verify_err, verify_k, verify_pos, verify_what;
   unsigned long long verify_rows;
+  int n_fused, n_primed, n_mispred, n_fuse_match;
 };
 
 #ifdef CVO_ELL8
diff --git a/unified_cvo_amd/csrc/cvo_internal.h b/unified_cvo_amd/csrc/cvo_internal.h
--- a/unified_cvo_amd/csrc/cvo_internal.h
+++ b/unified_cvo_amd/csrc/cvo_internal.h
@@ -52,12 +52,14 @@
 
 enum class ChunkKind { Full, FullNoDense, Lean, ShortLean, Calm };
 static const char* const kChunkNames[] = {"full", "full-nodense", "lean", "short", "calm"};
+static const char* const kChunkFused = "+fused";
 
 struct ChunkPlan {
   ChunkKind kind = ChunkKind::Full;
   bool dense = false;
   int U = 0;
   int period = 0;
+  bool fused = false;
   bool every_iteration() const { return kind == ChunkKind::Full || kind == ChunkKind::FullNoDense; }
 };
 
@@ -73,7 +75,7 @@
   bool idx16 = false, wide = false, instr = false, verify = false;
   ArenaArg arena{};
   auto fields() const {
-    return std::tie(plan.kind, plan.dense, plan.U, plan.period, n_pairs, p0, T, gx, gy, npb, nbl, nba, csplit, dense_blocks,
+    return std::tie(plan.kind, plan.dense, plan.U, plan.period, plan.fused, n_pairs, p0, T, gx, gy, npb, nbl, nba, csplit, dense_blocks,
                     horizon_cap, feat, idx16, wide, instr, verify, arena.base, arena.stride256, arena.Npad);
   }
   bool operator==(const GraphKey& o) const { return fields() == o.fields(); }
@@ -190,7 +192,7 @@
   hipStream_t gstream[MAX_GROUPS] = {};
   hipEvent_t ev_chk[2][MAX_GROUPS] = {};
   hipEvent_t ev_fork = nullptr, ev_join[MAX_GROUPS] = {};
-  static constexpr int GRAPH_SLOTS = 48;
+  static constexpr int GRAPH_SLOTS = 96;
   CachedGraph graphs[MAX_GROUPS][GRAPH_SLOTS];
   CachedGraph chain_graph;
   int last_chunks = 0, last_lean_launches = 0, last_full_launches = 0;
diff --git a/unified_cvo_amd/csrc/cvo_k_assoc.h b/unified_cvo_amd/csrc/cvo_k_assoc.h
--- a/unified_cvo_amd/csrc/cvo_k_assoc.h
+++ b/unified_cvo_amd/csrc/cvo_k_assoc.h
@@ -30,7 +30,8 @@
   }
   return acc;
 }
-__device__ __forceinline__ void twist_finalize(const PairDesc* __restrict__ D, int nparts, unsigned tag, int stamp_epoch, int stamp_k) {
+__device__ __forceinline__ void twist_finalize(const PairDesc* __restrict__ D, int nparts, unsigned tag, int stamp_epoch, int stamp_k,
+                                               float* twist_out = nullptr) {
   double acc = coeff_twist_load(D, nparts, tag);
   acc += dpp_f64<0x128>(acc);
   acc = xor16_sum(acc);
@@ -47,6 +48,10 @@
     own = own / sq;
 #pragma unroll
     for (int q = 0; q < 6; q++) ov[q] = __builtin_bit_cast(float, __builtin_amdgcn_readlane(__builtin_bit_cast(int, own), q));
+  }
+  if (twist_out) {
+#pragma unroll
+    for (int q = 0; q < 6; q++) twist_out[q] = ov[q];
   }
   XiMats M;
   xi_mats(ov, ov + 3, M);
@@ -149,7 +154,7 @@
   unsigned long long cnt[ASSOC_THREADS / 64][4];
 };
 
-template <typename IdxT, int ASSOC_CAP, int FEAT, bool INSTR>
+template <typename IdxT, int ASSOC_CAP, int FEAT, bool INSTR, bool FUSED = false>
 __device__ __forceinline__ void assoc_phase(const DevParams& P, const PairDesc* __restrict__ D, const IterView& iv,
                                             AssocShared& S, const int bx, const AssocRowHead& head, const unsigned tag) {
   const int N = D->N;
@@ -279,6 +284,12 @@
     cp[1] = a1;
     cp[2] = a2;
     cp[3] = a3;
+    if (FUSED) {
+      const unsigned long long t = (unsigned long long)tag << 32;
+      unsigned long long* cg = D->flow_part + (size_t)bx * FLOW_GRANULES + FLOW_COUNT_GRANULE;
+      __hip_atomic_store(cg, t | (unsigned long long)(unsigned)a0, __ATOMIC_RELAXED, __HIP_MEMORY_SCOPE_AGENT);
+      __hip_atomic_store(cg + 1, t | (unsigned long long)(unsigned)a1, __ATOMIC_RELAXED, __HIP_MEMORY_SCOPE_AGENT);
+    }
   }
 }
 
diff --git a/unified_cvo_amd/csrc/cvo_k_iter.h b/unified_cvo_amd/csrc/cvo_k_iter.h
--- /dev/null
+++ b/unified_cvo_amd/csrc/cvo_k_iter.h
@@ -0,0 +1,311 @@
+#pragma once
+#include "cvo_k_assoc.h"
+#include "cvo_k_coeff.h"
+#include "cvo_update.h"
+
+namespace cvo_dev {
+
+constexpr int SHADOW_EXT_FLAGS = 4, SHADOW_EXT_NNZ = 5, SHADOW_EXT_MAX = 6;
+static_assert(SHADOW_WORDS - HOT_DWORDS > SHADOW_EXT_MAX, "the shadow holds k_iter's three words behind UpdOut's four");
+constexpr int ITER_HEAD_WORDS = 20;
+static_assert(offsetof(PairState, Tinv) / 4 + 3 == ITER_HEAD_WORDS && ITER_HEAD_WORDS < 64, "the head of PairState");
+
+__device__ __forceinline__ unsigned iter_tag(unsigned long long serial, int epoch) {
+  return partial_tag(serial, 0x40000000u | (unsigned)epoch);
+}
+
+struct IterShared {
+  union {
+    AssocShared a;
+    CoeffShared c;
+    UpdateShared u;
+  };
+};
+
+struct PredHead {
+  bool valid;
+  int status, rebuild, n_ovf, K, epoch, k;
+  float ell;
+  Pose pose;
+};
+__device__ __forceinline__ PredHead load_pred_head(const unsigned long long* shadow, unsigned tag, int flags) {
+  const int lane = threadIdx.x & 63;
+  const int src = lane < ITER_HEAD_WORDS ? lane : HOT_DWORDS + SHADOW_EXT_FLAGS;
+  const unsigned long long g = ld_g<true>(as_global(shadow) + src);
+  const bool ok = lane > ITER_HEAD_WORDS || (unsigned)(g >> 32) == tag;
+  auto word = [&](int l) { return __builtin_amdgcn_readlane((int)(unsigned)g, l); };
+  PredHead h;
+  h.valid = __ballot(!ok) == 0ull && word(ITER_HEAD_WORDS) == flags;
+  h.status = word(offsetof(PairState, status) / 4);
+  h.rebuild = word(offsetof(PairState, rebuild) / 4);
+  h.n_ovf = word(offsetof(PairState, n_ovf) / 4);
+  h.K = word(offsetof(PairState, K) / 4);
+  h.ell = __int_as_float(word(offsetof(PairState, ell) / 4));
+  h.epoch = word(offsetof(PairState, epoch) / 4);
+  h.k = word(offsetof(PairState, k) / 4);
+#pragma unroll
+  for (int q = 0; q < 9; q++) h.pose.Ri[q] = __int_as_float(word(offsetof(PairState, Rinv) / 4 + q));
+#pragma unroll
+  for (int q = 0; q < 3; q++) h.pose.Ti[q] = __int_as_float(word(offsetof(PairState, Tinv) / 4 + q));
+  return h;
+}
+
+__device__ __forceinline__ void reduce_counts_tagged(const PairDesc* __restrict__ D, int nparts, unsigned tag, unsigned long long* s_n) {
+  const int lane = threadIdx.x & 63;
+  const CVO_GLOBAL unsigned long long* src = as_global(D->flow_part) + FLOW_COUNT_GRANULE;
+  unsigned sum = 0, mx = 0;
+  for (int b0 = 0; b0 < nparts; b0 += 64) {
+    const int b = min(b0 + lane, nparts - 1);
+    TaggedF64 p;
+    for (int polls = 0;; polls++) {
+      p = ld_tagged<true>(src + (size_t)b * FLOW_GRANULES);
+      if (__ballot(!p.carries(tag)) == 0ull) break;
+      if (polls > PARTIAL_POLL_LIMIT) {
+        if (lane == 0) D->st->sync_err = 1;
+        break;
+      }
+      __builtin_amdgcn_s_sleep(2);
+    }
+    if (b0 + lane < nparts) {
+      const unsigned a = (unsigned)p.lo, r = sum + a;
+      sum = r < sum ? 0xffffffffu : r;
+      mx = max(mx, (unsigned)p.hi);
+    }
+  }
+  const unsigned long long tot = wave_sum_u32(sum);
+  const unsigned m = wave_max_u32(mx);
+  if (lane == 0) {
+    s_n[0] = tot > 0xffffffffull ? 0xffffffffull : tot;
+    s_n[1] = m;
+    s_n[2] = 0ull;
+    s_n[3] = 0ull;
+  }
+}
+
+__device__ __forceinline__ bool iter_update(const UpdDesc& D, const DevParams& P, const int flags, UpdateShared& U, const float* twist,
+                                            const unsigned* preloaded_hot, const unsigned tag_coef, const unsigned tag_pred) {
+  PairState* const gst = D.st;
+  double* const s_c = U.c;
+  unsigned long long* const s_n = U.n;
+  unsigned* const s_hot = U.hot;
+  const int tid = threadIdx.x;
+  s_hot[tid] = preloaded_hot[0];
+  if (tid + 64 < HOT_DWORDS) s_hot[tid + 64] = preloaded_hot[1];
+  PairState* const st = reinterpret_cast<PairState*>(s_hot);
+  const unsigned long long g0 = ld_g<true>(as_global(D.shadow) + tid), g1 = ld_g<true>(as_global(D.shadow) + 64 + tid);
+  update_reduce<true>(D, P, D.nblk_coeff, tag_coef, st, s_c, s_n);
+  auto ext = [&](int q) { return (unsigned)__builtin_amdgcn_readlane((int)(unsigned)g1, HOT_DWORDS - 64 + q); };
+  const bool have_pred = __ballot((unsigned)(g0 >> 32) != tag_pred || (unsigned)(g1 >> 32) != tag_pred) == 0ull &&
+                         (int)ext(SHADOW_EXT_FLAGS) == flags;
+  if (have_pred && tid == 0) {
+    s_n[0] = ext(SHADOW_EXT_NNZ);
+    s_n[1] = ext(SHADOW_EXT_MAX);
+    s_n[2] = 0ull;
+    s_n[3] = 0ull;
+  }
+  __syncthreads();
+  float e_front = 0.f, s_front = 0.f;
+  if (tid == 0) {
+    e_front = gst->eq[st->e_head];
+    s_front = gst->sq[st->s_head];
+  }
+  const float step_w = select_step<true>(s_c[0], s_c[1], s_c[2], s_c[3], P.min_step, P.max_step);
+  bool hit = have_pred && __float_as_uint(step_w) == ext(3) && s_hot[offsetof(PairState, sync_err) / 4] == 0u;
+  if (hit && P.debug_fuse_mispredict > 0) {
+    const int m = gst->n_fuse_match + 1;
+    if (tid == 0) gst->n_fuse_match = m;
+    if (m % P.debug_fuse_mispredict == 0) hit = false;
+  }
+  UpdOut out;
+  if (hit) {
+    s_hot[tid] = (unsigned)g0;
+    if (tid + 64 < HOT_DWORDS) s_hot[tid + 64] = (unsigned)g1;
+    __builtin_amdgcn_wave_barrier();
+    if (tid == 0) {
+      st->B = s_c[0];
+      st->C = s_c[1];
+      st->D = s_c[2];
+      st->E = s_c[3];
+      st->n_adopted++;
+      gst->n_fused++;
+      if (ext(1)) {
+        *D.want_out = (int)ext(2);
+        *D.want_host = (int)ext(2);
+      }
+      if (ext(0)) {
+        *D.status_out = 1;
+        *D.status_host = 1;
+      }
+    }
+  } else if (tid == 0) {
+    update_advance<false>(D, P, flags | ITER_FROM_COEFF, st, gst->sq, gst->eq, s_c, s_n, step_w, twist, e_front, s_front, 0ull, false, out);
+    if (have_pred) gst->n_mispred++;
+  }
+  __syncthreads();
+  for (int q = tid; q < HOT_DWORDS; q += 64) reinterpret_cast<unsigned*>(gst)[q] = s_hot[q];
+  return hit;
+}
+
+__device__ __forceinline__ void iter_predict(const UpdDesc& D, const PairDesc* __restrict__ Dp, const DevParams& P, const int flags_next,
+                                             UpdateShared& U, const float* tw, const unsigned tag_assoc, const int nparts) {
+  const int tid = threadIdx.x;
+  PairState* const gst = D.st;
+  PairState* const st = reinterpret_cast<PairState*>(U.hot);
+  const float pred = st->step;
+  if (flags_next < 0 || !step_is_clamp(P, pred) || st->status != 0) return;
+  const unsigned tag = iter_tag(Dp->call_serial, st->epoch);
+  reduce_counts_tagged(Dp, nparts, tag_assoc, U.n);
+  __builtin_amdgcn_wave_barrier();
+  if (tid == 0) {
+    const float e_front = gst->eq[st->e_head], s_front = gst->sq[st->s_head];
+    const unsigned nnz = (unsigned)U.n[0], mx = (unsigned)U.n[1];
+    UpdOut out;
+    update_advance<false>(D, P, flags_next | ITER_FROM_COEFF, st, gst->sq, gst->eq, nullptr, U.n, pred, tw, e_front, s_front, 0ull, true, out);
+    U.ext[0] = (unsigned)out.done;
+    U.ext[1] = (unsigned)out.want_write;
+    U.ext[2] = (unsigned)out.want_val;
+    U.ext[3] = __float_as_uint(pred);
+    for (int q = 4; q < SHADOW_WORDS - HOT_DWORDS; q++) U.ext[q] = 0u;
+    U.ext[SHADOW_EXT_FLAGS] = (unsigned)flags_next;
+    U.ext[SHADOW_EXT_NNZ] = nnz;
+    U.ext[SHADOW_EXT_MAX] = mx;
+  }
+  __builtin_amdgcn_wave_barrier();
+  const unsigned long long t = (unsigned long long)tag << 32;
+  const unsigned w0 = U.hot[tid], w1 = (tid + 64 < HOT_DWORDS) ? U.hot[tid + 64] : U.ext[tid + 64 - HOT_DWORDS];
+  __hip_atomic_store(D.shadow + tid, t | w0, __ATOMIC_RELAXED, __HIP_MEMORY_SCOPE_AGENT);
+  __hip_atomic_store(D.shadow + 64 + tid, t | w1, __ATOMIC_RELAXED, __HIP_MEMORY_SCOPE_AGENT);
+}
+
+#ifndef CVO_ITER_WAVES
+#define CVO_ITER_WAVES 5
+#endif
+
+template <typename IdxT, int ASSOC_CAP, int FEAT>
+__global__ __launch_bounds__(ASSOC_THREADS, FEAT != FEAT_GEO ? 1 : CVO_ITER_WAVES) void k_iter(
+    const PairDesc* __restrict__ descs, const DevParams* __restrict__ Pp, PairState* states, const char* __restrict__ arena, int flags,
+    int flags_next, int nblk_pairs, unsigned stride256, int Npad) {
+  const AssocWord aw = unpack_assoc_word(nblk_pairs);
+  const int nblk = aw.nblk, n_pairs = aw.n_pairs;
+  PairBlock pb;
+  if (!pair_block(nblk, n_pairs, pb)) return;
+  const PairDesc* __restrict__ D = descs + pb.pair;
+  PairState* const st = states + pb.pair;
+  const PairState* __restrict__ st_in = states + pb.pair;
+  AssocRowHead ahead;
+  CoeffRowHead chead;
+  {
+    const char* wb = arena + (size_t)pb.pair * ((size_t)stride256 << 8);
+    const int pos = pb.bx * ASSOC_THREADS + threadIdx.x;
+    ahead.ip = FEAT != FEAT_GEO ? reinterpret_cast<const int*>(wb + row_off_ip(Npad))[pos] : 0;
+    ahead.j1 = (int)reinterpret_cast<const IdxT*>(wb + row_off_cand_j(Npad))[pos];
+    ahead.x = reinterpret_cast<const float4*>(wb + row_off_xp4(Npad))[pos];
+    ahead.cnt = __float_as_int(ahead.x.w);
+    chead.nnz = nnz_count(reinterpret_cast<const unsigned*>(wb + row_off_nnz(Npad))[pos]);
+    chead.x = ahead.x;
+    chead.dense = false;
+    chead.e_n = reinterpret_cast<const EllEntry*>(wb + row_off_ell(Npad))[pos];
+  }
+  const int status_v = st_in->status, rebuild_v = st_in->rebuild, ovf = st_in->n_ovf;
+  const int epoch = st_in->epoch, k_v = st_in->k;
+  const int xe = __float_as_int(st_in->xi[46]), xk = __float_as_int(st_in->xi[47]);
+  const DevParams P = *Pp;
+  XiMats Mu;
+  {
+    float* mu = reinterpret_cast<float*>(&Mu);
+#pragma unroll
+    for (int q = 0; q < (int)(sizeof(XiMats) / sizeof(float)); q++) mu[q] = st_in->xi[q];
+  }
+  const unsigned long long serial = D->call_serial;
+  const unsigned long long* const shadow = D->shadow;
+  if (status_v != 0) return;
+  const SlotState sv{rebuild_v, ovf};
+  if (slot_waits(flags, ITER_LEAN, ITER_LEAN_DENSE, &sv)) {
+    if (pb.bx == 0 && threadIdx.x == 0) {
+      st->n_stalls++;
+      if (ovf > 0) {
+        const int want = want_encode(2, true);
+        st->want_full = want;
+        *D->want_out = want;
+        *D->want_host = want;
+      }
+    }
+    return;
+  }
+  const bool primed = xe == epoch && xk == k_v;
+  __shared__ IterShared S;
+  __shared__ int s_last;
+  const int N_ = D->N, pos_ = pb.bx * ASSOC_THREADS + threadIdx.x;
+
+  IterView iv;
+  bool do_assoc;
+  int a_k;
+  if (!primed) {
+    iv = load_iter_view(st_in);
+    do_assoc = true;
+    a_k = k_v;
+  } else {
+    const PredHead ph = load_pred_head(shadow, iter_tag(serial, epoch), flags);
+    do_assoc = ph.valid && ph.status == 0 && ph.rebuild == 0 && ph.n_ovf == 0;
+    iv.K = ph.K;
+    iv.ell = ph.ell;
+    iv.row_max = st_in->row_max;
+    iv.pose = ph.pose;
+    a_k = ph.k;
+  }
+  const unsigned tag_assoc = partial_tag(serial, (unsigned)a_k);
+  const unsigned tag_coef = partial_tag(serial, 0x80000000u | (unsigned)epoch);
+
+  if (primed) {
+    if (pos_ >= N_) chead.nnz = 0;
+#ifdef CVO_ELL8
+    const Pose pose = load_pose(st_in);
+#else
+    const Pose pose{};
+#endif
+    coeff_rows<true>(P, D, st_in->ell, st_in->temp_coef, S.c, Mu, chead, pb.bx, 0, 1, pose, tag_coef);
+    if (do_assoc) __syncthreads();
+  }
+  if (do_assoc) assoc_phase<IdxT, ASSOC_CAP, FEAT, false, true>(P, D, iv, S.a, pb.bx, ahead, tag_assoc);
+  if (threadIdx.x >= 64) return;
+
+  unsigned hot_regs[2] = {0u, 0u};
+  hot_regs[0] = reinterpret_cast<const unsigned*>(st)[threadIdx.x];
+  if (threadIdx.x + 64 < HOT_DWORDS) hot_regs[1] = reinterpret_cast<const unsigned*>(st)[threadIdx.x + 64];
+  UpdDesc upd = load_upd_desc(D);
+  upd.nblk_coeff = nblk;
+  __syncthreads();
+  if (threadIdx.x == 0) {
+    if (primed) {
+      const unsigned per_it = (unsigned)(nblk * COEFF_SPLIT_MAX);
+      const unsigned done = (unsigned)__hip_atomic_fetch_add(D->done, (int)COEFF_SPLIT_MAX, __ATOMIC_RELAXED, __HIP_MEMORY_SCOPE_AGENT) + (unsigned)COEFF_SPLIT_MAX;
+      s_last = done == (unsigned)(epoch + 1) * per_it;
+    } else {
+      const int done = __hip_atomic_fetch_add(D->gate_flow, 1, __ATOMIC_RELAXED, __HIP_MEMORY_SCOPE_AGENT);
+      s_last = (done == nblk - 1) ? 1 : 0;
+      if (done == nblk - 1) __hip_atomic_store(D->gate_flow, 0, __ATOMIC_RELAXED, __HIP_MEMORY_SCOPE_AGENT);
+    }
+  }
+  __syncthreads();
+  if (!s_last) return;
+  if (primed) {
+    float twist[6];
+    for (int c = 0; c < 3; c++) {
+      twist[c] = Mu.omega[c];
+      twist[3 + c] = Mu.v[c];
+    }
+    const bool hit = iter_update(upd, P, flags, S.u, twist, hot_regs, tag_coef, iter_tag(serial, epoch));
+    if (!hit || !do_assoc) return;
+  } else {
+    S.u.hot[threadIdx.x] = hot_regs[0];
+    if (threadIdx.x + 64 < HOT_DWORDS) S.u.hot[threadIdx.x + 64] = hot_regs[1];
+    if (threadIdx.x == 0) st->n_primed++;
+  }
+  __builtin_amdgcn_wave_barrier();
+  const PairState* const cur = reinterpret_cast<const PairState*>(S.u.hot);
+  float tw[6];
+  twist_finalize(D, nblk, tag_assoc, cur->epoch, cur->k, tw);
+  iter_predict(upd, D, P, flags_next, S.u, tw, tag_assoc, nblk);
+}
+
+}
diff --git a/unified_cvo_amd/csrc/cvo_kernels.h b/unified_cvo_amd/csrc/cvo_kernels.h
--- a/unified_cvo_amd/csrc/cvo_kernels.h
+++ b/unified_cvo_amd/csrc/cvo_kernels.h
@@ -22,6 +22,7 @@
 #include "cvo_k_assoc_dense.h"
 #include "cvo_update.h"
 #include "cvo_k_coeff.h"
+#include "cvo_k_iter.h"
 #include "cvo_k_overlap.h"
 #include "cvo_k_coeff_dense.h"
 #include "cvo_k_debug.h"
diff --git a/unified_cvo_amd/csrc/cvo_launch.hip b/unified_cvo_amd/csrc/cvo_launch.hip
--- a/unified_cvo_amd/csrc/cvo_launch.hip
+++ b/unified_cvo_amd/csrc/cvo_launch.hip
@@ -78,6 +78,29 @@
   else
     hipLaunchKernelGGL(k_coeff<false>, row_grid(nblk * split + 1, n_pairs), dim3(ASSOC_THREADS), 0, s, descs, dp, st, A.base, flags,
                        packed, A.stride256, A.Npad);
+}
+
+void launch_iter(hipStream_t s, bool idx16, int feat, int nblk, int n_pairs, const PairDesc* descs, const DevParams* dp, PairState* st,
+                 const ArenaArg& A, int flags, int flags_next) {
+  const dim3 grid = row_grid(nblk, n_pairs), blk(ASSOC_THREADS);
+  const int packed = pack_assoc_word(0, nblk, n_pairs);
+#define CVO_ITER_CASE(F)                                                                                                       \
+  case F:                                                                                                                      \
+    if (idx16)                                                                                                                 \
+      hipLaunchKernelGGL((k_iter<unsigned short, ASSOC_CAP16, F>), grid, blk, 0, s, descs, dp, st, A.base, flags, flags_next, \
+                         packed, A.stride256, A.Npad);                                                                         \
+    else                                                                                                                       \
+      hipLaunchKernelGGL((k_iter<int, ASSOC_CAP32, F>), grid, blk, 0, s, descs, dp, st, A.base, flags, flags_next, packed,    \
+                         A.stride256, A.Npad);                                                                                 \
+    break;
+  switch (feat) {
+    CVO_ITER_CASE(FEAT_GEO)
+    CVO_ITER_CASE(FEAT_COL)
+    CVO_ITER_CASE(FEAT_HOT)
+    default:
+      CVO_ITER_CASE(FEAT_ALL)
+  }
+#undef CVO_ITER_CASE
 }
 
 void launch_verify(hipStream_t s, int feat, int nblk, int n_pairs, const PairDesc* descs, const DevParams* dp, const int* st,
@@ -174,11 +197,21 @@
     }
     return;
   }
+  auto lean_slot = [&](int u) {
+    const bool last = (u % p.period == p.period - 1) || u == p.U - 1;
+    return IterSlot{.lean = true, .lean_dense = p.dense, .idx32 = !g.idx16, .rebuild_follows = last, .horizon = std::min(p.period, g.horizon_cap)};
+  };
+  if (p.fused) {
+    for (int u = 0; u < p.U; u++) {
+      if (u % p.period == 0) launch_rebuild(c, g);
+      launch_iter(g.stream, g.idx16, g.feat, g.nba, g.n_pairs, c->d_descs + g.p0, c->d_params, c->d_states + g.p0, g.arena,
+                  iteration_words(lean_slot(u)).iter, iteration_words(lean_slot((u + 1) % p.U)).iter);
+    }
+    return;
+  }
   for (int u = 0; u < p.U; u++) {
     if (u % p.period == 0) launch_rebuild(c, g);
-    const bool last = (u % p.period == p.period - 1) || u == p.U - 1;
-    launch_core(c, g, {.lean = true, .lean_dense = p.dense, .idx32 = !g.idx16, .rebuild_follows = last,
-                       .horizon = std::min(p.period, g.horizon_cap)});
+    launch_core(c, g, lean_slot(u));
   }
 }
 
diff --git a/unified_cvo_amd/csrc/cvo_options.h b/unified_cvo_amd/csrc/cvo_options.h
--- a/unified_cvo_amd/csrc/cvo_options.h
+++ b/unified_cvo_amd/csrc/cvo_options.h
@@ -19,7 +19,7 @@
   int first_chunks = 2;
   int streams = 0;
   int queue_admit = 4;
-  bool no_sort = false, no_long_lists = false, no_onehot = false, ip_chain = false, keep_columns = false, no_speculate = false;
+  bool no_sort = false, no_long_lists = false, no_onehot = false, ip_chain = false, keep_columns = false, no_speculate = false, no_fuse = false;
   CloudOrder order = CloudOrder::Device;
   int row_max = ASSOC_CAP16;
   int voxel_host = -1;
@@ -31,7 +31,7 @@
   int voxel_prepass = 1;
   int verbose = 0;
   bool kernel_clock = false, phase_ticks = false, verify_lists = false, debug_no_motion_bound = false;
-  int debug_drop_partial = 0;
+  int debug_drop_partial = 0, debug_fuse_mispredict = 0;
 };
 
 enum class OptKind { Flag, Level, Integer, Real, Order };
@@ -70,6 +70,7 @@
     opt_flag("IP_CHAIN", &CtxOptions::ip_chain),
     opt_flag("KEEP_COLUMNS", &CtxOptions::keep_columns),
     opt_flag("NO_SPECULATE", &CtxOptions::no_speculate),
+    opt_flag("NO_FUSE", &CtxOptions::no_fuse),
     opt_int("VOXEL_HOST", &CtxOptions::voxel_host, -1, 1),
     opt_int("VOXEL_PREPASS", &CtxOptions::voxel_prepass, 0, 1),
     opt_int("RGBD_HOST", &CtxOptions::rgbd_host, -1, 1),
@@ -83,6 +84,7 @@
     opt_flag("VERIFY_LISTS", &CtxOptions::verify_lists),
     opt_flag("DEBUG_NO_MOTION_BOUND", &CtxOptions::debug_no_motion_bound),
     opt_int("DEBUG_DROP_PARTIAL", &CtxOptions::debug_drop_partial),
+    opt_int("DEBUG_FUSE_MISPREDICT", &CtxOptions::debug_fuse_mispredict, 0),
 };
 
 inline void parse_option(CtxOptions& o, const OptionSpec& s, const char* text) {
diff --git a/unified_cvo_amd/csrc/cvo_sched.hip b/unified_cvo_amd/csrc/cvo_sched.hip
--- a/unified_cvo_amd/csrc/cvo_sched.hip
+++ b/unified_cvo_amd/csrc/cvo_sched.hip
@@ -71,6 +71,7 @@
   d.verify_lists = o.verify_lists;
   d.debug_no_motion_bound = o.debug_no_motion_bound;
   d.debug_drop_partial = o.debug_drop_partial;
+  d.debug_fuse_mispredict = o.debug_fuse_mispredict;
   if (!c) return d;
 
   const cvo_align_opts_t* opts = c->opts;
@@ -173,6 +174,11 @@
     st.ell = opts->ell0;
     st.K = opts->K0;
   }
+  {
+    const int none = -1;
+    std::memcpy(&st.xi[46], &none, sizeof none);
+    std::memcpy(&st.xi[47], &none, sizeof none);
+  }
   st.K_last = 0;
 }
 
@@ -360,12 +366,20 @@
   int U, U_late, lean_U, lean_U2;
   bool instr;
   bool allow_lean, start_nodense, allow_calm;
+  bool fuse;
 };
+
+bool fuse_allowed(const cvo_ctx* ctx, const BatchSetup& S, const DevParams& dp) {
+  const CtxOptions& o = ctx->opt;
+  if (o.no_fuse || o.no_speculate || dp.no_speculate || dp.mode != CALL_ALIGN || dp.trace_capacity != 0) return false;
+  if (S.geom.instr || S.geom.verify || S.geom.csplit > 1) return false;
+  return dp.min_step > 0.f && dp.min_step * 0.9999f - 1e-6f > dp.eps_2 && dp.max_step <= 1.f;
+}
 
 LoopCfg loop_cfg(const cvo_ctx* ctx, const BatchSetup& S, const DevParams& dp, int U, int U_late) {
   const bool allow_lean = !ctx->opt.no_lean;
   return {U, U_late, std::max(1, std::min(dp.lean_U, U)), std::max(0, std::min(dp.lean_U2, U)), S.geom.instr,
-          allow_lean, allow_lean && S.N > 4096, dp.calm_U > 0};
+          allow_lean, allow_lean && S.N > 4096, dp.calm_U > 0, fuse_allowed(ctx, S, dp)};
 }
 
 LaunchGeom group_geom(const cvo_ctx* ctx, const BatchSetup& S, int n, int g) {
@@ -401,12 +415,13 @@
 ChunkPlan sized_chunk(const LoopCfg& c, ChunkPlan p, int U) {
   p.U = U;
   p.period = p.kind == ChunkKind::Lean ? c.lean_U : (p.kind == ChunkKind::ShortLean ? c.lean_U2 : (p.kind == ChunkKind::Calm ? U : 0));
+  p.fused = c.fuse && !p.every_iteration() && !p.dense;
   return p;
 }
 
 inline int graph_slot(const LoopCfg& c, const ChunkPlan& p) {
   const int kd = (int)p.kind + (p.dense ? 3 : 0);
-  return kd + (c.instr ? 8 : 0) + 16 * (p.U == c.U ? 0 : (p.U == c.U_late ? 1 : 2));
+  return kd + (c.instr ? 8 : 0) + 16 * (p.U == c.U ? 0 : (p.U == c.U_late ? 1 : 2)) + (p.fused ? 48 : 0);
 }
 
 int chunk_graph(cvo_ctx* ctx, const LaunchGeom* geom, int G, const LoopCfg& cfg, int g, const ChunkPlan& p, hipGraphExec_t* exec) {
@@ -463,7 +478,7 @@
   if (max_iter > 0) {
     const LoopCfg cfg = loop_cfg(ctx, S, dp, U, U_late);
     const int n_chunks = (max_iter + U_first - 1) / U_first;
-    const int chunk_cap = 4 * n_chunks + 16;
+    const int chunk_cap = (cfg.fuse ? 8 : 4) * n_chunks + 16;
     ChunkPlan next[cvo_ctx::MAX_GROUPS];
     for (int g = 0; g < G; g++) next[g] = first_chunk(cfg);
     bool all_done = false;
@@ -477,7 +492,7 @@
       const int Uc = ch < n_first_chunks ? U_first : (ch < n_early_chunks + n_first_chunks ? U : U_late);
       if (verbose >= 3) {
         fprintf(stderr, "[cvo] chunk %d (%d iterations): graphs", ch, Uc);
-        for (int g = 0; g < G; g++) fprintf(stderr, " %s%s", kChunkNames[(int)next[g].kind], next[g].dense ? "+dense" : "");
+        for (int g = 0; g < G; g++) fprintf(stderr, " %s%s%s", kChunkNames[(int)next[g].kind], next[g].dense ? "+dense" : "", sized_chunk(cfg, next[g], Uc).fused ? kChunkFused : "");
         fprintf(stderr, "\n");
       }
       for (int g = 0; g < G; g++) {
diff --git a/unified_cvo_amd/csrc/cvo_update.h b/unified_cvo_amd/csrc/cvo_update.h
--- a/unified_cvo_amd/csrc/cvo_update.h
+++ b/unified_cvo_amd/csrc/cvo_update.h
@@ -428,6 +428,82 @@
   __hip_atomic_store(D.shadow + 64 + tid, t | w1, __ATOMIC_RELAXED, __HIP_MEMORY_SCOPE_AGENT);
 }
 
+template <bool COH>
+__device__ __forceinline__ void update_reduce(const UpdDesc& D, const DevParams& P, const int n_flow_parts, const unsigned tag,
+                                              PairState* const st, double* const s_c, unsigned long long* const s_n) {
+  const int tid = threadIdx.x;
+  const int nba = n_flow_parts, nbc = D.nblk_coeff;
+  const int c = tid >> 4, bl = tid & 15;
+  double s = 0;
+  const CVO_GLOBAL unsigned* cnt32 = as_global(reinterpret_cast<const unsigned*>(D.cnt_part));
+  const CVO_GLOBAL unsigned long long* coef_part = as_global(D.coef_part);
+  unsigned vq[8];
+#pragma unroll
+  for (int u = 0; u < 8; u++) {
+    const int b = bl + 16 * u;
+    vq[u] = b < nba ? ld_g<false>(cnt32 + ((size_t)b * 4 + c) * 2) : 0u;
+  }
+  if (P.mode == CALL_ALIGN) {
+    for (int b0 = bl; b0 < nbc; b0 += 64) {
+      TaggedF64 v[4];
+      for (int polls = 0;; polls++) {
+        bool ok = true;
+#pragma unroll
+        for (int u = 0; u < 4; u++) {
+          const int b = min(b0 + 16 * u, nbc - 1);
+          v[u] = ld_tagged<COH>(coef_part + (size_t)b * COEF_GRANULES + 2 * c);
+        }
+#pragma unroll
+        for (int u = 0; u < 4; u++) ok = ok && (!COH || v[u].carries(tag));
+        if (__ballot(!ok) == 0ull) break;
+        if (polls > PARTIAL_POLL_LIMIT) {
+          if (tid == 0) st->sync_err = 2;
+          break;
+        }
+        __builtin_amdgcn_s_sleep(2);
+      }
+#pragma unroll
+      for (int u = 0; u < 4; u++) s += (b0 + 16 * u < nbc) ? v[u].value() : 0.0;
+    }
+  } else if (c == 0) {
+    for (int b = bl; b < nba; b += 16) s += ld_tagged<false>(as_global(D.flow_part) + (size_t)b * FLOW_GRANULES + 12).value();
+  }
+  auto addsat = [](unsigned a, unsigned b) { const unsigned r = a + b; return r < a ? 0xffffffffu : r; };
+  unsigned q = 0;
+#pragma unroll
+  for (int u = 0; u < 8; u++) q = (c == 1) ? max(q, vq[u]) : addsat(q, vq[u]);
+  for (int b0 = bl + 128; b0 < nba; b0 += 128) {
+    unsigned v[8];
+#pragma unroll
+    for (int u = 0; u < 8; u++) {
+      const int b = b0 + 16 * u;
+      v[u] = b < nba ? ld_g<false>(cnt32 + ((size_t)b * 4 + c) * 2) : 0u;
+    }
+#pragma unroll
+    for (int u = 0; u < 8; u++) q = (c == 1) ? max(q, v[u]) : addsat(q, v[u]);
+  }
+  s += dpp_f64<DPP_XOR1>(s);
+  s += dpp_f64<DPP_XOR2>(s);
+  s += dpp_f64<DPP_HALF_MIRROR>(s);
+  s += dpp_f64<DPP_MIRROR>(s);
+  {
+    auto meet = [&](unsigned o) { q = (c == 1) ? max(q, o) : addsat(q, o); };
+    meet((unsigned)dpp_i32<DPP_XOR1>((int)q));
+    meet((unsigned)dpp_i32<DPP_XOR2>((int)q));
+    meet((unsigned)dpp_i32<DPP_HALF_MIRROR>((int)q));
+    meet((unsigned)dpp_i32<DPP_MIRROR>((int)q));
+  }
+#pragma unroll
+  for (int cc = 0; cc < 4; cc++) {
+    const double sv = lane_f64(s, 16 * cc);
+    const unsigned long long qv = (unsigned long long)(unsigned)__builtin_amdgcn_readlane((int)q, 16 * cc);
+    if (tid == 0) {
+      s_c[cc] = sv;
+      s_n[cc] = qv;
+    }
+  }
+}
+
 template <bool INIT, bool COH>
 __device__ __forceinline__ void update_body(const UpdDesc& D, const DevParams& P, int flags,
                                             int n_flow_parts, UpdateShared& U, const float* twist,
@@ -464,78 +540,7 @@
       g1 = ld_g<true>(as_global(D.shadow) + 64 + tid);
     }
   }
-  if (!INIT && act) {
-    const int nba = n_flow_parts, nbc = D.nblk_coeff;
-    const int c = tid >> 4, bl = tid & 15;
-    double s = 0;
-    const CVO_GLOBAL unsigned* cnt32 = as_global(reinterpret_cast<const unsigned*>(D.cnt_part));
-    const CVO_GLOBAL unsigned long long* coef_part = as_global(D.coef_part);
-    unsigned vq[8];
-#pragma unroll
-    for (int u = 0; u < 8; u++) {
-      const int b = bl + 16 * u;
-      vq[u] = b < nba ? ld_g<false>(cnt32 + ((size_t)b * 4 + c) * 2) : 0u;
-    }
-    if (P.mode == CALL_ALIGN) {
-      for (int b0 = bl; b0 < nbc; b0 += 64) {
-        TaggedF64 v[4];
-        for (int polls = 0;; polls++) {
-          bool ok = true;
-#pragma unroll
-          for (int u = 0; u < 4; u++) {
-            const int b = min(b0 + 16 * u, nbc - 1);
-            v[u] = ld_tagged<COH>(coef_part + (size_t)b * COEF_GRANULES + 2 * c);
-          }
-#pragma unroll
-          for (int u = 0; u < 4; u++) ok = ok && (!COH || v[u].carries(tag));
-          if (__ballot(!ok) == 0ull) break;
-          if (polls > PARTIAL_POLL_LIMIT) {
-            if (tid == 0) st->sync_err = 2;
-            break;
-          }
-          __builtin_amdgcn_s_sleep(2);
-        }
-#pragma unroll
-        for (int u = 0; u < 4; u++) s += (b0 + 16 * u < nbc) ? v[u].value() : 0.0;
-      }
-    } else if (c == 0) {
-      for (int b = bl; b < nba; b += 16) s += ld_tagged<false>(as_global(D.flow_part) + (size_t)b * FLOW_GRANULES + 12).value();
-    }
-    auto addsat = [](unsigned a, unsigned b) { const unsigned r = a + b; return r < a ? 0xffffffffu : r; };
-    unsigned q = 0;
-#pragma unroll
-    for (int u = 0; u < 8; u++) q = (c == 1) ? max(q, vq[u]) : addsat(q, vq[u]);
-    for (int b0 = bl + 128; b0 < nba; b0 += 128) {
-      unsigned v[8];
-#pragma unroll
-      for (int u = 0; u < 8; u++) {
-        const int b = b0 + 16 * u;
-        v[u] = b < nba ? ld_g<false>(cnt32 + ((size_t)b * 4 + c) * 2) : 0u;
-      }
-#pragma unroll
-      for (int u = 0; u < 8; u++) q = (c == 1) ? max(q, v[u]) : addsat(q, v[u]);
-    }
-    s += dpp_f64<DPP_XOR1>(s);
-    s += dpp_f64<DPP_XOR2>(s);
-    s += dpp_f64<DPP_HALF_MIRROR>(s);
-    s += dpp_f64<DPP_MIRROR>(s);
-    {
-      auto meet = [&](unsigned o) { q = (c == 1) ? max(q, o) : addsat(q, o); };
-      meet((unsigned)dpp_i32<DPP_XOR1>((int)q));
-      meet((unsigned)dpp_i32<DPP_XOR2>((int)q));
-      meet((unsigned)dpp_i32<DPP_HALF_MIRROR>((int)q));
-      meet((unsigned)dpp_i32<DPP_MIRROR>((int)q));
-    }
-#pragma unroll
-    for (int cc = 0; cc < 4; cc++) {
-      const double sv = lane_f64(s, 16 * cc);
-      const unsigned long long qv = (unsigned long long)(unsigned)__builtin_amdgcn_readlane((int)q, 16 * cc);
-      if (tid == 0) {
-        s_c[cc] = sv;
-        s_n[cc] = qv;
-      }
-    }
-  }
+  if (!INIT && act) update_reduce<COH>(D, P, n_flow_parts, tag, st, s_c, s_n);
   __syncthreads();
   float e_front = 0.f, s_front = 0.f;
   if (!INIT && tid == 0) {
diff --git a/unified_cvo_amd/csrc/cvo_wave.h b/unified_cvo_amd/csrc/cvo_wave.h
--- a/unified_cvo_amd/csrc/cvo_wave.h
+++ b/unified_cvo_amd/csrc/cvo_wave.h
@@ -176,6 +176,7 @@
   return t;
 }
 constexpr int FLOW_GRANULES = 16, COEF_GRANULES = 8;
+constexpr int FLOW_COUNT_GRANULE = 14;
 constexpr int PARTIAL_POLL_LIMIT = 400000;
 
 }
```

Result: slower. 1088 (-7.4%).
